# paulvoliva/XNODE-WAN-PDE-solver

Measured on AMD Instinct MI355X. Metric: WAN training-steps/sec (optimiser sub-steps, d=20 cube, N_r=4096 paths per GPU), higher is better.
Workload: dtype f64

## Files before the change

include/xnwan.h:

```cpp
#ifndef XNWAN_H
#define XNWAN_H
#ifdef __cplusplus
extern "C" {
#endif

#define XW_E_DIMS     (-1)
#define XW_E_ARG      (-2)
#define XW_E_WORKSPACE (-3)
#define XW_E_COMM     (-4)

int xw_abi_version(void);
int xw_supported_dims(char* buf, int buflen);

int xw_theta_size(int d, int H, int K);
int xw_phi_size(int d, int W);

int xw_ode_fwd(const double* xT, const double* t, const double* start, const double* theta,
               int method, int N, int L, int d, int H, int K, int m,
               double* u, double* Y, void* stream);

typedef struct { const double* xT; const double* start; double* u; double* Y; double* act; int N;
                 int act_x_only;
                 int narrow;
                 int prio_drop;
               } XwOdeFwdJob;
int xw_ode_act_rows(int method, int H, int K, int m);
int xw_ode_fwd_multi(const XwOdeFwdJob* jobs, int njobs, const double* t, const double* theta,
                     int method, int L, int d, int H, int K, int m, double* zero16, void* stream);

int xw_ode_bwd_slabs(int N);

int xw_ode_bwd(const double* xT, const double* t, const double* start, const double* theta, const double* Y,
               const double* ubar, int method, int N, int L, int d, int H, int K, int m, int mode,
               double* gx, double* gs, double* gslab, void* stream);

typedef struct { const double* xT; const double* start; const double* Y; const double* act; const double* ubar;
                 double* gx; double* gs; double* gslab; int N;
                 int res_first_only; const double* res_u; const double* res_ref; double res_coef; double res_base;
                 int res_w_per_point; const double* res_w; const double* res_c; const double* res_cp; double res_kappa2;
               } XwOdeBwdJob;
int xw_ode_bwd_multi(const XwOdeBwdJob* jobs, int njobs, const double* t, const double* theta,
                     int method, int L, int d, int H, int K, int m, int mode, void* stream);

int xw_disc_fwd(const double* xT, const double* t, const double* tpp, const double* phi,
                int N, int L, int d, int W, int q, double* v, double* vt, double* gxv, double* gtv, int ngrad,
                int max_blocks, double* act, void* stream);
int xw_disc_xproj(const double* xT, const double* phi, int N, int d, int W, double* xproj, void* stream);
int xw_disc_fwd_xproj(const double* xT, const double* t, const double* tpp, const double* phi,
                      int N, int L, int d, int W, int q, double* v, double* vt, double* gxv, double* gtv, int ngrad,
                      int max_blocks, double* act, const double* xproj, void* stream);
int xw_disc_act_rows(int W, int q);

int xw_disc_gradx(const double* xT, const double* t, const double* tpp, const double* phi, const double* vbar,
                  int N, int d, int W, int q, double* gxv, double* gtv, void* stream);

int xw_disc_bwd_slabs(int N, int L);
int xw_disc_bwd(const double* xT, const double* t, const double* tpp, const double* phi, const double* vbar,
                int N, int L, int d, int W, int q, const double* act, double* gslab, void* stream);

int xw_weak_partials(const double* u, const double* v, const double* vt, const double* w, int w_per_point,
                     const double* wt, const double* s3x, const double* gx, const double* gs, const double* ghT,
                     const double* gxv, const double* w0, const double* gwx0T, int d, const double* c, double ckappa,
                     const double* f, const double* h, const double* href, int pairwise, double s3_scale, int N, int L,
                     double Vol, double Nglob, double* work, double* scal, int finalize, int Lb, double Nbglob, double alpha,
                     double init_off, double bdry_off, long long* step, const double* ub, const double* gb, long Pb,
                     void* stream);
int xw_pair_fold(double* scal, double Vol, double Nglob, void* stream);
int xw_reduce_work_size(void);
int xw_cube_weight(const float* x, int N, int d, double top, double bot, double* w, double* w0, double* gwT, double* xT,
                   void* stream);
int xw_weak_contract_general(const double* A0, int amode, const double* B0, const double* gx, const double* gs,
                             const double* ghT, const double* gxv, const double* w0, const double* gwx0T, const double* v0,
                             int d, int N, double* s3x, void* stream);
int xw_bdry_partials(const double* ub, const double* g, int Nb, int L, double alpha, double Nbglob,
                     double* ubar_b, double* work, double* scal, void* stream);
int xw_gen_cotangents(const double* u, const double* v, const double* w, int w_per_point, const double* c,
                      const double* cp, double ckappa, const double* h, int N, int L, double Vol, double Nglob,
                      double alpha, double pollution, const double* scal, double* ubarA, double* ubarB, void* stream);
int xw_disc_cotangent(const double* u, const double* v, const double* w, int w_per_point, const double* c,
                      double ckappa, const double* f, const double* h, int N, int L, double Vol, double Nglob,
                      double pollution, double s3_scale, const double* scal_in, double* vbar, void* stream);
int xw_losses(double* scal, int L, int Lb, double Vol, double Nglob, double Nbglob, double alpha, double init_off,
              double bdry_off, long long* step, void* stream);

int xw_adam(double* param, const double* gslabA, int nA, const double* gextraA, const double* gslabB, int nB,
            const double* gextraB, const double* scal, double* m, double* v, long long* step, int bump_step, int P,
            double lr, double beta1, double beta2, double eps, double* gsum_out, int lag_lo, int lag_hi, int skip,
            long long* lag, void* stream);
int xw_slab_sum(const double* gslab, int nslab, int P, int accumulate, double* out, void* stream);
int xw_slab_sum2(const double* gA, int nA, double* outA, const double* gB, int nB, double* outB, int P, void* stream);

typedef struct {
  int N, Nb, L, Lb, d;
  int same_grid;
  int w_per_point, amode, pair_i, pair_b;
  int ns_u, ns_b;
  int narrow;
  int sharded;
  double Vol, Nglob, Nbglob, s3_scale, init_off, bdry_off, ckappa;
  const double *xT, *xvT, *xbT, *t, *tb, *tpp, *xvT_pts;
  const double *start, *start_b, *h, *href, *f, *g, *w, *wt, *w0, *ghT, *gwx0T, *c, *cp, *A0, *B0;
  double *u, *ub, *Y, *Yb, *act, *act_b, *v, *vt, *gxv, *gtv, *gx, *gs, *vbar, *s3x, *vact, *slabA, *slabB, *slab_v, *work_i, *work_b;
  double *xproj;
} XwGroup;
typedef int (*XwExchangeFn)(double* buf, int count, void* ctx, void* stream);
typedef struct {
  int method, H, K, m, W, q, Pu, Pv, adjoint;
  int v_blocks, v_blocks_disc;
  int lag_lo, lag_hi;
  double alpha, pollution, lr_u, lr_v, beta1, beta2, eps;
  double *theta, *phi, *scal, *grad_u, *grad_v, *m_u, *v_u, *m_v, *v_v;
  long long *step_u, *step_v, *lag_u;
  XwExchangeFn exchange;
  void* exchange_ctx;
  double* pack_u;
} XwSolverState;
int xw_substep_gen(const XwGroup* g, const XwSolverState* s, int skip_v, int store_record, double* accum, int adam_skip_field,
                   void* stream);
int xw_substep_disc(const XwGroup* g, const XwSolverState* s, int skip_v, int use_record, double* accum, void* stream);

int xw_comm_available(void);
int xw_comm_unique_id(unsigned char* id128);
int xw_comm_init(const unsigned char* id128, int nranks, int rank, void** comm);
int xw_allreduce(double* buf, int count, void* comm, void* stream);
int xw_comm_destroy(void* comm);

typedef struct XwGather {
  const double* src;
  double* dst;
  long n0, n1, n2;
  long s0, s1, s2;
  long before;
} XwGather;
int xw_gather_fields(const XwGather* table_dev, int count, long total, void* stream);

int xw_mt19937_uniform_f32(void* state_blob, long blob_bytes, float* out, long n, float from, float to, int fused);

int xw_mt19937_legacy_normal_f64(unsigned int* key, int* pos, int* has_gauss, double* cached_gaussian, double* out, long n);

#ifdef __cplusplus
}
#endif
#endif
```

xnode_wan_pde_solver_amd/_lib.py:

```python
import ctypes
import os

_HERE = os.path.dirname(os.path.abspath(__file__))
LIB_PATH = os.environ.get('XW_LIBRARY') or os.path.join(_HERE, 'libxnwan.so')
ABI_VERSION = 31

c_f32p = ctypes.c_void_p
c_f64p = ctypes.c_void_p
c_i64p = ctypes.c_void_p
c_int, c_dbl, c_vp = ctypes.c_int, ctypes.c_double, ctypes.c_void_p


class XwOdeFwdJob(ctypes.Structure):
    _fields_ = [('xT', c_vp), ('start', c_vp), ('u', c_vp), ('Y', c_vp), ('act', c_vp), ('N', c_int), ('act_x_only', c_int),
                ('narrow', c_int), ('prio_drop', c_int)]


class XwOdeBwdJob(ctypes.Structure):
    _fields_ = [('xT', c_vp), ('start', c_vp), ('Y', c_vp), ('act', c_vp), ('ubar', c_vp), ('gx', c_vp), ('gs', c_vp),
                ('gslab', c_vp), ('N', c_int), ('res_first_only', c_int), ('res_u', c_vp), ('res_ref', c_vp),
                ('res_coef', ctypes.c_double), ('res_base', ctypes.c_double), ('res_w_per_point', c_int), ('res_w', c_vp),
                ('res_c', c_vp), ('res_cp', c_vp), ('res_kappa2', ctypes.c_double)]


class XwGroup(ctypes.Structure):
    _fields_ = ([(n, c_int) for n in ('N', 'Nb', 'L', 'Lb', 'd', 'same_grid', 'w_per_point', 'amode', 'pair_i', 'pair_b', 'ns_u', 'ns_b',
                                      'narrow', 'sharded')]
                + [(n, c_dbl) for n in ('Vol', 'Nglob', 'Nbglob', 's3_scale', 'init_off', 'bdry_off', 'ckappa')]
                + [(n, c_vp) for n in ('xT', 'xvT', 'xbT', 't', 'tb', 'tpp', 'xvT_pts', 'start', 'start_b', 'h', 'href', 'f', 'g', 'w',
                                       'wt', 'w0', 'ghT', 'gwx0T', 'c', 'cp', 'A0', 'B0', 'u', 'ub', 'Y', 'Yb', 'act', 'act_b', 'v',
                                       'vt', 'gxv', 'gtv', 'gx', 'gs', 'vbar', 's3x', 'vact', 'slabA', 'slabB', 'slab_v', 'work_i',
                                       'work_b', 'xproj')])


class XwSolverState(ctypes.Structure):
    _fields_ = ([(n, c_int) for n in ('method', 'H', 'K', 'm', 'W', 'q', 'Pu', 'Pv', 'adjoint', 'v_blocks', 'v_blocks_disc', 'lag_lo',
                                      'lag_hi')]
                + [(n, c_dbl) for n in ('alpha', 'pollution', 'lr_u', 'lr_v', 'beta1', 'beta2', 'eps')]
                + [(n, c_vp) for n in ('theta', 'phi', 'scal', 'grad_u', 'grad_v', 'm_u', 'v_u', 'm_v', 'v_v', 'step_u', 'step_v',
                                       'lag_u', 'exchange', 'exchange_ctx', 'pack_u')])


EXCHANGE_FN = ctypes.CFUNCTYPE(ctypes.c_int, ctypes.c_void_p, ctypes.c_int, ctypes.c_void_p, ctypes.c_void_p)


SIGNATURES = {
    'xw_abi_version': [],
    'xw_supported_dims': [ctypes.c_char_p, c_int],
    'xw_theta_size': [c_int, c_int, c_int],
    'xw_phi_size': [c_int, c_int],
    'xw_ode_fwd': [c_f32p, c_f32p, c_f64p, c_f64p, c_int, c_int, c_int, c_int, c_int, c_int, c_int, c_f64p, c_f64p, c_vp],
    'xw_ode_fwd_multi': [ctypes.POINTER(XwOdeFwdJob), c_int, c_f32p, c_f64p, c_int, c_int, c_int, c_int, c_int, c_int, c_f64p,
                         c_vp],
    'xw_ode_bwd_slabs': [c_int],
    'xw_ode_act_rows': [c_int, c_int, c_int, c_int],
    'xw_ode_bwd_multi': [ctypes.POINTER(XwOdeBwdJob), c_int, c_f32p, c_f64p, c_int, c_int, c_int, c_int, c_int, c_int, c_int, c_vp],
    'xw_ode_bwd': [c_f32p, c_f32p, c_f64p, c_f64p, c_f64p, c_f64p, c_int, c_int, c_int, c_int, c_int, c_int, c_int, c_int,
                   c_f64p, c_f64p, c_f64p, c_vp],
    'xw_disc_fwd': [c_f32p, c_f32p, c_f32p, c_f64p, c_int, c_int, c_int, c_int, c_int, c_f64p, c_f64p, c_f64p, c_f64p, c_int,
                    c_int, c_f64p, c_vp],
    'xw_disc_xproj': [c_f32p, c_f64p, c_int, c_int, c_int, c_f64p, c_vp],
    'xw_disc_fwd_xproj': [c_f32p, c_f32p, c_f32p, c_f64p, c_int, c_int, c_int, c_int, c_int, c_f64p, c_f64p, c_f64p, c_f64p, c_int,
                          c_int, c_f64p, c_f64p, c_vp],
    'xw_disc_act_rows': [c_int, c_int],
    'xw_disc_gradx': [c_f32p, c_f32p, c_f32p, c_f64p, c_f64p, c_int, c_int, c_int, c_int, c_f64p, c_f64p, c_vp],
    'xw_disc_bwd_slabs': [c_int, c_int],
    'xw_disc_bwd': [c_f32p, c_f32p, c_f32p, c_f64p, c_f64p, c_int, c_int, c_int, c_int, c_int, c_f64p, c_f64p, c_vp],
    'xw_mt19937_uniform_f32': [c_vp, ctypes.c_long, c_vp, ctypes.c_long, ctypes.c_float, ctypes.c_float, c_int],
    'xw_gather_fields': [c_vp, c_int, ctypes.c_long, c_vp],
    'xw_mt19937_legacy_normal_f64': [c_vp, ctypes.POINTER(c_int), ctypes.POINTER(c_int), ctypes.POINTER(c_dbl), c_vp, ctypes.c_long],
    'xw_weak_partials': [c_f64p, c_f64p, c_f64p, c_f64p, c_int, c_f64p, c_f64p, c_f64p, c_f64p, c_f64p, c_f64p, c_f64p,
                         c_f64p, c_int, c_f64p, c_dbl, c_f64p, c_f64p, c_f64p, c_int, c_dbl, c_int, c_int, c_dbl, c_dbl, c_f64p, c_f64p,
                         c_int, c_int, c_dbl, c_dbl, c_dbl, c_dbl, c_i64p, c_f64p, c_f64p, ctypes.c_long, c_vp],
    'xw_pair_fold': [c_f64p, c_dbl, c_dbl, c_vp],
    'xw_cube_weight': [c_vp, c_int, c_int, c_dbl, c_dbl, c_f64p, c_f64p, c_f64p, c_f64p, c_vp],
    'xw_bdry_partials': [c_f64p, c_f64p, c_int, c_int, c_dbl, c_dbl, c_f64p, c_f64p, c_f64p, c_vp],
    'xw_reduce_work_size': [],
    'xw_weak_contract_general': [c_f64p, c_int, c_f64p, c_f64p, c_f64p, c_f64p, c_f64p, c_f64p, c_f64p, c_f64p, c_int, c_int, c_f64p, c_vp],
    'xw_gen_cotangents': [c_f64p, c_f64p, c_f64p, c_int, c_f64p, c_f64p, c_dbl, c_f64p, c_int, c_int, c_dbl, c_dbl, c_dbl,
                          c_dbl, c_f64p, c_f64p, c_f64p, c_vp],
    'xw_disc_cotangent': [c_f64p, c_f64p, c_f64p, c_int, c_f64p, c_dbl, c_f64p, c_f64p, c_int, c_int, c_dbl, c_dbl, c_dbl,
                          c_dbl, c_f64p, c_f64p, c_vp],
    'xw_losses': [c_f64p, c_int, c_int, c_dbl, c_dbl, c_dbl, c_dbl, c_dbl, c_dbl, c_i64p, c_vp],
    'xw_adam': [c_f64p, c_f64p, c_int, c_f64p, c_f64p, c_int, c_f64p, c_f64p, c_f64p, c_f64p, c_i64p, c_int, c_int, c_dbl,
                c_dbl, c_dbl, c_dbl, c_f64p, c_int, c_int, c_int, c_i64p, c_vp],
    'xw_substep_gen': [ctypes.POINTER(XwGroup), ctypes.POINTER(XwSolverState), c_int, c_int, c_f64p, c_int, c_vp],
    'xw_substep_disc': [ctypes.POINTER(XwGroup), ctypes.POINTER(XwSolverState), c_int, c_int, c_f64p, c_vp],
    'xw_slab_sum': [c_f64p, c_int, c_int, c_int, c_f64p, c_vp],
    'xw_slab_sum2': [c_f64p, c_int, c_f64p, c_f64p, c_int, c_f64p, c_int, c_vp],
    'xw_comm_available': [],
    'xw_comm_unique_id': [ctypes.c_char_p],
    'xw_comm_init': [ctypes.c_char_p, c_int, c_int, ctypes.POINTER(c_vp)],
    'xw_allreduce': [c_f64p, c_int, c_vp, c_vp],
    'xw_comm_destroy': [c_vp],
}

ERRORS = {-1: 'XW_E_DIMS: network widths/depths not among the compiled kernel instantiations',
          -2: 'XW_E_ARG: null pointer, non-positive size or bad enum',
          -3: 'XW_E_WORKSPACE: workspace too small',
          -4: 'XW_E_COMM: RCCL is not available in this process, or a collective call failed'}


class XnwanError(RuntimeError):
    pass


def _load():
    if not os.path.exists(LIB_PATH):
        raise XnwanError(
            'libxnwan.so not found at %s -- build it with `python -c "import __graft_entry__ as g; g.build()"` '
            'or `make -C xnode_wan_pde_solver_amd/csrc`.  There is no CPU fallback.' % LIB_PATH)
    import torch
    lib = ctypes.CDLL(LIB_PATH)
    for name, argtypes in SIGNATURES.items():
        fn = getattr(lib, name)
        fn.argtypes = argtypes
        fn.restype = ctypes.c_int
    got = lib.xw_abi_version()
    if got != ABI_VERSION:
        raise XnwanError('libxnwan.so ABI version %d, host expects %d -- rebuild' % (got, ABI_VERSION))
    return lib


lib = _load()


def check(status, what):
    if status == 0:
        return
    if status in ERRORS:
        buf = ctypes.create_string_buffer(512)
        lib.xw_supported_dims(buf, 512)
        raise XnwanError('%s: %s (compiled: %s)' % (what, ERRORS[status], buf.value.decode()))
    raise XnwanError('%s: HIP launch error %d' % (what, status))
```

xnode_wan_pde_solver_amd/csrc/xw_common.h:

```cpp
#pragma once
#include <hip/hip_runtime.h>

typedef double d4 __attribute__((ext_vector_type(4)));
#define XW_MFMA(a, b, c) __builtin_amdgcn_mfma_f64_16x16x4f64((a), (b), (c), 0, 0, 0)
#define XW_MFMA4(a, b, c) __builtin_amdgcn_mfma_f64_4x4x4f64((a), (b), (c), 0, 0, 0)

#define XW_E_DIMS (-1)
#define XW_ODE_MAX_LAYERS 10
#define XW_E_ARG (-2)
#define XW_E_WORKSPACE (-3)
#define XW_E_COMM (-4)

struct UOff {
  int IL0w, IL0b, IL2w, IL2b, IL4w, IL4b, Win, Winb, Wh, Whb, Wo, Wob, FLw, FLb, total, ldin;
};
__host__ __device__ inline UOff u_offsets(int d, int H, int K) {
  UOff o;
  int p = 0;
  o.IL0w = p; p += H;
  o.IL0b = p; p += H;
  o.IL2w = p; p += H * H;
  o.IL2b = p; p += H;
  o.IL4w = p; p += H * H;
  o.IL4b = p; p += H;
  o.ldin = d + 1 + H;
  o.Win = p; p += K * o.ldin;
  o.Winb = p; p += K;
  o.Wh = p; p += K * K;
  o.Whb = p; p += K;
  o.Wo = p; p += H * K;
  o.Wob = p; p += H;
  o.FLw = p; p += H;
  o.FLb = p; p += 1;
  o.total = p;
  return o;
}
struct VOff {
  int Vin, Vinb, Vh, Vhb, Vo, Vob, total, ldin;
};
__host__ __device__ inline VOff v_offsets(int d, int W) {
  VOff o;
  int p = 0;
  o.ldin = d + 1;
  o.Vin = p; p += W * o.ldin;
  o.Vinb = p; p += W;
  o.Vh = p; p += W * W;
  o.Vhb = p; p += W;
  o.Vo = p; p += W;
  o.Vob = p; p += 1;
  o.total = p;
  return o;
}

typedef const double __attribute__((address_space(1)))* xw_gcp;
typedef double __attribute__((address_space(1)))* xw_gp;
__device__ __forceinline__ double xw_ld_g(const double* p) { return *(xw_gcp)p; }
__device__ __forceinline__ void xw_st_g(double v, double* p) { *(xw_gp)p = v; }
__device__ __forceinline__ double xw_ld_nt(const double* p) { return __builtin_nontemporal_load((xw_gcp)p); }
__device__ __forceinline__ void xw_st_nt(double v, double* p) { __builtin_nontemporal_store(v, (xw_gp)p); }

__device__ __forceinline__ int xw_lane() { return threadIdx.x & 63; }

__device__ __forceinline__ double xw_fragA(const double* __restrict__ Mx, int ld, int rows, int cols, int r0, int c0) {
  const int l = xw_lane();
  const int r = r0 + (l & 15), c = c0 + (l >> 4);
  return (r < rows && c < cols) ? xw_ld_g(Mx + (r * ld + c)) : 0.0;
}
__device__ __forceinline__ double xw_fragAT(const double* __restrict__ Mx, int ld, int rows, int cols, int r0, int c0) {
  const int l = xw_lane();
  const int r = r0 + (l & 15), c = c0 + (l >> 4);
  return (r < cols && c < rows) ? xw_ld_g(Mx + (c * ld + r)) : 0.0;
}
__device__ __forceinline__ double xw_fragAT_l(const double* __restrict__ Mx, int ld, int rows, int cols, int r0, int c0, int l) {
  const int r = r0 + (l & 15), c = c0 + (l >> 4);
  return (r < cols && c < rows) ? xw_ld_g(Mx + (c * ld + r)) : 0.0;
}
__device__ __forceinline__ double xw_fragA4(const double* __restrict__ Mx, int ld, int rows, int cols, int r0, int c0) {
  const int l = xw_lane();
  const int r = r0 + (l & 3), c = c0 + (l >> 4);
  return (r < rows && c < cols) ? xw_ld_g(Mx + (r * ld + c)) : 0.0;
}
__device__ __forceinline__ double xw_fragAT4(const double* __restrict__ Mx, int ld, int rows, int cols, int r0, int c0) {
  const int l = xw_lane();
  const int r = r0 + (l & 3), c = c0 + (l >> 4);
  return (r < cols && c < rows) ? xw_ld_g(Mx + (c * ld + r)) : 0.0;
}
__device__ __forceinline__ double xw_relu1(double x) { return __builtin_fmax(x, 0.0); }
__device__ __forceinline__ d4 xw_vecD(const double* __restrict__ b, int rows, int r0) {
  const int g = xw_lane() >> 4;
  d4 v;
#pragma unroll
  for (int r = 0; r < 4; ++r) {
    const int i = r0 + g + 4 * r;
    v[r] = (i < rows) ? xw_ld_g(b + i) : 0.0;
  }
  return v;
}
__device__ __forceinline__ d4 xw_vecD_strided(const double* __restrict__ b, int stride, int rows, int r0) {
  const int g = xw_lane() >> 4;
  d4 v;
#pragma unroll
  for (int r = 0; r < 4; ++r) {
    const int i = r0 + g + 4 * r;
    v[r] = (i < rows) ? xw_ld_g(b + (long)i * stride) : 0.0;
  }
  return v;
}
__device__ __forceinline__ d4 xw_relu(d4 z) {
  d4 o;
#pragma unroll
  for (int r = 0; r < 4; ++r) o[r] = z[r] > 0.0 ? z[r] : 0.0;
  return o;
}
__device__ __forceinline__ double xw_gate_pos(double b, double x) {
  const unsigned t = (unsigned)__double2loint(b) | (unsigned)__double2hiint(b);
  const int m = -(int)(t < 1u ? t : 1u);
  return __hiloint2double(__double2hiint(x) & m, __double2loint(x) & m);
}
__device__ __forceinline__ d4 xw_zero4() { d4 z = {0.0, 0.0, 0.0, 0.0}; return z; }

__device__ __forceinline__ double xw_tanh(double x) {
  const double am = fmin(fabs(x), 40.0);
  const double y = -2.0 * am;
  const double nb = fma(y, 1.4426950408889634, 6755399441055744.0);
  const double n = nb - 6755399441055744.0;
  double r = fma(n, -6.93147180369123816490e-01, y);
  r = fma(n, -1.90821492927058770002e-10, r);
  double p = 2.08767569878681e-09;
  p = fma(p, r, 2.505210838544172e-08);
  p = fma(p, r, 2.755731922398589e-07);
  p = fma(p, r, 2.7557319223985893e-06);
  p = fma(p, r, 2.48015873015873e-05);
  p = fma(p, r, 0.0001984126984126984);
  p = fma(p, r, 0.001388888888888889);
  p = fma(p, r, 0.008333333333333333);
  p = fma(p, r, 0.041666666666666664);
  p = fma(p, r, 0.16666666666666666);
  p = fma(p, r, 0.5);
  p = fma(p, r, 1.0);
  p = fma(p, r, 1.0);
  const double e = __hiloint2double(__double2hiint(p) + (__double2loint(nb) << 20), __double2loint(p));
  const double num = 1.0 - e, den = 1.0 + e;
  double rc = __builtin_amdgcn_rcp(den);
  rc = fma(fma(-den, rc, 1.0), rc, rc);
  double q = num * rc;
  q = fma(fma(-den, q, num), rc, q);
  return fma(x, 0.0, copysign(q, x));
}

__device__ __forceinline__ double xw_sum_over_g(double x) {
  typedef unsigned xw_u2 __attribute__((ext_vector_type(2)));
  unsigned lo = __double2loint(x), hi = __double2hiint(x);
  xw_u2 a = __builtin_amdgcn_permlane16_swap(lo, lo, false, false);
  xw_u2 b = __builtin_amdgcn_permlane16_swap(hi, hi, false, false);
  x = __hiloint2double(b[0], a[0]) + __hiloint2double(b[1], a[1]);
  lo = __double2loint(x), hi = __double2hiint(x);
  a = __builtin_amdgcn_permlane32_swap(lo, lo, false, false);
  b = __builtin_amdgcn_permlane32_swap(hi, hi, false, false);
  return __hiloint2double(b[0], a[0]) + __hiloint2double(b[1], a[1]);
}
__device__ __forceinline__ double xw_fold32(double a, double b) {
  typedef unsigned xw_u2 __attribute__((ext_vector_type(2)));
  const xw_u2 lo = __builtin_amdgcn_permlane32_swap(__double2loint(a), __double2loint(b), false, false);
  const xw_u2 hi = __builtin_amdgcn_permlane32_swap(__double2hiint(a), __double2hiint(b), false, false);
  return __hiloint2double(hi[0], lo[0]) + __hiloint2double(hi[1], lo[1]);
}
__device__ __forceinline__ double xw_fold16(double a, double b) {
  typedef unsigned xw_u2 __attribute__((ext_vector_type(2)));
  const xw_u2 lo = __builtin_amdgcn_permlane16_swap(__double2loint(a), __double2loint(b), false, false);
  const xw_u2 hi = __builtin_amdgcn_permlane16_swap(__double2hiint(a), __double2hiint(b), false, false);
  return __hiloint2double(hi[0], lo[0]) + __hiloint2double(hi[1], lo[1]);
}
#define XW_DPP_ADD(x, CTRL)                                                                                                    \
  {                                                                                                                            \
    const int lo_ = __builtin_amdgcn_update_dpp(0, __double2loint(x), (CTRL), 0xf, 0xf, true);                                 \
    const int hi_ = __builtin_amdgcn_update_dpp(0, __double2hiint(x), (CTRL), 0xf, 0xf, true);                                 \
    x += __hiloint2double(hi_, lo_);                                                                                           \
  }
__device__ __forceinline__ double xw_sum_over_n(double x) {
  XW_DPP_ADD(x, 0xB1)
  XW_DPP_ADD(x, 0x4E)
  XW_DPP_ADD(x, 0x141)
  XW_DPP_ADD(x, 0x140)
  return x;
}

#define XW_TSTRIDE 17
#define XW_TTILE (16 * XW_TSTRIDE)
__device__ __forceinline__ void xw_writeT(double* tile, d4 q) {
  const int l = xw_lane();
  const int g = l >> 4, n = l & 15;
#pragma unroll
  for (int r = 0; r < 4; ++r) tile[(g + 4 * r) * XW_TSTRIDE + n] = q[r];
}
template <int NR> __device__ __forceinline__ void xw_writeT_n(double* tile, d4 q) {
  const int l = xw_lane();
  const int g = l >> 4, n = l & 15;
#pragma unroll
  for (int r = 0; r < NR; ++r) tile[(g + 4 * r) * XW_TSTRIDE + n] = q[r];
}
template <int NR> __device__ __forceinline__ void xw_writeT_pn(double* tile, d4 q) {
  const int l = xw_lane();
  const int g = l >> 4, n = l & 15, pn = ((n & 3) << 2) | (n >> 2);
#pragma unroll
  for (int r = 0; r < NR; ++r) tile[(g + 4 * r) * XW_TSTRIDE + pn] = q[r];
}
__device__ __forceinline__ double xw_readT(const double* tile, int ks) {
  const int l = xw_lane();
  return tile[(l & 15) * XW_TSTRIDE + 4 * ks + (l >> 4)];
}

static inline int xw_launch_status() {
  hipError_t e = hipGetLastError();
  return e == hipSuccess ? 0 : (int)e;
}
```

xnode_wan_pde_solver_amd/csrc/xw_disc.hip:

```cpp
#include "xw_common.h"
#include "xw_generic.h"
#include <atomic>
#include <cstdlib>

namespace {

template <int W> struct VDim {
  static constexpr int MT = (W + 15) / 16;
  static constexpr int KS = (W + 3) / 4;
  static constexpr int TR = W - 16 * (MT - 1);
  static constexpr bool VTAIL = TR <= 3;
  static constexpr int MTF = VTAIL ? MT - 1 : MT;
  __device__ static constexpr int LR(int mt) { return (W + 1 - 16 * mt) >= 16 ? 4 : (W + 1 - 16 * mt + 3) / 4; }
  static constexpr bool BIASROW = (W % 16) != 0;
  static_assert(MT == 4 || MT == 6 || MT == 8, "row tiles of the compiled widths");
};

struct Pt {
  int p, n;
  bool valid;
  double t;
};
__device__ __forceinline__ Pt locate(long tile, long P, int N, const double* __restrict__ tf, const double* __restrict__ tpp) {
  Pt q;
// ... 74 lines not shown
  }
  if (threadIdx.x < 16 * D::MT) {
    sB[threadIdx.x] = (int)threadIdx.x < W ? ph[o.Vhb + threadIdx.x] : 0.0;
    sB[16 * D::MT + threadIdx.x] = (int)threadIdx.x < W ? ph[o.Vo + threadIdx.x] : 0.0;
    if (VINLDS || XPROJ) {
      sIn[threadIdx.x] = (int)threadIdx.x < W ? ph[o.Vin + (long)threadIdx.x * o.ldin] : 0.0;
      sIn[16 * D::MT + threadIdx.x] = (int)threadIdx.x < W ? ph[o.Vinb + threadIdx.x] : 0.0;
    }
  }
  const int ksd = (d + 3) / 4;
  const int ksl = ksd < VKS ? ksd : VKS;
  if (VINLDS)
    for (int idx = wave; idx < ksl * D::MT; idx += 4) {
      const int ks = idx / D::MT, mt = idx - ks * D::MT;
      sVin[idx * 64 + lane] = xw_fragA(ph + o.Vin + 1, o.ldin, W, d, 16 * mt, 4 * ks);
    }
  if (D::VTAIL)
    for (int idx = threadIdx.x; idx < D::KS * 4 * D::TR; idx += blockDim.x) {
      const int r = idx % D::TR, k = idx / D::TR;
      sT[idx] = k < W ? ph[o.Vh + (long)(16 * (D::MT - 1) + r) * W + k] : 0.0;
    }
  __syncthreads();
  const double vob = ph[o.Vob];
  const long G = (long)gridDim.x * 4;
  const long rot = ntiles >= G ? ntiles % G : 0;
  const int nq = (int)gridDim.x < XW_DISC_NQ ? (int)gridDim.x : XW_DISC_NQ;
  int cur = blockIdx.x % nq, tries = 0;
  int zr = 0;
  asm volatile("" : "+v"(zr));
#ifdef XW_CLOCK_PROBE
  const unsigned long long ck0 = __builtin_amdgcn_s_memtime(), rt0 = __builtin_amdgcn_s_memrealtime();
#endif
  for (long it = (long)blockIdx.x * 4 + wave; it < ntiles;) {
    const long tile = DYN ? it : (it < G ? it - rot + (it < rot ? G : 0) : it);
    long nxt = it + G;
    unsigned int ticket = 0;
    if (DYN && lane == 0) ticket = atomicAdd(queue + cur * XW_DISC_QSTRIDE, 1u);
    const Pt pt = locate(tile, P, N, tf, tpp);
    const bool want_grad = gxv != nullptr && tile * 16 < ngrad;
    d4 a[D::MT], ad[D::MT];
    const long tu = __builtin_amdgcn_readfirstlane((int)tile);
    double* actl = act + tu * ((long)(q + 1) * W * 16);
    asm volatile("" : "+s"(actl));
    const int aoff = lane;
    const double* pht = ph;
    asm volatile("" : "+s"(pht));
    if (XPROJ) {
      const double* xp = xproj + pt.n;
#pragma unroll
      for (int mt = 0; mt < D::MT; ++mt)
#pragma unroll
        for (int r = 0; r < 4; ++r) {
          ad[mt][r] = sIn[16 * mt + g + 4 * r];
          a[mt][r] = (16 * mt + 4 * r < W) ? fma(ad[mt][r], pt.t, xw_ld_g(xp + (long)(16 * mt + 4 * r + g) * N)) : 0.0;
        }
    } else if (VINLDS) {
#pragma unroll
      for (int mt = 0; mt < D::MT; ++mt)
#pragma unroll
        for (int r = 0; r < 4; ++r) {
          ad[mt][r] = sIn[16 * mt + g + 4 * r];
          a[mt][r] = sIn[16 * D::MT + 16 * mt + g + 4 * r] + ad[mt][r] * pt.t;
        }
      for (int ks = 0; ks < ksl; ++ks) {
        const int i = 4 * ks + g;
        const double b = i < d ? xT[(long)i * N + pt.n] : 0.0;
#pragma unroll
        for (int mt = 0; mt < D::MT; ++mt) a[mt] = XW_MFMA(sVin[(ks * D::MT + mt) * 64 + lane], b, a[mt]);
      }
      for (int ks = ksl; ks < ksd; ++ks) {
        const int i = 4 * ks + g;
        const double b = i < d ? xT[(long)i * N + pt.n] : 0.0;
#pragma unroll
        for (int mt = 0; mt < D::MT; ++mt) a[mt] = XW_MFMA(xw_fragA(pht + o.Vin + 1, o.ldin, W, d, 16 * mt, 4 * ks), b, a[mt]);
      }
    } else {
      input_layer<W>(pht, o, xT, N, d, pt, a, ad);
    }
#pragma unroll
    for (int mt = 0; mt < D::MT; ++mt)
#pragma unroll
      for (int r = 0; r < 4; ++r) {
        const double x = a[mt][r];
        a[mt][r] = __hiloint2double(x == 0.0 ? (int)0x80000000 : __double2hiint(x), __double2loint(x));
      }
    if (DYN) {
      nxt = G + cur + (long)nq * (unsigned int)__builtin_amdgcn_readfirstlane((int)ticket);
      while (nxt >= ntiles && tries < XW_DISC_STEAL && tries + 1 < nq) {
        ++tries;
        cur = cur + 1 < nq ? cur + 1 : 0;
        if (lane == 0) ticket = atomicAdd(queue + cur * XW_DISC_QSTRIDE, 1u);
        nxt = G + cur + (long)nq * (unsigned int)__builtin_amdgcn_readfirstlane((int)ticket);
      }
    }
    auto layer = [&](int j, const d4 (&ai)[D::MT], const d4 (&adi)[D::MT], d4 (&nw)[D::MT], d4 (&nd)[D::MT]) {
#pragma unroll
      for (int mt = 0; mt < D::MT; ++mt) {
#pragma unroll
        for (int r = 0; r < 4; ++r) nw[mt][r] = sB[16 * mt + g + 4 * r];
        nd[mt] = xw_zero4();
      }
      if (want_grad) {
        unsigned int mask = 0;
#pragma unroll
        for (int mt = 0; mt < D::MT; ++mt)
#pragma unroll
          for (int r = 0; r < 4; ++r) mask |= (ai[mt][r] > 0.0 ? 1u : 0u) << (4 * mt + r);
        sMask[j][threadIdx.x] = mask;
      }
      double tv[D::TR], td[D::TR];
#pragma unroll
      for (int r = 0; r < D::TR; ++r) tv[r] = td[r] = 0.0;
      double wn[D::MTF], tn[D::TR];
#pragma unroll
      for (int mt = 0; mt < D::MTF; ++mt) wn[mt] = sVh[(mt * D::KS) * 64 + lane];
      if (D::VTAIL)
#pragma unroll
        for (int r = 0; r < D::TR; ++r) tn[r] = sT[g * D::TR + r];
#pragma unroll
      for (int ks = 0; ks < D::KS; ++ks) {
        const double av = ai[ks >> 2][ks & 3];
        int sgn = __double2hiint(av) >> 31;
        asm volatile("" : "+v"(sgn));
        const double adv = adi[ks >> 2][ks & 3];
        const double b = __hiloint2double((sgn & zr) | (~sgn & __double2hiint(av)), (sgn & zr) | (~sgn & __double2loint(av)));
        const double bd = __hiloint2double((sgn & zr) | (~sgn & __double2hiint(adv)), (sgn & zr) | (~sgn & __double2loint(adv)));
        if (ACT) {
          double* __restrict__ rowp = actl + (j * W + 4 * ks) * 16;
          if (4 * ks + 3 < W || 4 * ks + g < W) xw_st_nt(b, rowp + aoff);
        }
        double wc[D::MTF], tc[D::TR];
#pragma unroll
        for (int mt = 0; mt < D::MTF; ++mt) wc[mt] = wn[mt];
#pragma unroll
        for (int r = 0; r < D::TR; ++r) tc[r] = D::VTAIL ? tn[r] : 0.0;
        if (ks + 1 < D::KS) {
#pragma unroll
          for (int mt = 0; mt < D::MTF; ++mt) wn[mt] = sVh[(mt * D::KS + ks + 1) * 64 + lane];
          if (D::VTAIL)
#pragma unroll
            for (int r = 0; r < D::TR; ++r) tn[r] = sT[(4 * (ks + 1) + g) * D::TR + r];
        }
        asm volatile("" ::: "memory");
#pragma unroll
        for (int mt = 0; mt < D::MTF; ++mt) {
          nw[mt] = XW_MFMA(wc[mt], b, nw[mt]);
          nd[mt] = XW_MFMA(wc[mt], bd, nd[mt]);
        }
        if (D::VTAIL) {
#pragma unroll
          for (int r = 0; r < D::TR; ++r) {
            tv[r] = fma(tc[r], b, tv[r]);
            td[r] = fma(tc[r], bd, td[r]);
          }
        }
      }
      if (D::VTAIL && D::TR == 2) {
        const double R = xw_fold16(xw_fold32(tv[0], td[0]), xw_fold32(tv[1], td[1]));
        d4 tw = xw_zero4(), tdd = xw_zero4();
        tw[0] = R + nw[D::MT - 1][0];
        const unsigned rl = __double2loint(R), rh = __double2hiint(R);
        typedef unsigned xw_u2 __attribute__((ext_vector_type(2)));
        const xw_u2 sl = __builtin_amdgcn_permlane32_swap(rl, rl, false, false), sh = __builtin_amdgcn_permlane32_swap(rh, rh, false, false);
        tdd[0] = __hiloint2double(sh[1], sl[1]);
        nw[D::MT - 1] = tw;
        nd[D::MT - 1] = tdd;
      } else
      if (D::VTAIL) {
        d4 tw = xw_zero4(), tdd = xw_zero4();
#pragma unroll
        for (int r = 0; r < D::TR; ++r) {
          const double sv_ = xw_sum_over_g(tv[r]) + nw[D::MT - 1][0], sd_ = xw_sum_over_g(td[r]);
          if (g == r) {
            tw[0] = sv_;
            tdd[0] = sd_;
          }
        }
        nw[D::MT - 1] = tw;
        nd[D::MT - 1] = tdd;
      }
    };
    {
      d4 b0[D::MT], bd0[D::MT];
      int j = 0;
      for (; j + 1 < q; j += 2) {
        layer(j, a, ad, b0, bd0);
        layer(j + 1, b0, bd0, a, ad);
      }
      if (j < q) {
        layer(j, a, ad, b0, bd0);
#pragma unroll
        for (int mt = 0; mt < D::MT; ++mt) {
          a[mt] = b0[mt];
          ad[mt] = bd0[mt];
        }
      }
    }
    double sv = 0.0, sd = 0.0;
#pragma unroll
    for (int mt = 0; mt < D::MT; ++mt)
#pragma unroll
      for (int r = 0; r < 4; ++r)
        if (16 * mt + 4 * r < W) {
          const double th = xw_tanh(a[mt][r]);
          if (ACT && (16 * mt + 4 * r + 3 < W || 16 * mt + 4 * r + g < W))
            xw_st_nt(th, actl + (q * W + 16 * mt + 4 * r) * 16 + aoff);
          const double vo = sB[16 * D::MT + 16 * mt + g + 4 * r];
          sv += vo * th;
          sd += vo * (1.0 - th * th) * ad[mt][r];
          a[mt][r] = vo * (1.0 - th * th);
        } else {
          a[mt][r] = 0.0;
        }
    sv = xw_sum_over_g(sv) + vob;
    sd = xw_sum_over_g(sd);
    if (g == 0 && pt.valid) {
      v[pt.p] = sv;
      if (vt != nullptr) vt[pt.p] = sd;
    }
    if (want_grad) {
      const double* phg = ph;
      asm volatile("" : "+s"(phg));
      int ll = lane;
      asm volatile("" : "+v"(ll));
      d4 (&dl)[D::MT] = a;
      auto fragT = [&](int mt, int ks) -> double { return xw_fragAT_l(phg + o.Vh, W, W, W, 16 * mt, 4 * ks, ll); };
      for (int j = q - 1; j >= 0; --j) {
        d4 nd[D::MT];
#pragma unroll
        for (int mt = 0; mt < D::MT; ++mt) nd[mt] = xw_zero4();
        double fn[D::MT];
#pragma unroll
        for (int mt = 0; mt < D::MT; ++mt) fn[mt] = fragT(mt, 0);
#pragma unroll
        for (int ks = 0; ks < D::KS; ++ks) {
          const double b = dl[ks >> 2][ks & 3];
          double fc[D::MT];
#pragma unroll
          for (int mt = 0; mt < D::MT; ++mt) fc[mt] = fn[mt];
          if (ks + 1 < D::KS) {
#pragma unroll
            for (int mt = 0; mt < D::MT; ++mt) fn[mt] = fragT(mt, ks + 1);
          }
          asm volatile("" ::: "memory");
#pragma unroll
          for (int mt = 0; mt < D::MT; ++mt) nd[mt] = XW_MFMA(fc[mt], b, nd[mt]);
        }
        const unsigned int mask = sMask[j][threadIdx.x];
#pragma unroll
        for (int mt = 0; mt < D::MT; ++mt)
#pragma unroll
          for (int r = 0; r < 4; ++r) dl[mt][r] = ((mask >> (4 * mt + r)) & 1u) ? nd[mt][r] : 0.0;
      }
      int ngl = ngrad;
      asm volatile("" : "+s"(ngl));
      const bool gl = pt.valid && pt.p < ngl;
      for (int rt = 0; rt < (d + 15) / 16; ++rt) {
        d4 vv = xw_zero4();
#pragma unroll
        for (int ks = 0; ks < D::KS; ++ks) {
          if ((ks & 3) == 0) asm volatile("" ::: "memory");
          vv = XW_MFMA(xw_fragAT_l(phg + o.Vin + 1, o.ldin, W, d, 16 * rt, 4 * ks, ll), dl[ks >> 2][ks & 3], vv);
        }
#pragma unroll
        for (int r = 0; r < 4; ++r) {
          const int i = 16 * rt + g + 4 * r;
          if (i < d && gl) gxv[(long)i * ngl + pt.p] = vv[r];
        }
      }
      double st_ = 0.0;
#pragma unroll
      for (int mt = 0; mt < D::MT; ++mt) {
        const d4 v0 = xw_vecD_strided(phg + o.Vin, o.ldin, W, 16 * mt);
#pragma unroll
        for (int r = 0; r < 4; ++r) st_ += v0[r] * dl[mt][r];
      }
      st_ = xw_sum_over_g(st_);
      if (gtv != nullptr && g == 0 && gl) gtv[pt.p] = st_;
    }
    it = nxt;
  }
#ifdef XW_CLOCK_PROBE
  if (lane == 0 && blockIdx.x * 4 + wave < 4096) {
    xw_clock_buf[2 * (blockIdx.x * 4 + wave)] = __builtin_amdgcn_s_memtime() - ck0;
    xw_clock_buf[2 * (blockIdx.x * 4 + wave) + 1] = __builtin_amdgcn_s_memrealtime() - rt0;
  }
#endif
  if (DYN && lane == 0) {
    if (atomicAdd(&sDone, 1u) == 3u && atomicAdd(queue + XW_DISC_NQ * XW_DISC_QSTRIDE, 1u) == gridDim.x - 1u)
      for (int s_ = 0; s_ <= XW_DISC_NQ; ++s_) atomicExch(queue + s_ * XW_DISC_QSTRIDE, 0u);
  }
}

template <int W> struct BwdLds {
  typedef VDim<W> D;
  static constexpr int nfrag = D::MT * D::KS * 64;
  static constexpr int ntt = 4 * D::MT * XW_TTILE;
  static constexpr int oVh = 0, oVhT = nfrag, oD = 2 * nfrag, oR = 2 * nfrag + ntt, oO = 2 * nfrag + 2 * ntt;
  static constexpr int oB = oO + 4 * 64 * 16;
  static constexpr int total = oB + 2 * 16 * D::MT;
  static_assert(total * 8 <= 160 * 1024, "LDS budget of one CU");
};

template <int W, int Q, int CTG, bool PARAMS, bool INGRAD>
__global__ void __launch_bounds__(256) k_disc_bwd(const double* __restrict__ xT, const double* __restrict__ tf,
                                                  const double* __restrict__ tpp, const double* __restrict__ ph,
                                                  const double* __restrict__ vbar, int N, int L, int d,
                                                  double* __restrict__ gslab, double* __restrict__ gxv,
                                                  double* __restrict__ gtv) {
  typedef VDim<W> D;
  typedef BwdLds<W> S;
  static_assert(D::MT == 4, "the recomputing reverse kernel maps the 4 row tiles of dVh onto the 4 waves of a block");
  static_assert(D::BIASROW, "the recomputing reverse kernel takes dVh.b from the ones row");
  __shared__ double lds[S::total];
  double* sVh = lds + S::oVh;
  double* sVhT = lds + S::oVhT;
  double* sD = lds + S::oD;
  double* sR = lds + S::oR;
  double* sO = lds + S::oO;
  const int lane = xw_lane(), g = lane >> 4, n = lane & 15;
  const int wave = threadIdx.x >> 6;
  const VOff o = v_offsets(d, W);
  const long P = (long)N * L;
  const long nsuper = (P + 63) / 64;

  double* sB = lds + S::oB;
  for (int idx = wave; idx < D::MT * D::KS; idx += 4) {
    const int mt = idx / D::KS, ks = idx - mt * D::KS;
    sVh[idx * 64 + lane] = xw_fragA(ph + o.Vh, W, W, W, 16 * mt, 4 * ks);
    sVhT[idx * 64 + lane] = xw_fragAT(ph + o.Vh, W, W, W, 16 * mt, 4 * ks);
  }
  if (threadIdx.x < 16 * D::MT) {
    sB[threadIdx.x] = (int)threadIdx.x < W ? ph[o.Vhb + threadIdx.x] : 0.0;
    sB[16 * D::MT + threadIdx.x] = (int)threadIdx.x < W ? ph[o.Vo + threadIdx.x] : 0.0;
  }
  if (PARAMS)
    for (int i = 0; i < 16; ++i) sO[i * 256 + wave * 64 + lane] = 0.0;
  __syncthreads();

  d4 accH[D::MT], accIn[CTG * 4];
#pragma unroll
  for (int ct = 0; ct < D::MT; ++ct) accH[ct] = xw_zero4();
#pragma unroll
  for (int ct = 0; ct < CTG * 4; ++ct) accIn[ct] = xw_zero4();

  auto layer = [&](const d4 (&r)[D::MT], d4 (&out)[D::MT]) {
    asm volatile("" ::: "memory");
#pragma unroll
    for (int mt = 0; mt < D::MT; ++mt)
#pragma unroll
      for (int rr = 0; rr < 4; ++rr) out[mt][rr] = sB[16 * mt + g + 4 * rr];
#pragma unroll
    for (int ks = 0; ks < D::KS; ++ks) {
      const double b = r[ks >> 2][ks & 3];
#pragma unroll
      for (int mt = 0; mt < D::MT; ++mt) out[mt] = XW_MFMA(sVh[(mt * D::KS + ks) * 64 + lane], b, out[mt]);
    }
  };

  constexpr int SEG = CTG == 1 ? 1 : 3;
  constexpr int NSEG = (Q + SEG - 1) / SEG;
  for (long st = blockIdx.x; st < nsuper; st += gridDim.x) {
    const Pt pt = locate(st * 4 + wave, P, N, tf, tpp);
    d4 ck[NSEG][D::MT];
    d4 a[D::MT], ad[D::MT];
    input_layer<W>(ph, o, xT, N, d, pt, a, ad);
#pragma unroll
    for (int j = 0; j < Q; ++j) {
      d4 r[D::MT];
#pragma unroll
      for (int mt = 0; mt < D::MT; ++mt) {
#pragma unroll
        for (int q_ = 0; q_ < 4; ++q_)
          if (q_ < D::LR(mt)) {
            r[mt][q_] = a[mt][q_] > 0.0 ? a[mt][q_] : 0.0;
            if (j % SEG == 0) ck[j / SEG][mt][q_] = r[mt][q_];
          }
      }
      layer(r, a);
    }
    const double vb = pt.valid ? (vbar != nullptr ? vbar[pt.p] : 1.0) : 0.0;
    d4 dl[D::MT];
#pragma unroll
    for (int mt = 0; mt < D::MT; ++mt)
#pragma unroll
      for (int r = 0; r < 4; ++r) {
        double th = 0.0;
        if (16 * mt + 4 * r < W) th = xw_tanh(a[mt][r]);
        dl[mt][r] = sB[16 * D::MT + 16 * mt + g + 4 * r] * (1.0 - th * th) * vb;
        if (PARAMS) sO[(mt * 4 + r) * 256 + wave * 64 + lane] += (mt == D::MT - 1 && r == 3) ? (g == 0 ? vb : 0.0) : vb * th;
      }
#pragma unroll
    for (int sg = NSEG - 1; sg >= 0; --sg) {
      d4 seg[SEG][D::MT];
#pragma unroll
      for (int mt = 0; mt < D::MT; ++mt)
#pragma unroll
        for (int q_ = 0; q_ < 4; ++q_)
          if (q_ < D::LR(mt)) seg[0][mt][q_] = ck[sg][mt][q_];
#pragma unroll
      for (int k = 1; k < SEG; ++k)
        if (sg * SEG + k < Q) {
          d4 tmp[D::MT];
          layer(seg[k - 1], tmp);
#pragma unroll
          for (int mt = 0; mt < D::MT; ++mt)
#pragma unroll
            for (int q_ = 0; q_ < 4; ++q_)
              if (q_ < D::LR(mt)) seg[k][mt][q_] = tmp[mt][q_] > 0.0 ? tmp[mt][q_] : 0.0;
        }
#pragma unroll
      for (int k = SEG - 1; k >= 0; --k) {
        if (sg * SEG + k >= Q) continue;
        if (PARAMS) {
#pragma unroll
          for (int mt = 0; mt < D::MT; ++mt) {
            d4 rj = seg[k][mt];
            if (mt == (W >> 4)) {
              if (g == ((W & 15) & 3)) rj[(W & 15) >> 2] = 1.0;
            }
            if (mt < D::MT - 1) {
              xw_writeT(sD + (wave * D::MT + mt) * XW_TTILE, dl[mt]);
              xw_writeT(sR + (wave * D::MT + mt) * XW_TTILE, rj);
            } else {
              xw_writeT_n<D::LR(D::MT - 1)>(sD + (wave * D::MT + mt) * XW_TTILE, dl[mt]);
              xw_writeT_n<D::LR(D::MT - 1)>(sR + (wave * D::MT + mt) * XW_TTILE, rj);
            }
          }
        }
        d4 nd[D::MT];
        asm volatile("" ::: "memory");
#pragma unroll
        for (int mt = 0; mt < D::MT; ++mt) nd[mt] = xw_zero4();
#pragma unroll
        for (int ks = 0; ks < D::KS; ++ks) {
          const double b = dl[ks >> 2][ks & 3];
#pragma unroll
          for (int mt = 0; mt < D::MT; ++mt) nd[mt] = XW_MFMA(sVhT[(mt * D::KS + ks) * 64 + lane], b, nd[mt]);
        }
        if (PARAMS) {
          __syncthreads();
#pragma unroll
          for (int pw = 0; pw < 4; ++pw)
#pragma unroll
            for (int ks = 0; ks < 4; ++ks) {
              const double av = xw_readT(sD + (pw * D::MT + wave) * XW_TTILE, ks);
#pragma unroll
              for (int ct = 0; ct < D::MT; ++ct)
                accH[ct] = XW_MFMA(av, xw_readT(sR + (pw * D::MT + ct) * XW_TTILE, ks), accH[ct]);
            }
          __syncthreads();
        }
#pragma unroll
        for (int mt = 0; mt < D::MT; ++mt)
#pragma unroll
          for (int r = 0; r < 4; ++r)
            if (r < D::LR(mt)) dl[mt][r] = seg[k][mt][r] > 0.0 ? nd[mt][r] : 0.0;
      }
    }
    if (PARAMS) {
#pragma unroll
      for (int mt = 0; mt < D::MT; ++mt) xw_writeT(sD + (wave * D::MT + mt) * XW_TTILE, dl[mt]);
#pragma unroll
      for (int grp = 0; grp < CTG; ++grp) {
#pragma unroll
        for (int rr = 0; rr < 16; ++rr) {
          const int cl = g + 4 * rr;
          const int c = 64 * grp + cl;
          double val = 0.0;
          if (pt.valid) {
            if (c == 0) val = pt.t;
            else if (c <= d) val = xT[(long)(c - 1) * N + pt.n];
            else if (c == d + 1) val = 1.0;
          }
          sR[(wave * D::MT + (cl >> 4)) * XW_TTILE + (cl & 15) * XW_TSTRIDE + n] = val;
        }
        __syncthreads();
#pragma unroll
        for (int pw = 0; pw < 4; ++pw)
#pragma unroll
          for (int ks = 0; ks < 4; ++ks) {
            const double av = xw_readT(sD + (pw * D::MT + wave) * XW_TTILE, ks);
#pragma unroll
            for (int ct = 0; ct < 4; ++ct)
              accIn[grp * 4 + ct] = XW_MFMA(av, xw_readT(sR + (pw * D::MT + ct) * XW_TTILE, ks), accIn[grp * 4 + ct]);
          }
        __syncthreads();
      }
    }
    if (INGRAD) {
      for (int rt = 0; rt < (d + 15) / 16; ++rt) {
        d4 vv = xw_zero4();
#pragma unroll
        for (int ks = 0; ks < D::KS; ++ks)
          vv = XW_MFMA(xw_fragAT(ph + o.Vin + 1, o.ldin, W, d, 16 * rt, 4 * ks), dl[ks >> 2][ks & 3], vv);
#pragma unroll
        for (int r = 0; r < 4; ++r) {
          const int i = 16 * rt + g + 4 * r;
          if (i < d && pt.valid) gxv[(long)i * P + pt.p] = vv[r];
        }
      }
      double st_ = 0.0;
#pragma unroll
      for (int mt = 0; mt < D::MT; ++mt) {
        const d4 v0 = xw_vecD_strided(ph + o.Vin, o.ldin, W, 16 * mt);
#pragma unroll
        for (int r = 0; r < 4; ++r) st_ += v0[r] * dl[mt][r];
      }
      st_ = xw_sum_over_g(st_);
      if (gtv != nullptr && g == 0 && pt.valid) gtv[pt.p] = st_;
    }
  }

  if (PARAMS) {
    double* slab = gslab + (long)blockIdx.x * o.total;
#pragma unroll
    for (int ct = 0; ct < D::MT; ++ct) {
      const int c = 16 * ct + n;
#pragma unroll
      for (int r = 0; r < 4; ++r) {
        const int row = 16 * wave + g + 4 * r;
        if (row < W) {
          if (c < W) slab[o.Vh + row * W + c] = accH[ct][r];
          else if (c == W) slab[o.Vhb + row] = accH[ct][r];
        }
      }
    }
#pragma unroll
    for (int ct = 0; ct < CTG * 4; ++ct) {
      const int c = 16 * ct + n;
#pragma unroll
      for (int r = 0; r < 4; ++r) {
        const int row = 16 * wave + g + 4 * r;
        if (row < W) {
          if (c <= d) slab[o.Vin + row * o.ldin + c] = accIn[ct][r];
          else if (c == d + 1) slab[o.Vinb + row] = accIn[ct][r];
        }
      }
    }
    __syncthreads();
    const int tid = threadIdx.x;
    if (tid <= W) {
      double s = 0.0;
      if (tid < W) {
        const int mt = tid >> 4, gg = tid & 3, r = (tid & 15) >> 2;
        for (int wv = 0; wv < 4; ++wv)
          for (int nn = 0; nn < 16; ++nn) s += sO[(mt * 4 + r) * 256 + wv * 64 + gg * 16 + nn];
        slab[o.Vo + tid] = s;
      } else {
        for (int wv = 0; wv < 4; ++wv)
          for (int nn = 0; nn < 16; ++nn) s += sO[15 * 256 + wv * 64 + nn];
        slab[o.Vob] = s;
      }
    }
  }
}

#ifdef XW_REC_PROBE
__device__ unsigned long long xw_rec_clock[12 * 2048];
#define XW_PH(i) { const unsigned long long t_ = __builtin_amdgcn_s_memtime(); phc[i] += t_ - phl; phl = t_; }
#else
#define XW_PH(i)
#endif
template <int W> struct RecLds {
  typedef VDim<W> D;
  static constexpr bool VT = D::VTAIL;
  static_assert(!VT || D::LR(D::MT - 1) == 1, "short last row tile: vector-ALU tail + one live 4-row group");
  static constexpr int T3 = VT ? 4 * XW_TSTRIDE : XW_TTILE;
  static constexpr int wset = (D::MT - 1) * XW_TTILE + T3;
  static constexpr bool FRAG_LDS = D::MT == 4;
  static constexpr int oVhT = 0;
  static constexpr int oTT = oVhT + (FRAG_LDS ? D::MTF * D::KS * 64 : 0);
  static constexpr int oVo = oTT + (VT ? 4 * D::KS * D::TR : 0);
  static constexpr int oD = oVo + 16 * D::MT;
  static constexpr int oR = oD + 4 * wset;
  static constexpr int oO = oR + 4 * wset;
  static constexpr int NO = 4 * D::MT;
  static constexpr int total = oO + (NO + 1) * 16;
  static_assert(total * 8 <= (VT ? 80 : 160) * 1024, "two blocks per CU (short tail) / one");
  __device__ static constexpr int toff(int mt) { return mt * XW_TTILE; }
};

template <int W> __device__ __forceinline__ double rec_readT(const double* set, int mt, int ks) {
  const int l = xw_lane();
  const int row = (RecLds<W>::VT && mt == VDim<W>::MT - 1) ? (l & 3) : (l & 15);
  return set[RecLds<W>::toff(mt) + row * XW_TSTRIDE + 4 * ks + (l >> 4)];
}

template <int W, int Q, int NG, bool TSUM>
__global__ void __launch_bounds__(256, RecLds<W>::VT ? 2 : 1) k_disc_rec(const double* __restrict__ xT, const double* __restrict__ tf,
                                                     const double* __restrict__ tpp, const double* __restrict__ ph,
                                                     const double* __restrict__ vbar, int N, int L, int d,
                                                     double* __restrict__ gslab, const double* __restrict__ act, int qrt) {
  typedef VDim<W> D;
  typedef RecLds<W> S;
  __shared__ double lds[S::total];
  double* sVhT = lds + S::oVhT;
  double* sTT = lds + S::oTT;
  double* sVo = lds + S::oVo;
  double* sO = lds + S::oO;
  const int lane = xw_lane(), g = lane >> 4, n = lane & 15;
  const int wave = threadIdx.x >> 6;
  double* myD = lds + S::oD + wave * S::wset;
  double* myR = lds + S::oR + wave * S::wset;
#ifdef XW_REC_PROBE
  const unsigned long long ck_in = __builtin_amdgcn_s_memtime(), rt_in = __builtin_amdgcn_s_memrealtime();
#endif
  const VOff o = v_offsets(d, W);
  const long P = (long)N * L;
  const long nsuper = (P + 63) / 64;
  const int nq = Q > 0 ? Q : qrt;
  constexpr int UNROLL = Q > 0 ? Q : 1;
  constexpr int TW = D::MT / 2;
  const int wi = wave >> 1, wj = wave & 1;

  if (S::FRAG_LDS)
    for (int idx = wave; idx < D::MTF * D::KS; idx += 4) {
      const int mt = idx / D::KS, ks = idx - mt * D::KS;
      sVhT[idx * 64 + lane] = xw_fragAT(ph + o.Vh, W, W, W, 16 * mt, 4 * ks);
    }
  if (S::VT)
    for (int idx = threadIdx.x; idx < 4 * D::KS * D::TR; idx += blockDim.x) {
      const int r = idx % D::TR, k = idx / D::TR;
      sTT[idx] = k < W ? ph[o.Vh + (long)k * W + 16 * (D::MT - 1) + r] : 0.0;
    }
  if (threadIdx.x < 16 * D::MT) sVo[threadIdx.x] = (int)threadIdx.x < W ? ph[o.Vo + threadIdx.x] : 0.0;
  for (int idx = threadIdx.x; idx < (S::NO + 1) * 16; idx += blockDim.x) sO[idx] = 0.0;
  __syncthreads();

  d4 accH[TW * TW], accB[D::MT];
#pragma unroll
  for (int ct = 0; ct < TW * TW; ++ct) accH[ct] = xw_zero4();
#pragma unroll
  for (int ct = 0; ct < D::MT; ++ct) accB[ct] = xw_zero4();
  constexpr bool EDGE = S::VT;
  constexpr int NE = 7;
  double accE[NE];
#pragma unroll
  for (int e = 0; e < NE; ++e) accE[e] = 0.0;
  const int vstart = wave == 1 ? 7 : wave == 3 ? 6 : 0;
  const int lane16 = (lane & 15) * XW_TSTRIDE + (lane >> 4);
  const int lane4 = (lane & 3) * XW_TSTRIDE + ((lane >> 2) & 3) * 4 + (lane >> 4);
  const int offC = (wave < 3 ? S::oD + wave * XW_TTILE : S::oR + 2 * XW_TTILE) + lane16;
  const int offW = (wave < 3 ? S::oR : S::oD) + lane16;
  const int offX = (wave < 2 ? S::oD : S::oR) + 48 * XW_TSTRIDE + lane4;
  const int offV = (wave < 2 ? S::oR : S::oD) + vstart * 4 * XW_TSTRIDE + lane4;
  double* slab = gslab + (long)blockIdx.x * o.total;

#ifdef XW_REC_PROBE
  unsigned long long phc[8] = {0, 0, 0, 0, 0, 0, 0, 0}, phl = __builtin_amdgcn_s_memtime();
#endif
  const long ngs = N >> 6;
  const long ub = nsuper / gridDim.x, ur = nsuper % gridDim.x;
  const long u0 = (long)blockIdx.x * ub + ((long)blockIdx.x < ur ? (long)blockIdx.x : ur), u1 = u0 + ub + ((long)blockIdx.x < ur ? 1 : 0);
  d4 sumS[D::MT], sumT[D::MT];
#pragma unroll
  for (int mt = 0; mt < D::MT; ++mt) sumS[mt] = sumT[mt] = xw_zero4();
  bool slab_first = true;
  for (long it = TSUM ? u0 : (long)blockIdx.x; it < (TSUM ? u1 : nsuper); it += TSUM ? 1 : (long)gridDim.x) {
    const long ung = TSUM ? it / L : 0;
    const long st = TSUM ? (it - ung * L) * ngs + ung : it;
    const Pt pt = locate(st * 4 + wave, P, N, tf, tpp);
    const long ntile = (P + 15) >> 4;
    const long tl = st * 4 + wave < ntile ? st * 4 + wave : ntile - 1;
    const double* tbase = act + (long)__builtin_amdgcn_readfirstlane((int)tl) * ((long)(nq + 1) * W * 16);
    const int aoff = lane;
    auto load_layer = [&](int j, d4 (&r)[D::MT]) {
      const double* base = tbase + j * W * 16;
      asm volatile("" : "+s"(base));
#pragma unroll
      for (int mt = 0; mt < D::MT; ++mt)
#pragma unroll
        for (int q_ = 0; q_ < 4; ++q_)
          if (q_ < D::LR(mt)) {
            const int row = 16 * mt + 4 * q_ + g;
            r[mt][q_] = (16 * mt + 4 * q_ + 3 < W || row < W) ? xw_ld_nt(base + (16 * mt + 4 * q_) * 16 + aoff) : 0.0;
          }
    };
    d4 a[D::MT], rnext[D::MT];
    load_layer(nq, a);
    if (nq > 0) load_layer(nq - 1, rnext);
    const double vb = pt.valid ? (vbar != nullptr ? xw_ld_g(vbar + pt.p) : 1.0) : 0.0;
    d4 dl[D::MT];
#pragma unroll
    for (int mt = 0; mt < D::MT; ++mt)
#pragma unroll
      for (int r = 0; r < 4; ++r) {
        if (r < D::LR(mt) && 16 * mt + 4 * r < W) {
          const double th = a[mt][r];
          dl[mt][r] = sVo[16 * mt + g + 4 * r] * (1.0 - th * th) * vb;
          const double s_ = xw_sum_over_n(vb * th);
          if (n == 0) sO[(mt * 4 + r) * 16 + wave * 4 + g] += s_;
        } else {
          dl[mt][r] = 0.0;
        }
      }
    {
      const double s_ = xw_sum_over_n(vb);
      if (lane == 0) sO[S::NO * 16 + wave * 4] += s_;
    }
    XW_PH(6)
#pragma unroll UNROLL
    for (int sg = nq - 1; sg >= 0; --sg) {
      bool open[4 * D::MT];
#pragma unroll
      for (int mt = 0; mt < D::MT; ++mt)
#pragma unroll
        for (int r = 0; r < 4; ++r) open[4 * mt + r] = r < D::LR(mt) && rnext[mt][r] > 0.0;
#pragma unroll
      for (int mt = 0; mt < D::MT; ++mt) {
        d4 rr = rnext[mt];
        if (D::BIASROW && mt == (W >> 4)) {
          if (g == ((W & 15) & 3)) rr[(W & 15) >> 2] = 1.0;
        }
        if (!D::BIASROW) accB[mt] = accB[mt] + dl[mt];
        if (mt < D::MT - 1 || !S::VT) {
          xw_writeT(myD + S::toff(mt), dl[mt]);
          xw_writeT(myR + S::toff(mt), rr);
        } else {
          xw_writeT_n<1>(myD + S::toff(mt), dl[mt]);
          xw_writeT_n<1>(myR + S::toff(mt), rr);
        }
      }
      if (sg > 0) load_layer(sg - 1, rnext);
      XW_PH(0)
      d4 nd[D::MT];
      asm volatile("" ::: "memory");
#pragma unroll
      for (int mt = 0; mt < D::MT; ++mt) nd[mt] = xw_zero4();
      double tv[D::TR];
#pragma unroll
      for (int r = 0; r < D::TR; ++r) tv[r] = 0.0;
      if constexpr (S::FRAG_LDS) {
#pragma unroll
        for (int ks = 0; ks < D::KS; ++ks) {
          const double b = dl[ks >> 2][ks & 3];
          if ((ks & 1) == 0) asm volatile("" ::: "memory");
#pragma unroll
          for (int mt = 0; mt < D::MTF; ++mt) nd[mt] = XW_MFMA(sVhT[(mt * D::KS + ks) * 64 + lane], b, nd[mt]);
          if (S::VT) {
#pragma unroll
            for (int r = 0; r < D::TR; ++r) tv[r] = fma(sTT[(4 * ks + g) * D::TR + r], b, tv[r]);
          }
        }
      } else {
        const double* phg = ph;
        int ll = lane;
        asm volatile("" : "+s"(phg), "+v"(ll));
        double fn[D::MT];
#pragma unroll
        for (int mt = 0; mt < D::MT; ++mt) fn[mt] = xw_fragAT_l(phg + o.Vh, W, W, W, 16 * mt, 0, ll);
#pragma unroll
        for (int ks = 0; ks < D::KS; ++ks) {
          const double b = dl[ks >> 2][ks & 3];
          double fc[D::MT];
#pragma unroll
          for (int mt = 0; mt < D::MT; ++mt) fc[mt] = fn[mt];
          if (ks + 1 < D::KS) {
#pragma unroll
            for (int mt = 0; mt < D::MT; ++mt) fn[mt] = xw_fragAT_l(phg + o.Vh, W, W, W, 16 * mt, 4 * (ks + 1), ll);
          }
          asm volatile("" ::: "memory");
#pragma unroll
          for (int mt = 0; mt < D::MT; ++mt) nd[mt] = XW_MFMA(fc[mt], b, nd[mt]);
        }
      }
      if (S::VT) {
#pragma unroll
        for (int r = 0; r < D::TR; ++r) {
          const double s_ = xw_sum_over_g(tv[r]);
          if (g == r) nd[D::MT - 1][0] = s_;
        }
      }
      XW_PH(1)
      if (EDGE) {
#pragma unroll
        for (int ks = 0; ks < 4; ++ks)
          accH[2] = XW_MFMA(xw_readT(myD + S::toff(2), ks), xw_readT(myR + S::toff(2), ks), accH[2]);
      }
      XW_PH(2)
      __syncthreads();
      XW_PH(3)
      if (EDGE) {
#pragma unroll
        for (int pw = 0; pw < 4; ++pw) {
          const double* set = lds + pw * S::wset;
#pragma unroll
          for (int ks = 0; ks < 4; ++ks) {
            if ((ks & 1) == 0) asm volatile("" ::: "memory");
            const double xc = set[offC + 4 * ks], w0 = set[offW + 4 * ks], w1 = set[offW + XW_TTILE + 4 * ks];
            accH[0] = XW_MFMA(xc, w0, accH[0]);
            accH[1] = XW_MFMA(xc, w1, accH[1]);
          }
          asm volatile("" ::: "memory");
          const double x = set[offX];
#pragma unroll
          for (int e = 0; e < NE; ++e)
            if (e < NE - 1 || wave == 0) accE[e] = XW_MFMA4(x, set[offV + e * 4 * XW_TSTRIDE], accE[e]);
        }
      } else {
#pragma unroll
        for (int pw = 0; pw < 4; ++pw) {
          const double* setD = lds + S::oD + pw * S::wset;
          const double* setR = lds + S::oR + pw * S::wset;
#pragma unroll
          for (int ks = 0; ks < 4; ++ks) {
            if ((ks & 1) == 0) asm volatile("" ::: "memory");
            double aa[TW], bb[TW];
#pragma unroll
            for (int i_ = 0; i_ < TW; ++i_) {
              aa[i_] = rec_readT<W>(setD, TW * wi + i_, ks);
              bb[i_] = rec_readT<W>(setR, TW * wj + i_, ks);
            }
#pragma unroll
            for (int i_ = 0; i_ < TW; ++i_)
#pragma unroll
              for (int j_ = 0; j_ < TW; ++j_) accH[i_ * TW + j_] = XW_MFMA(aa[i_], bb[j_], accH[i_ * TW + j_]);
          }
        }
      }
      XW_PH(4)
      __syncthreads();
      XW_PH(5)
#pragma unroll
      for (int mt = 0; mt < D::MT; ++mt)
#pragma unroll
        for (int r = 0; r < 4; ++r) dl[mt][r] = open[4 * mt + r] ? nd[mt][r] : 0.0;
    }
    constexpr int RH = (D::MT + 3) / 4;
    struct InAcc { d4 v[RH]; };
    auto contract_input = [&](const d4 (&Dm)[D::MT], const int rows, const InAcc& acc0, InAcc* keep0) {
#pragma unroll
      for (int mt = 0; mt < D::MT; ++mt) {
        if (mt < D::MT - 1 || !S::VT) xw_writeT(myD + S::toff(mt), Dm[mt]);
        else xw_writeT_n<1>(myD + S::toff(mt), Dm[mt]);
      }
      const double* xl = xT;
      double* sl = slab;
      int gl = g, nl = n;
      asm volatile("" : "+s"(xl), "+s"(sl), "+v"(gl), "+v"(nl));
#pragma unroll
      for (int grp = 0; grp < NG; ++grp) {
        if (rows == 2 && grp > 0) break;
        const int nct = rows == 2 ? 1 : (d + 2 - 48 * grp >= 33 ? 3 : d + 2 - 48 * grp >= 17 ? 2 : 1);
#pragma unroll
        for (int rr = 0; rr < 12; ++rr) {
          if (rr >= 4 * nct) continue;
          const int cl = gl + 4 * rr;
          const int c = 48 * grp + cl;
          double val = 0.0;
          if (pt.valid) {
            if (rows == 2) val = c == 0 ? 1.0 : 0.0;
            else if (c == 0) val = rows == 0 ? pt.t : 0.0;
            else if (c <= d) val = xw_ld_g(xl + (long)(c - 1) * N + pt.n);
            else if (c == d + 1) val = 1.0;
          }
          myR[S::toff(cl >> 4) + (cl & 15) * XW_TSTRIDE + nl] = val;
        }
        __syncthreads();
        d4 accIn[RH][3];
#pragma unroll
        for (int rh = 0; rh < RH; ++rh) {
#pragma unroll
          for (int ct = 0; ct < 3; ++ct) accIn[rh][ct] = xw_zero4();
          if (grp == 0) accIn[rh][0] = acc0.v[rh];
        }
#pragma unroll
        for (int pw = 0; pw < 4; ++pw) {
          const double* setD = lds + S::oD + pw * S::wset;
          const double* setR = lds + S::oR + pw * S::wset;
#pragma unroll
          for (int ks = 0; ks < 4; ++ks) {
            double av[RH], bv[3];
#pragma unroll
            for (int rh = 0; rh < RH; ++rh) av[rh] = rec_readT<W>(setD, wave + 4 * rh < D::MT ? wave + 4 * rh : wave, ks);
#pragma unroll
            for (int ct = 0; ct < 3; ++ct) bv[ct] = ct < nct ? rec_readT<W>(setR, ct, ks) : 0.0;
#pragma unroll
            for (int rh = 0; rh < RH; ++rh)
#pragma unroll
              for (int ct = 0; ct < 3; ++ct)
                if (ct < nct) accIn[rh][ct] = XW_MFMA(av[rh], bv[ct], accIn[rh][ct]);
          }
        }
        __syncthreads();
        if (keep0 != nullptr) {
#pragma unroll
          for (int rh = 0; rh < RH; ++rh) keep0->v[rh] = accIn[rh][0];
          break;
        }
#pragma unroll
        for (int rh = 0; rh < RH; ++rh)
#pragma unroll
          for (int ct = 0; ct < 3; ++ct) {
            if (ct >= nct) continue;
            const int c = 48 * grp + 16 * ct + nl;
#pragma unroll
            for (int r = 0; r < 4; ++r) {
              const int row = 16 * (wave + 4 * rh) + gl + 4 * r;
              if (wave + 4 * rh < D::MT && row < W && c <= d + 1) {
                double* dst = c <= d ? sl + o.Vin + row * o.ldin + c : sl + o.Vinb + row;
                xw_st_g(slab_first ? accIn[rh][ct][r] : xw_ld_g(dst) + accIn[rh][ct][r], dst);
              }
            }
          }
      }
    };
    InAcc zacc;
#pragma unroll
    for (int rh = 0; rh < RH; ++rh) zacc.v[rh] = xw_zero4();
    if (!TSUM) {
      contract_input(dl, 0, zacc, nullptr);
      slab_first = false;
    } else {
      const double tl = pt.t;
#pragma unroll
      for (int mt = 0; mt < D::MT; ++mt)
#pragma unroll
        for (int r = 0; r < 4; ++r)
          if (r < D::LR(mt)) {
            sumS[mt][r] += dl[mt][r];
            sumT[mt][r] = fma(tl, dl[mt][r], sumT[mt][r]);
          }
      if (it + 1 == u1 || (it + 1) / L != ung) {
        InAcc tcol;
        contract_input(sumT, 2, zacc, &tcol);
        contract_input(sumS, 1, tcol, nullptr);
        slab_first = false;
#pragma unroll
        for (int mt = 0; mt < D::MT; ++mt) sumS[mt] = sumT[mt] = xw_zero4();
      }
    }
    XW_PH(7)
  }
#ifdef XW_REC_PROBE
  const unsigned long long ck_loop = __builtin_amdgcn_s_memtime();
#endif

  if (EDGE) {
#pragma unroll
    for (int t2 = 0; t2 < 2; ++t2)
#pragma unroll
      for (int r = 0; r < 4; ++r) {
        const int row = wave < 3 ? 16 * wave + g + 4 * r : 16 * t2 + n, c = wave < 3 ? 16 * t2 + n : 32 + g + 4 * r;
        slab[o.Vh + row * W + c] = accH[t2][r];
      }
    __syncthreads();
    double* s22 = lds + S::oD;
#pragma unroll
    for (int r = 0; r < 4; ++r) s22[wave * 256 + (g + 4 * r) * 16 + n] = accH[2][r];
    __syncthreads();
    {
      const int i = threadIdx.x >> 4, j = threadIdx.x & 15;
      slab[o.Vh + (32 + i) * W + 32 + j] = (s22[threadIdx.x] + s22[256 + threadIdx.x]) + (s22[512 + threadIdx.x] + s22[768 + threadIdx.x]);
    }
#pragma unroll
    for (int e = 0; e < NE; ++e) {
      double s_ = accE[e];
      s_ += __shfl_xor(s_, 4);
      s_ += __shfl_xor(s_, 8);
      if ((e < NE - 1 || wave == 0) && (lane & 12) == 0) {
        const int i = lane >> 4, j = lane & 3, blk = vstart + e;
        const int row = wave < 2 ? 48 + i : 4 * blk + j, c = wave < 2 ? 4 * blk + j : 48 + i;
        if (row < W) {
          if (c < W) slab[o.Vh + row * W + c] = s_;
          else if (c == W) slab[o.Vhb + row] = s_;
        }
      }
    }
  } else {
#pragma unroll
    for (int t4 = 0; t4 < TW * TW; ++t4) {
      const int c = 16 * (TW * wj + (t4 % TW)) + n;
#pragma unroll
      for (int r = 0; r < 4; ++r) {
        const int row = 16 * (TW * wi + (t4 / TW)) + g + 4 * r;
        if (row < W) {
          if (c < W) slab[o.Vh + row * W + c] = accH[t4][r];
          else if (c == W) slab[o.Vhb + row] = accH[t4][r];
        }
      }
    }
  }
  __syncthreads();
  const int tid = threadIdx.x;
  if (!D::BIASROW) {
    double* sBsum = lds + S::oD;
#pragma unroll
    for (int mt = 0; mt < D::MT; ++mt)
#pragma unroll
      for (int r = 0; r < 4; ++r) {
        const double s_ = xw_sum_over_n(accB[mt][r]);
        if (n == 0) sBsum[wave * 16 * D::MT + 16 * mt + 4 * r + g] = s_;
      }
    __syncthreads();
    if (tid < W) slab[o.Vhb + tid] = sBsum[tid] + sBsum[16 * D::MT + tid] + sBsum[32 * D::MT + tid] + sBsum[48 * D::MT + tid];
  }
  if (tid <= W) {
    double s_ = 0.0;
    if (tid < W) {
      const int mt = tid >> 4, gg = tid & 3, r = (tid & 15) >> 2;
      for (int wv = 0; wv < 4; ++wv) s_ += sO[(mt * 4 + r) * 16 + wv * 4 + gg];
      slab[o.Vo + tid] = s_;
    } else {
      for (int wv = 0; wv < 4; ++wv) s_ += sO[S::NO * 16 + wv * 4];
      slab[o.Vob] = s_;
    }
  }
#ifdef XW_REC_PROBE
  if (lane == 0 && blockIdx.x * 4 + wave < 2048) {
    unsigned long long* o_ = xw_rec_clock + 12 * (blockIdx.x * 4 + wave);
    for (int i = 0; i < 8; ++i) o_[i] = phc[i];
    const unsigned long long ck_out = __builtin_amdgcn_s_memtime();
    o_[8] = ck_loop - ck_in - (phc[0] + phc[1] + phc[2] + phc[3] + phc[4] + phc[5] + phc[6] + phc[7]);
    o_[9] = ck_out - ck_loop;
    o_[10] = ck_out - ck_in;
    o_[11] = __builtin_amdgcn_s_memrealtime() - rt_in;
  }
#endif
}

int bwd_blocks(long P) {
  long nsuper = (P + 63) / 64;
  return (int)(nsuper < 512 ? nsuper : 512);
}

}

static bool disc_width_ok(int W) { return W == 50 || W == 64 || W == 96 || W == 128; }
extern "C" int xw_disc_act_rows(int W, int q) { return ((disc_width_ok(W) && q >= 0) || xwg_disc_ok(1, W, q)) ? (q + 1) * W : XW_E_DIMS; }

namespace {
__global__ void __launch_bounds__(256) k_disc_xproj(const double* __restrict__ xT, const double* __restrict__ ph, int N, int d, int W,
                                                     double* __restrict__ xproj) {
  const int n = blockIdx.x * 256 + threadIdx.x;
  const int r0 = blockIdx.y * 4;
  if (n >= N) return;
  const VOff o = v_offsets(d, W);
  const int r1 = r0 + 1 < W ? r0 + 1 : W - 1, r2 = r0 + 2 < W ? r0 + 2 : W - 1, r3 = r0 + 3 < W ? r0 + 3 : W - 1, rr = r0 < W ? r0 : W - 1;
  const double* w0 = ph + o.Vin + (long)rr * o.ldin + 1;
  const double* w1 = ph + o.Vin + (long)r1 * o.ldin + 1;
  const double* w2 = ph + o.Vin + (long)r2 * o.ldin + 1;
  const double* w3 = ph + o.Vin + (long)r3 * o.ldin + 1;
  double a0 = ph[o.Vinb + rr], a1 = ph[o.Vinb + r1], a2 = ph[o.Vinb + r2], a3 = ph[o.Vinb + r3];
#pragma unroll 4
  for (int i = 0; i < d; ++i) {
    const double x = xT[(long)i * N + n];
    a0 = fma(w0[i], x, a0);
    a1 = fma(w1[i], x, a1);
    a2 = fma(w2[i], x, a2);
    a3 = fma(w3[i], x, a3);
  }
  xproj[(long)r0 * N + n] = r0 < W ? a0 : 0.0;
  xproj[(long)(r0 + 1) * N + n] = r0 + 1 < W ? a1 : 0.0;
  xproj[(long)(r0 + 2) * N + n] = r0 + 2 < W ? a2 : 0.0;
  xproj[(long)(r0 + 3) * N + n] = r0 + 3 < W ? a3 : 0.0;
}
}

extern "C" int xw_disc_xproj(const double* xT, const double* phi, int N, int d, int W, double* xproj, void* stream) {
  if (!xT || !phi || !xproj || N <= 0 || d <= 0) return XW_E_ARG;
  if (!disc_width_ok(W)) return XW_E_DIMS;
  hipLaunchKernelGGL(k_disc_xproj, dim3((N + 255) / 256, W > 96 ? 32 : W > 64 ? 24 : 16), dim3(256), 0, (hipStream_t)stream, xT, phi, N, d, W, xproj);
  return xw_launch_status();
}

extern "C" int xw_disc_fwd(const double* xT, const double* t, const double* tpp, const double* phi, int N, int L, int d,
                           int W, int q, double* v, double* vt, double* gxv, double* gtv, int ngrad, int max_blocks,
                           double* act, void* stream) {
  return xw_disc_fwd_xproj(xT, t, tpp, phi, N, L, d, W, q, v, vt, gxv, gtv, ngrad, max_blocks, act, nullptr, stream);
}

extern "C" int xw_disc_fwd_xproj(const double* xT, const double* t, const double* tpp, const double* phi, int N, int L, int d,
                                 int W, int q, double* v, double* vt, double* gxv, double* gtv, int ngrad, int max_blocks,
                                 double* act, const double* xproj, void* stream) {
  if (!xT || !phi || !v || N <= 0 || L <= 0 || d <= 0 || q < 0) return XW_E_ARG;
  if (!tpp && !t) return XW_E_ARG;
  if (tpp && L != 1) return XW_E_ARG;
  if (gxv && (ngrad <= 0 || (long)ngrad > (long)N * L || q > XW_QMAX)) return XW_E_ARG;
  if (!disc_width_ok(W)) return xwg_disc_fwd(xT, t, tpp, phi, N, L, d, W, q, v, vt, gxv, gtv, ngrad, act, stream);
  if (xproj != nullptr && tpp != nullptr) return XW_E_ARG;
  const long ntiles = ((long)N * L + 15) / 16;
  long blocks = (ntiles + 3) / 4;
  long cap = max_blocks > 0 ? max_blocks : 512;
  if (blocks > cap) blocks = cap;
  if ((long)N * L * 4 >= (1L << 31)) return XW_E_ARG;
  static const bool dyn_on = [] { const char* e = getenv("XW_DISC_DYNAMIC"); return !(e && e[0] == '0'); }();
  static unsigned int* qbase = [] { void* p = nullptr; (void)hipGetSymbolAddress(&p, HIP_SYMBOL(xw_disc_queue)); return (unsigned int*)p; }();
  static std::atomic<unsigned int> next_slot[2];
  const bool dyn = dyn_on && qbase != nullptr && ntiles > 4 * blocks;
  unsigned int* queue = nullptr;
  if (dyn) {
    hipStreamCaptureStatus cs = hipStreamCaptureStatusNone;
    if (hipStreamIsCapturing((hipStream_t)stream, &cs) != hipSuccess) cs = hipStreamCaptureStatusNone;
    const int half = cs == hipStreamCaptureStatusActive ? 1 : 0;
    const unsigned int slot = half * (XW_DISC_SLOTS / 2) + next_slot[half].fetch_add(1) % (XW_DISC_SLOTS / 2);
    queue = qbase + (size_t)slot * ((XW_DISC_NQ + 1) * XW_DISC_QSTRIDE);
  }
  static const bool vin_on = [] { const char* e = getenv("XW_DISC_VIN_LDS"); return !(e && e[0] == '0'); }();
  const int vks = xproj != nullptr ? -1 : (!vin_on || W > 64) ? 0 : ((d + 3) / 4 <= XW_VIN_KS ? XW_VIN_KS : XW_VIN_KS_WIDE);
#define XW_DISC_FWD2(W_, ACT_, DYN_, VIN_)                                                                                \
  hipLaunchKernelGGL((k_disc_fwd<W_, ACT_, DYN_, VIN_>), dim3((unsigned)blocks), dim3(256), 0, (hipStream_t)stream, xT, t,  \
                     tpp, phi, N, L, d, q, v, vt, gxv, gtv, ngrad, act, queue, xproj)
#define XW_DISC_FWD(W_, ACT_, DYN_) do { if (vks < 0) XW_DISC_FWD2(W_, ACT_, DYN_, -1); else if (vks == XW_VIN_KS) XW_DISC_FWD2(W_, ACT_, DYN_, XW_VIN_KS); else if (vks) XW_DISC_FWD2(W_, ACT_, DYN_, XW_VIN_KS_WIDE); else XW_DISC_FWD2(W_, ACT_, DYN_, 0); } while (0)
#define XW_DISC_FWD_W(W_)                                                                                                 \
  if (act != nullptr) {                                                                                                   \
    if (dyn) XW_DISC_FWD(W_, true, true); else XW_DISC_FWD(W_, true, false);                                              \
  } else {                                                                                                                \
    if (dyn) XW_DISC_FWD(W_, false, true); else XW_DISC_FWD(W_, false, false);                                            \
  }
  if (W == 50) { XW_DISC_FWD_W(50) } else if (W == 64) { XW_DISC_FWD_W(64) }
  else {
    if (blocks > 256) blocks = 256;
#define XW_DISC_FWDW(W_, ACT_, DYN_) do { if (vks < 0) XW_DISC_FWD2(W_, ACT_, DYN_, -1); else XW_DISC_FWD2(W_, ACT_, DYN_, 0); } while (0)
#define XW_DISC_FWD128(ACT_, DYN_) do { if (W == 96) XW_DISC_FWDW(96, ACT_, DYN_); else XW_DISC_FWDW(128, ACT_, DYN_); } while (0)
    const bool dyn128 = dyn && ntiles > 4 * blocks;
    if (!dyn128) queue = nullptr;
    if (act != nullptr) { if (dyn128) XW_DISC_FWD128(true, true); else XW_DISC_FWD128(true, false); }
    else { if (dyn128) XW_DISC_FWD128(false, true); else XW_DISC_FWD128(false, false); }
#undef XW_DISC_FWD128
#undef XW_DISC_FWDW
  }
#undef XW_DISC_FWD_W
#undef XW_DISC_FWD
#undef XW_DISC_FWD2
  return xw_launch_status();
}

#ifdef XW_CLOCK_PROBE
extern "C" int xw_debug_clock(unsigned long long* host, int nwaves) {
  return (int)hipMemcpyFromSymbol(host, HIP_SYMBOL(xw_clock_buf), sizeof(unsigned long long) * 2 * nwaves);
}
#endif

#ifdef XW_REC_PROBE
extern "C" int xw_debug_rec_clock(unsigned long long* host, int nwaves) {
  return (int)hipMemcpyFromSymbol(host, HIP_SYMBOL(xw_rec_clock), sizeof(unsigned long long) * 12 * nwaves);
}
#endif

extern "C" int xw_disc_bwd_slabs(int N, int L) { return bwd_blocks((long)N * L); }

#define XW_DISC_BWD(PARAMS, INGRAD)                                                                                      \
  if (d + 2 <= 64)                                                                                                       \
    hipLaunchKernelGGL((k_disc_bwd<50, 9, 1, PARAMS, INGRAD>), dim3(blocks), dim3(256), 0, s, xT, t, tpp, phi, vbar,     \
                       N, L, d, gslab, gxv, gtv);                                                                        \
  else                                                                                                                   \
    hipLaunchKernelGGL((k_disc_bwd<50, 9, 2, PARAMS, INGRAD>), dim3(blocks), dim3(256), 0, s, xT, t, tpp, phi, vbar,     \
                       N, L, d, gslab, gxv, gtv);

extern "C" int xw_disc_bwd(const double* xT, const double* t, const double* tpp, const double* phi, const double* vbar,
                           int N, int L, int d, int W, int q, const double* act, double* gslab, void* stream) {
  if (!xT || !phi || !gslab || N <= 0 || L <= 0 || d <= 0) return XW_E_ARG;
  if (!tpp && !t) return XW_E_ARG;
  if (tpp && L != 1) return XW_E_ARG;
  if (!disc_width_ok(W)) return xwg_disc_bwd(xT, t, tpp, phi, vbar, N, L, d, W, q, act, gslab, bwd_blocks((long)N * L), stream);
  if (q < 0 || d + 2 > 128 || ((q != 9 || W != 50) && act == nullptr)) return XW_E_DIMS;
  if ((long)N * L * 4 >= (1L << 31)) return XW_E_ARG;
  hipStream_t s = (hipStream_t)stream;
  const int blocks = bwd_blocks((long)N * L);
  double* gxv = nullptr;
  double* gtv = nullptr;
  if (act != nullptr) {
    const int ng = d + 2 <= 48 ? 1 : d + 2 <= 96 ? 2 : 3;
    static const bool tsum_on = [] { const char* e = getenv("XW_DISC_REC_TSUM"); return !(e && e[0] == '0'); }();
    const bool tsum = tsum_on && tpp == nullptr && (N % 64) == 0;
#define XW_DISC_REC(W_, Q, NG)                                                                                          \
    if (tsum) hipLaunchKernelGGL((k_disc_rec<W_, Q, NG, true>), dim3(blocks), dim3(256), 0, s, xT, t, tpp, phi, vbar, N, L, d, gslab, act, q); \
    else hipLaunchKernelGGL((k_disc_rec<W_, Q, NG, false>), dim3(blocks), dim3(256), 0, s, xT, t, tpp, phi, vbar, N, L, d, gslab, act, q);
    if (W == 128) {
      if (ng == 1) { XW_DISC_REC(128, 0, 1) } else if (ng == 2) { XW_DISC_REC(128, 0, 2) } else { XW_DISC_REC(128, 0, 3) }
    } else if (W == 96) {
      if (ng == 1) { XW_DISC_REC(96, 0, 1) } else if (ng == 2) { XW_DISC_REC(96, 0, 2) } else { XW_DISC_REC(96, 0, 3) }
    } else if (W == 64) {
      if (ng == 1) { XW_DISC_REC(64, 0, 1) } else if (ng == 2) { XW_DISC_REC(64, 0, 2) } else { XW_DISC_REC(64, 0, 3) }
    } else {
      if (ng == 1) { XW_DISC_REC(50, 0, 1) } else if (ng == 2) { XW_DISC_REC(50, 0, 2) } else { XW_DISC_REC(50, 0, 3) }
    }
#undef XW_DISC_REC
  } else {
    XW_DISC_BWD(true, false)
  }
  return xw_launch_status();
}

extern "C" int xw_disc_gradx(const double* xT, const double* t, const double* tpp, const double* phi, const double* vbar,
                             int N, int d, int W, int q, double* gxv, double* gtv, void* stream) {
  if (!xT || !phi || !gxv || N <= 0 || d <= 0) return XW_E_ARG;
  if (!tpp && !t) return XW_E_ARG;
  if (W != 50 || q != 9 || d + 2 > 128) return XW_E_DIMS;
  hipStream_t s = (hipStream_t)stream;
  const int L = 1;
  const int blocks = bwd_blocks((long)N);
  double* gslab = nullptr;
  XW_DISC_BWD(false, true)
  return xw_launch_status();
}
```

xnode_wan_pde_solver_amd/csrc/xw_substep.hip:

```cpp
#include <hip/hip_runtime.h>
#include <string.h>
#include "xnwan.h"

namespace {
struct Side {
  hipStream_t s = nullptr;
  hipEvent_t fork = nullptr, fwd = nullptr, done = nullptr;
};
Side* side_of_current_device() {
  static Side sides[64];
  int dev = 0;
  if (hipGetDevice(&dev) != hipSuccess || dev < 0 || dev >= 64) return nullptr;
  Side& x = sides[dev];
  if (x.s == nullptr) {
    if (hipStreamCreateWithFlags(&x.s, hipStreamNonBlocking) != hipSuccess) return nullptr;
    if (hipEventCreateWithFlags(&x.fork, hipEventDisableTiming) != hipSuccess || hipEventCreateWithFlags(&x.fwd, hipEventDisableTiming) != hipSuccess ||
        hipEventCreateWithFlags(&x.done, hipEventDisableTiming) != hipSuccess)
      return nullptr;
  }
  return &x;
}
#define XW_HIP(call) { const hipError_t e_ = (call); if (e_ != hipSuccess) return (int)e_; }

inline XwOdeFwdJob fwd_job(const double* xT, const double* start, double* u, double* Y, double* act, int N, int x_only, int narrow) {
  XwOdeFwdJob j;
  j.xT = xT; j.start = start; j.u = u; j.Y = Y; j.act = act; j.N = N; j.act_x_only = x_only; j.narrow = narrow; j.prio_drop = 0;
  return j;
}
inline XwOdeBwdJob bwd_job(const double* xT, const double* start, const double* Y, const double* act, int N) {
  XwOdeBwdJob j;
  memset(&j, 0, sizeof(j));
  j.xT = xT; j.start = start; j.Y = Y; j.act = act; j.N = N;
  return j;
}
#define XW_TRY(call) { const int rc_ = (call); if (rc_ != 0) return rc_; }

int test_net(const XwGroup* g, const XwSolverState* s, int blocks, double* record, void* stream) {
  if (g->tpp != nullptr)
    return xw_disc_fwd(g->xvT_pts, nullptr, g->tpp, s->phi, g->N * g->L, 1, g->d, s->W, s->q, g->v, g->vt, g->gxv, g->gtv, g->N, blocks,
                       record, stream);
  if (g->xproj != nullptr) XW_TRY(xw_disc_xproj(g->xvT, s->phi, g->N, g->d, s->W, g->xproj, stream));
  return xw_disc_fwd_xproj(g->xvT, g->t, nullptr, s->phi, g->N, g->L, g->d, s->W, s->q, g->v, g->vt, g->gxv, g->gtv, g->N, blocks, record,
                           g->xproj, stream);
}
int contract(const XwGroup* g, const XwSolverState* s, long long* step, bool with_bdry, bool finalize, void* stream) {
  const double* s3x = nullptr;
  if (g->A0 != nullptr || g->B0 != nullptr) {
    XW_TRY(xw_weak_contract_general(g->A0, g->amode, g->B0, g->gx, g->gs, g->ghT, g->gxv, g->w0, g->gwx0T, g->v, g->d, g->N, g->s3x,
                                    stream));
    s3x = g->s3x;
  }
  const bool fused = s3x == nullptr;
  return xw_weak_partials(g->u, g->v, g->vt, g->w, g->w_per_point, g->wt, s3x, fused ? g->gx : nullptr, fused ? g->gs : nullptr,
                          fused ? g->ghT : nullptr, fused ? g->gxv : nullptr, fused ? g->w0 : nullptr, fused ? g->gwx0T : nullptr,
                          fused ? g->d : 0, g->c, g->ckappa, g->f, g->h, g->pair_i ? g->href : nullptr, g->pair_i ? 1 : 0,
                          g->pair_i ? g->s3_scale : 1.0, g->N, g->L, g->Vol, g->Nglob, g->work_i, s->scal, finalize ? 1 : 0,
                          g->Lb > 0 ? g->Lb : 1, g->Nbglob, s->alpha, g->init_off, g->bdry_off, finalize ? step : nullptr, with_bdry && g->Nb > 0 ? g->ub : nullptr,
                          with_bdry && g->Nb > 0 ? g->g : nullptr, with_bdry && g->Nb > 0 ? (long)g->Nb * g->Lb : 0, stream);
}
inline bool sharded(const XwGroup* g, const XwSolverState* s) { return g->sharded != 0 && s->exchange != nullptr; }
#define XW_ZERO(ptr, count) XW_HIP(hipMemsetAsync((ptr), 0, sizeof(double) * (size_t)(count), (hipStream_t)stream))
}

extern "C" int xw_substep_gen(const XwGroup* g, const XwSolverState* s, int skip_v, int store_record, double* accum,
                              int adam_skip_field, void* stream) {
  if (!g || !s || g->N < 0 || g->Nb < 0 || g->L <= 0) return XW_E_ARG;
  const bool shard = sharded(g, s);
  if (g->N == 0 && !shard) return XW_E_ARG;
  if (shard && (!s->pack_u || s->scal != s->pack_u + 2 * (long)s->Pu)) return XW_E_ARG;
  const bool fused_x = s->pollution == 1.0 && !s->adjoint;
  const bool have_i = g->N > 0, have_b = g->Nb > 0;
  const bool joint = have_i && have_b && g->same_grid;
  const int adj = s->adjoint ? 8 : 0;
  void* const main_stream = stream;
  if (have_i) {
    Side* sd = side_of_current_device();
    if (sd == nullptr) return XW_E_ARG;
    XW_HIP(hipEventRecord(sd->fork, (hipStream_t)main_stream));
    XW_HIP(hipStreamWaitEvent(sd->s, sd->fork, 0));
    if (!skip_v) XW_TRY(test_net(g, s, s->v_blocks, store_record ? g->vact : nullptr, main_stream));
    stream = (void*)sd->s;
    {
      XwOdeFwdJob jobs[2] = {fwd_job(g->xT, g->start, g->u, g->Y, g->act, g->N, 0, (g->narrow >> 0) & 1),
                             fwd_job(g->xbT, g->start_b, g->ub, g->Yb, g->act_b, g->Nb, 0, (g->narrow >> 0) & 1)};
      XW_TRY(xw_ode_fwd_multi(jobs, joint ? 2 : 1, g->t, s->theta, s->method, g->L, g->d, s->H, s->K, s->m, s->scal, stream));
      if (have_b && !joint) {
        XwOdeFwdJob jb = fwd_job(g->xbT, g->start_b, g->ub, g->Yb, g->act_b, g->Nb, 0, (g->narrow >> 1) & 1);
        XW_TRY(xw_ode_fwd_multi(&jb, 1, g->tb, s->theta, s->method, g->Lb, g->d, s->H, s->K, s->m, nullptr, stream));
      }
    }
    XW_HIP(hipEventRecord(sd->fwd, sd->s));
    stream = main_stream;
    XW_HIP(hipStreamWaitEvent((hipStream_t)main_stream, sd->fwd, 0));
  } else {
    XW_ZERO(s->scal, 16);
    if (have_b) {
      XwOdeFwdJob jb = fwd_job(g->xbT, g->start_b, g->ub, g->Yb, g->act_b, g->Nb, 0, (g->narrow >> 1) & 1);
      XW_TRY(xw_ode_fwd_multi(&jb, 1, g->tb, s->theta, s->method, g->Lb, g->d, s->H, s->K, s->m, nullptr, stream));
    }
  }
  if (have_i && !fused_x) {
    XwOdeBwdJob jx = bwd_job(g->xT, g->start, g->Y, g->act, g->N);
    jx.gx = g->gx; jx.gs = g->gs;
    XW_TRY(xw_ode_bwd_multi(&jx, 1, g->t, s->theta, s->method, g->L, g->d, s->H, s->K, s->m, 1 | adj | (((g->narrow >> 5) & 1) ? 16 : 0),
                            stream));
  }
  {
    XwOdeBwdJob jobs[3];
    int nj = 0;
    if (have_i) {
      jobs[nj] = bwd_job(g->xT, g->start, g->Y, g->act, g->N);
      jobs[nj].gslab = g->slabA;
      if (fused_x) { jobs[nj].gx = g->gx; jobs[nj].gs = g->gs; }
      jobs[nj].res_u = g->u; jobs[nj].res_ref = g->pair_i ? g->href : g->h; jobs[nj].res_first_only = 1;
      jobs[nj].res_coef = 2.0 * s->alpha / g->Nglob; jobs[nj].res_base = s->pollution;
      ++nj;
    }
    XwOdeBwdJob jb = bwd_job(g->xbT, g->start_b, g->Yb, g->act_b, g->Nb);
    if (have_b) {
      jb.gslab = g->slabA + (long)g->ns_u * s->Pu;
      jb.res_u = g->ub; jb.res_ref = g->g; jb.res_first_only = 0;
      jb.res_coef = 2.0 * s->alpha / (g->Nbglob * g->Lb); jb.res_base = 0.0;
    }
    if (joint) jobs[nj++] = jb;
    if (have_i) {
      XwOdeBwdJob jB = bwd_job(g->xT, g->start, g->Y, g->act, g->N);
      jB.gslab = g->slabB;
      jB.res_first_only = 2; jB.res_u = g->u; jB.res_ref = g->v;
      jB.res_coef = g->Vol / g->Nglob / g->L * g->s3_scale; jB.res_base = g->Vol / g->Nglob;
      jB.res_w_per_point = g->w_per_point; jB.res_w = g->w; jB.res_c = g->c; jB.res_cp = g->cp; jB.res_kappa2 = 2.0 * g->ckappa;
      jobs[nj++] = jB;
      const int modeA = (fused_x ? (1 | 2 | 4) : 2) | adj | (((g->narrow >> 2) & 1) ? 16 : 0);
      XW_TRY(xw_ode_bwd_multi(jobs, nj, g->t, s->theta, s->method, g->L, g->d, s->H, s->K, s->m, modeA, stream));
    }
    if (have_b && !joint)
      XW_TRY(xw_ode_bwd_multi(&jb, 1, g->tb, s->theta, s->method, g->Lb, g->d, s->H, s->K, s->m, 2 | adj | (((g->narrow >> 3) & 1) ? 16 : 0),
                              stream));
  }
  if (have_i) {
    XW_TRY(contract(g, s, s->step_u, true, !shard, stream));
  } else if (have_b) {
    XW_TRY(xw_bdry_partials(g->ub, g->g, g->Nb, g->Lb, s->alpha, g->Nbglob, nullptr, g->work_b, s->scal, stream));
  }
  if (!shard) {
    XW_TRY(xw_adam(s->theta, g->slabA, g->ns_u + g->ns_b, accum, g->slabB, g->ns_u, nullptr, s->scal, s->m_u, s->v_u, s->step_u, -1, s->Pu,
                   s->lr_u, s->beta1, s->beta2, s->eps, s->grad_u, s->lag_lo, s->lag_hi, adam_skip_field, s->lag_u, stream));
  } else {
    const int nA = (have_i ? g->ns_u : 0) + (have_b ? g->ns_b : 0), nB = have_i ? g->ns_u : 0;
    double* const pA = s->pack_u;
    double* const pB = s->pack_u + s->Pu;
    if (nA > 0 && nB > 0) {
      XW_TRY(xw_slab_sum2(g->slabA, nA, pA, g->slabB, nB, pB, s->Pu, stream));
    } else {
      if (nA > 0) { XW_TRY(xw_slab_sum(g->slabA + (have_i ? 0 : (long)g->ns_u * s->Pu), nA, s->Pu, 0, pA, stream)); } else { XW_ZERO(pA, s->Pu); }
      XW_ZERO(pB, s->Pu);
    }
    XW_TRY(s->exchange(s->pack_u, 2 * s->Pu + 16, s->exchange_ctx, stream));
    if (g->pair_i) XW_TRY(xw_pair_fold(s->scal, g->Vol, g->Nglob, stream));
    XW_TRY(xw_losses(s->scal, g->L, g->Lb > 0 ? g->Lb : 1, g->Vol, g->Nglob, g->Nbglob, s->alpha, g->init_off, g->bdry_off, s->step_u, stream));
    XW_TRY(xw_adam(s->theta, accum, accum != nullptr ? 1 : 0, pA, nullptr, 0, pB, s->scal, s->m_u, s->v_u, s->step_u, -1, s->Pu, s->lr_u,
                   s->beta1, s->beta2, s->eps, s->grad_u, s->lag_lo, s->lag_hi, adam_skip_field, s->lag_u, stream));
  }
  if (accum != nullptr) {
    const hipError_t e = hipMemcpyAsync(accum, s->grad_u, sizeof(double) * s->Pu, hipMemcpyDeviceToDevice, (hipStream_t)stream);
    if (e != hipSuccess) return (int)e;
  }
  return 0;
}

extern "C" int xw_substep_disc(const XwGroup* g, const XwSolverState* s, int skip_v, int use_record, double* accum, void* stream) {
  if (!g || !s || g->N < 0 || g->L <= 0) return XW_E_ARG;
  const bool shard = sharded(g, s);
  if (g->N == 0 && !shard) return XW_E_ARG;
  const bool have_i = g->N > 0;
  const int adj = s->adjoint ? 8 : 0;
  double* record = use_record ? g->vact : nullptr;
  void* const main_stream = stream;
  if (have_i) {
    Side* sd = side_of_current_device();
    if (sd == nullptr) return XW_E_ARG;
    XW_HIP(hipEventRecord(sd->fork, (hipStream_t)main_stream));
    XW_HIP(hipStreamWaitEvent(sd->s, sd->fork, 0));
    if (!skip_v) XW_TRY(test_net(g, s, s->v_blocks_disc, record, main_stream));
    stream = (void*)sd->s;
    {
      XwOdeFwdJob jf = fwd_job(g->xT, g->start, g->u, g->Y, g->act, g->N, 1, (g->narrow >> 6) & 1);
      XW_TRY(xw_ode_fwd_multi(&jf, 1, g->t, s->theta, s->method, g->L, g->d, s->H, s->K, s->m, s->scal, stream));
      XwOdeBwdJob jx = bwd_job(g->xT, g->start, g->Y, g->act, g->N);
      jx.gx = g->gx; jx.gs = g->gs;
      XW_TRY(xw_ode_bwd_multi(&jx, 1, g->t, s->theta, s->method, g->L, g->d, s->H, s->K, s->m, 1 | adj | (((g->narrow >> 7) & 1) ? 16 : 0),
                              stream));
    }
    XW_HIP(hipEventRecord(sd->done, sd->s));
    stream = main_stream;
    XW_HIP(hipStreamWaitEvent((hipStream_t)main_stream, sd->done, 0));
    XW_TRY(contract(g, s, s->step_v, false, !shard, stream));
  } else {
    XW_ZERO(s->scal, 16);
  }
  if (shard) {
    XW_TRY(s->exchange(s->scal, 9, s->exchange_ctx, stream));
    if (g->pair_i) XW_TRY(xw_pair_fold(s->scal, g->Vol, g->Nglob, stream));
  }
  const int nsv = have_i ? xw_disc_bwd_slabs(g->N, g->L) : 0;
  if (have_i) {
    XW_TRY(xw_disc_cotangent(g->u, g->v, g->w, g->w_per_point, g->c, g->ckappa, g->f, g->h, g->N, g->L, g->Vol, g->Nglob, s->pollution,
                             g->s3_scale, s->scal, g->vbar, stream));
    if (g->tpp != nullptr) {
      XW_TRY(xw_disc_bwd(g->xvT_pts, nullptr, g->tpp, s->phi, g->vbar, g->N * g->L, 1, g->d, s->W, s->q, record, g->slab_v, stream));
    } else {
      XW_TRY(xw_disc_bwd(g->xvT, g->t, nullptr, s->phi, g->vbar, g->N, g->L, g->d, s->W, s->q, record, g->slab_v, stream));
    }
  }
  if (!shard) {
    XW_TRY(xw_adam(s->phi, g->slab_v, nsv, accum, nullptr, 0, nullptr, nullptr, s->m_v, s->v_v, s->step_v, -1, s->Pv, s->lr_v, s->beta1,
                   s->beta2, s->eps, s->grad_v, 0, 0, 0, nullptr, stream));
  } else {
    if (have_i) { XW_TRY(xw_slab_sum(g->slab_v, nsv, s->Pv, 0, s->grad_v, stream)); } else { XW_ZERO(s->grad_v, s->Pv); }
    XW_TRY(s->exchange(s->grad_v, s->Pv, s->exchange_ctx, stream));
    XW_TRY(xw_losses(s->scal, g->L, g->Lb > 0 ? g->Lb : 1, g->Vol, g->Nglob, g->Nbglob, s->alpha, 0.0, 0.0, s->step_v, stream));
    XW_TRY(xw_adam(s->phi, accum, accum != nullptr ? 1 : 0, s->grad_v, nullptr, 0, nullptr, nullptr, s->m_v, s->v_v, s->step_v, -1, s->Pv,
                   s->lr_v, s->beta1, s->beta2, s->eps, s->grad_v, 0, 0, 0, nullptr, stream));
  }
  if (accum != nullptr) {
    const hipError_t e = hipMemcpyAsync(accum, s->grad_v, sizeof(double) * s->Pv, hipMemcpyDeviceToDevice, (hipStream_t)stream);
    if (e != hipSuccess) return (int)e;
  }
  return 0;
}
```

xnode_wan_pde_solver_amd/csrc/xw_weak.hip:

```cpp
#include "xw_common.h"
#include "xnwan.h"

namespace {

__device__ __forceinline__ double wave_sum(double x) { return xw_sum_over_g(xw_sum_over_n(x)); }
template <int NV>
__device__ __forceinline__ bool grid_sum(double (&val)[NV], double* __restrict__ work, double* __restrict__ dst) {
  __shared__ double red[NV][16];
  __shared__ int is_last;
  const int wave = threadIdx.x >> 6, lane = threadIdx.x & 63;
#pragma unroll
  for (int i = 0; i < NV; ++i) {
    const double s = wave_sum(val[i]);
    if (lane == 0) red[i][wave] = s;
  }
  __syncthreads();
  if (threadIdx.x < NV) {
    double s = 0.0;
    for (int w = 0; w < (int)(blockDim.x >> 6); ++w) s += red[threadIdx.x][w];
    work[(long)blockIdx.x * NV + threadIdx.x] = s;
  }
  asm volatile("s_waitcnt vmcnt(0)" ::: "memory");
  __syncthreads();
  unsigned int* ticket = reinterpret_cast<unsigned int*>(work + (long)gridDim.x * NV);
  if (threadIdx.x == 0) {
    __builtin_amdgcn_fence(__ATOMIC_RELEASE, "agent");
    asm volatile("s_waitcnt vmcnt(0)" ::: "memory");
    const unsigned int t = __hip_atomic_fetch_add(ticket, 1u, __ATOMIC_RELAXED, __HIP_MEMORY_SCOPE_AGENT);
    is_last = (t == gridDim.x - 1);
    if (is_last) {
      __builtin_amdgcn_fence(__ATOMIC_ACQUIRE, "agent");
      asm volatile("s_waitcnt vmcnt(0)" ::: "memory");
    }
  }
  __syncthreads();
  if (!is_last) return false;
#pragma unroll
  for (int i = 0; i < NV; ++i) {
    double part = 0.0;
    for (unsigned int b = threadIdx.x; b < gridDim.x; b += blockDim.x) part += work[(long)b * NV + i];
    const double s = wave_sum(part);
    if (lane == 0) red[i][wave] = s;
  }
  __syncthreads();
  if (threadIdx.x < NV) {
    double tot = 0.0;
    for (int w = 0; w < (int)(blockDim.x >> 6); ++w) tot += red[threadIdx.x][w];
    dst[threadIdx.x < 3 ? threadIdx.x : (threadIdx.x < 5 ? threadIdx.x + 4 : threadIdx.x - 2)] += tot;
  }
  if (threadIdx.x == 0) *ticket = 0u;
  return true;
}

__device__ __forceinline__ double interior_loss(const double* scal, double Vol, double Nglob, int L) {
  const double I = scal[0], S = scal[1];
  return log(I * I) - log(Vol * S / (Nglob * (double)L));
}

__device__ __forceinline__ void fold_pairs(double* scal, double cN) {
  scal[0] -= cN * scal[7] * scal[8];
  scal[7] = 0.0;
  scal[8] = 0.0;
}
__device__ __forceinline__ void loss_values(double* scal, int L, int Lb, double Vol, double Nglob, double Nbglob,
                                            double alpha, double init_off, double bdry_off) {
  const double in_ = interior_loss(scal, Vol, Nglob, L);
  scal[6] = in_;
  scal[4] = in_ + alpha * ((scal[2] / Nglob + init_off) + (scal[3] / (Nbglob * (double)Lb) + bdry_off));
  scal[5] = -in_;
}

__global__ void __launch_bounds__(1024) k_weak_partials(const double* __restrict__ u, const double* __restrict__ v,
                                                       const double* __restrict__ vt, const double* __restrict__ w,
                                                       int w_per_point, const double* __restrict__ wt,
                                                       const double* __restrict__ s3x, const double* __restrict__ gx,
                                                       const double* __restrict__ gs, const double* __restrict__ ghT,
                                                       const double* __restrict__ gxv, const double* __restrict__ w0,
                                                       const double* __restrict__ gwx0T, int d,
                                                       const double* __restrict__ c, double ckappa,
                                                       const double* __restrict__ f, const double* __restrict__ h,
                                                       const double* __restrict__ href, int pairwise, double s3_scale,
                                                       int N, int L, double Vol, double Nglob, double* __restrict__ work,
                                                       double* __restrict__ scal, int finalize, int Lb, double Nbglob,
                                                       double alpha, double init_off, double bdry_off,
                                                       long long* __restrict__ step, const double* __restrict__ ub,
                                                       const double* __restrict__ gb, long Pb) {
  double acc[6] = {0.0, 0.0, 0.0, 0.0, 0.0, 0.0};
  const double cN = Vol / Nglob, cNL = Vol / Nglob / (double)L;
  const long P = (long)N * L;
  for (long p = (long)blockIdx.x * blockDim.x + threadIdx.x; p < P; p += (long)gridDim.x * blockDim.x) {
    const int l = (int)(p / N), n = (int)(p - (long)l * N);
    const double ul = u[p], vl = v[p];
    const double wl = w_per_point ? w[p] : w[n];
    const double phi = vl * wl;
    double phit = wl * vt[p];
    if (wt != nullptr) phit += vl * wt[p];
    const double cl = c != nullptr ? c[p] : ckappa * ul;
    double s3 = cl * ul * phi + f[p] * phi;
    double I = 0.0;
    if (l == 0) {
      const double hn = h[n];
      double s31;
      s31 = s3x != nullptr ? s3x[n] : 0.0;
      s3 += s31;
      I -= cN * hn * vl;
      const double hr = href != nullptr ? href[n] : hn;
      acc[2] += (ul - hr) * (ul - hr);
    }
    if (s3x == nullptr) {
      double part = 0.0;
      if (l < d) {
        const double w0n = w0[n], gsn = gs[n], v0n = v[n];
        for (int i = l; i < d; i += L) {
          const long q = (long)i * N + n;
          part += (w0n * gxv[q] + v0n * gwx0T[q]) * (gx[q] + gsn * ghT[q]);
        }
      }
      I += cNL * s3_scale * part;
    }
    if (l == L - 1) I += cN * ul * vl;
    if (pairwise) {
      I += cNL * s3_scale * s3;
      acc[3] += ul;
      acc[4] += phit;
    } else {
      I -= cNL * (ul * phit - s3_scale * s3);
    }
    acc[0] += I;
    acc[1] += vl * vl;
  }
  if (ub != nullptr)
    for (long p = (long)blockIdx.x * blockDim.x + threadIdx.x; p < Pb; p += (long)gridDim.x * blockDim.x) {
      const double r = ub[p] - gb[p];
      acc[5] += r * r;
    }
  const bool last = grid_sum<6>(acc, work, scal);
  if (finalize && last) {
    __syncthreads();
    if (threadIdx.x == 0) {
      if (step != nullptr) *step += 1;
      if (pairwise) fold_pairs(scal, cN);
      loss_values(scal, L, Lb, Vol, Nglob, Nbglob, alpha, init_off, bdry_off);
    }
  }
}

__global__ void __launch_bounds__(1024) k_bdry(const double* __restrict__ ub, const double* __restrict__ gb, long P,
                                              double coef, double* __restrict__ ubar_b, double* __restrict__ work,
                                              double* __restrict__ scal) {
  double acc[1] = {0.0};
  for (long p = (long)blockIdx.x * blockDim.x + threadIdx.x; p < P; p += (long)gridDim.x * blockDim.x) {
    const double r = ub[p] - gb[p];
    acc[0] += r * r;
    if (ubar_b != nullptr) ubar_b[p] = coef * r;
  }
  grid_sum<1>(acc, work, scal + 3);
}


__global__ void __launch_bounds__(256) k_gen_cots(const double* __restrict__ u, const double* __restrict__ v,
                                                  const double* __restrict__ w, int w_per_point,
                                                  const double* __restrict__ c, const double* __restrict__ cp,
                                                  double ckappa, const double* __restrict__ h, int N, int L, double Vol,
                                                  double Nglob, double alpha, double pollution,
                                                  const double* __restrict__ scal, double* __restrict__ ubarA,
                                                  double* __restrict__ ubarB) {
  const double cI = scal != nullptr ? 2.0 / scal[0] : 0.0;
  const double cN = Vol / Nglob, cNL = Vol / Nglob / (double)L;
  const long P = (long)N * L;
  for (long p = (long)blockIdx.x * blockDim.x + threadIdx.x; p < P; p += (long)gridDim.x * blockDim.x) {
    const int l = (int)(p / N), n = (int)(p - (long)l * N);
    const double ul = u[p];
    const bool needB = ubarB != nullptr || scal != nullptr;
    const double vl = needB ? v[p] : 0.0;
    const double wl = w_per_point ? w[p] : w[n];
    const double dcu = c != nullptr ? c[p] + ul * cp[p] : 2.0 * ckappa * ul;
    double gB = 0.0;
    if (needB) {
      gB = cNL * dcu * vl * wl;
      if (l == L - 1) gB += cN * vl;
      if (ubarB != nullptr) ubarB[p] = gB;
    }
    if (ubarA != nullptr) {
      double gA = pollution;
      if (l == 0) gA += alpha * 2.0 * (ul - h[n]) / Nglob;
      ubarA[p] = gA + cI * gB;
    }
  }
}

__global__ void k_losses(double* __restrict__ scal, int L, int Lb, double Vol, double Nglob, double Nbglob, double alpha,
                         double init_off, double bdry_off, long long* __restrict__ step) {
  if (blockIdx.x == 0 && threadIdx.x == 0) {
    if (step != nullptr) *step += 1;
    loss_values(scal, L, Lb, Vol, Nglob, Nbglob, alpha, init_off, bdry_off);
  }
}
__global__ void k_pair_fold(double* __restrict__ scal, double cN) {
  if (blockIdx.x == 0 && threadIdx.x == 0) fold_pairs(scal, cN);
}

__global__ void __launch_bounds__(256) k_cube_weight(const float* __restrict__ x, int N, int d, float top, float bot,
                                                     double* __restrict__ w, double* __restrict__ w0,
                                                     double* __restrict__ gwT, double* __restrict__ xT) {
  for (int n = blockIdx.x * blockDim.x + threadIdx.x; n < N; n += gridDim.x * blockDim.x) {
    const float* xn = x + (long)n * d;
    float at = fabsf(top - xn[0]), ab = fabsf(bot - xn[0]);
    int it = 0, ib = 0;
    for (int i = 1; i < d; ++i) {
      const float a = fabsf(top - xn[i]), b = fabsf(bot - xn[i]);
      if (a < at) { at = a; it = i; }
      if (b < ab) { ab = b; ib = i; }
    }
    const float wv = ab < at ? ab : at;
    const float ct = (at < ab ? 1.0f : 0.0f) + (at == ab ? 0.5f : 0.0f), cb = (ab < at ? 1.0f : 0.0f) + (at == ab ? 0.5f : 0.0f);
    const float dt = top - xn[it], db = bot - xn[ib];
    const float gt = -(dt > 0.0f ? 1.0f : (dt < 0.0f ? -1.0f : 0.0f)) * ct, gb = -(db > 0.0f ? 1.0f : (db < 0.0f ? -1.0f : 0.0f)) * cb;
    w[n] = (double)wv;
    if (w0) w0[n] = (double)wv;
    for (int i = 0; i < d; ++i) {
      float g = 0.0f;
      if (i == it) g += gt;
      if (i == ib) g += gb;
      gwT[(long)i * N + n] = (double)g;
      if (xT) xT[(long)i * N + n] = (double)xn[i];
    }
  }
}

__global__ void __launch_bounds__(256) k_disc_cot(const double* __restrict__ u, const double* __restrict__ v,
                                                  const double* __restrict__ w, int w_per_point,
                                                  const double* __restrict__ c, double ckappa,
                                                  const double* __restrict__ f, const double* __restrict__ h, int N,
                                                  int L, double Vol, double Nglob, double pollution, double s3_scale,
                                                  const double* __restrict__ scal_in, double* __restrict__ vbar) {
  const double I = scal_in[0], S = scal_in[1];
  const double cI = 2.0 / I;
  const double cN = Vol / Nglob, cNL = Vol / Nglob / (double)L;
  const long P = (long)N * L;
  for (long p = (long)blockIdx.x * blockDim.x + threadIdx.x; p < P; p += (long)gridDim.x * blockDim.x) {
    const int l = (int)(p / N), n = (int)(p - (long)l * N);
    const double ul = u[p], vl = v[p];
    const double wl = w_per_point ? w[p] : w[n];
    const double cl = c != nullptr ? c[p] : ckappa * ul;
    double dI = cNL * s3_scale * (cl * ul + f[p]) * wl;
    if (l == L - 1) dI += cN * ul;
    if (l == 0) dI -= cN * h[n];
    vbar[p] = pollution * wl - cI * dI + 2.0 * vl / S;
  }
}

#define XW_ADAM_PARAMS 16
#define XW_ADAM_GROUPS 64
__global__ void __launch_bounds__(1024) k_adam(double* __restrict__ param, const double* __restrict__ gA, int nA,
                                               const double* eA, const double* __restrict__ gB, int nB,
                                               const double* eB, const double* __restrict__ scal,
                                               double* __restrict__ m, double* __restrict__ v,
                                               const long long* __restrict__ step, int step_is_current, int P, double lr,
                                               double beta1, double beta2, double eps, double* gsum_out,
                                               int lag_lo, int lag_hi, int skip, const long long* __restrict__ lag) {
  __shared__ double red[2][XW_ADAM_GROUPS][XW_ADAM_PARAMS];
  const int tx = threadIdx.x % XW_ADAM_PARAMS, ty = threadIdx.x / XW_ADAM_PARAMS;
  const int i = blockIdx.x * XW_ADAM_PARAMS + tx;
  double a = 0.0, b = 0.0;
  if (i < P) {
    for (int s = ty; s < nA; s += XW_ADAM_GROUPS) a += gA[(long)s * P + i];
    for (int s = ty; s < nB; s += XW_ADAM_GROUPS) b += gB[(long)s * P + i];
  }
  red[0][ty][tx] = a;
  red[1][ty][tx] = b;
  __syncthreads();
  if (ty != 0 || i >= P) return;
  a = eA != nullptr ? eA[i] : 0.0;
  b = eB != nullptr ? eB[i] : 0.0;
#pragma unroll 8
  for (int k = 0; k < XW_ADAM_GROUPS; ++k) {
    a += red[0][k][tx];
    b += red[1][k][tx];
  }
  const double coefB = scal != nullptr ? 2.0 / scal[0] : 1.0;
  const double g = a + coefB * b;
  if (gsum_out != nullptr) gsum_out[i] = g;
  const bool lagged = i >= lag_lo && i < lag_hi;
  if (lagged && skip) return;
  const long long t = *step + (step_is_current ? 0 : 1) - (lagged && lag != nullptr ? *lag : 0);
  const double bc1 = 1.0 - pow(beta1, (double)t), bc2 = 1.0 - pow(beta2, (double)t);
  const double mi = beta1 * m[i] + (1.0 - beta1) * g;
  const double vi = beta2 * v[i] + (1.0 - beta2) * g * g;
  m[i] = mi;
  v[i] = vi;
  param[i] -= (lr / bc1) * (mi / (sqrt(vi) / sqrt(bc2) + eps));
}
__global__ void k_step_inc(long long* step) { *step += 1; }

__global__ void __launch_bounds__(1024) k_slab_sum(const double* __restrict__ gslab, int nslab, int P, int accumulate,
                                                   double* __restrict__ out) {
  __shared__ double red[XW_ADAM_GROUPS][XW_ADAM_PARAMS];
  const int tx = threadIdx.x % XW_ADAM_PARAMS, ty = threadIdx.x / XW_ADAM_PARAMS;
  const int i = blockIdx.x * XW_ADAM_PARAMS + tx;
  double a = 0.0;
  if (i < P)
    for (int s = ty; s < nslab; s += XW_ADAM_GROUPS) a += gslab[(long)s * P + i];
  red[ty][tx] = a;
  __syncthreads();
  if (ty != 0 || i >= P) return;
  double g = accumulate ? out[i] : 0.0;
#pragma unroll 8
  for (int k = 0; k < XW_ADAM_GROUPS; ++k) g += red[k][tx];
  out[i] = g;
}

inline int reduce_cap(long points) {
  static const int v = [] { const char* e = getenv("XW_REDUCE_BLOCKS"); const int x = e ? atoi(e) : 0; return x > 0 && x <= 1024 ? x : 0; }();
  return v ? v : (points > (1L << 18) ? 256 : 128);
}
inline int reduce_threads() {
  static const int v = [] { const char* e = getenv("XW_REDUCE_THREADS"); const int x = e ? atoi(e) : 0; return (x == 256 || x == 512) ? x : 1024; }();
  return v;
}
inline int blocks_for(long n, int per, int cap) {
  long b = (n + per - 1) / per;
  if (b < 1) b = 1;
  return (int)(b > cap ? cap : b);
}


__global__ void __launch_bounds__(256) k_weak_contract(const double* __restrict__ A0, int amode,
                                                       const double* __restrict__ B0, const double* __restrict__ gx,
                                                       const double* __restrict__ gs, const double* __restrict__ ghT,
                                                       const double* __restrict__ gxv, const double* __restrict__ w0,
                                                       const double* __restrict__ gwx0T, const double* __restrict__ v0,
                                                       int d, int N, double* __restrict__ s3x) {
  const int n = blockIdx.x * blockDim.x + threadIdx.x;
  if (n >= N) return;
  const double w = w0[n], v = v0[n], gsn = gs[n];
  double acc = 0.0, bsum = 0.0;
  for (int i = 0; i < d; ++i) {
    const double dphi = w * gxv[(long)i * N + n] + v * gwx0T[(long)i * N + n];
    const double dui = gx[(long)i * N + n] + gsn * ghT[(long)i * N + n];
    if (B0 != nullptr) bsum += B0[(long)i * N + n] * dui;
    if (amode == 0) {
      acc += dphi * dui;
    } else if (amode == 2) {
      acc += A0[(long)i * N + n] * dphi * dui;
    } else {
      double row = 0.0;
      for (int j = 0; j < d; ++j) {
        const double duj = gx[(long)j * N + n] + gsn * ghT[(long)j * N + n];
        const double a = amode == 1 ? A0[i * d + j] : A0[((long)i * d + j) * N + n];
        row += a * duj;
      }
      acc += dphi * row;
    }
  }
  s3x[n] = acc + v * w * bsum;
}
}

extern "C" int xw_weak_partials(const double* u, const double* v, const double* vt, const double* w, int w_per_point,
                                const double* wt, const double* s3x, const double* gx, const double* gs, const double* ghT,
                                const double* gxv, const double* w0, const double* gwx0T, int d, const double* c,
                                double ckappa, const double* f, const double* h, const double* href, int pairwise,
                                double s3_scale, int N, int L, double Vol, double Nglob, double* work, double* scal,
                                int finalize, int Lb, double Nbglob, double alpha, double init_off, double bdry_off,
                                long long* step, const double* ub, const double* gb, long Pb, void* stream) {
  if (!u || !v || !vt || !w || !f || !h || !work || !scal || N <= 0 || L <= 0 || (finalize && Lb <= 0)) return XW_E_ARG;
  if ((ub == nullptr) != (gb == nullptr) || (ub != nullptr && Pb <= 0)) return XW_E_ARG;
  if (!s3x && (!gx || !gs || !ghT || !gxv || !w0 || !gwx0T || d <= 0)) return XW_E_ARG;
  if (pairwise && L != 1) return XW_E_ARG;
  hipLaunchKernelGGL(k_weak_partials, dim3(blocks_for((long)N * L, reduce_threads(), reduce_cap((long)N * L))), dim3(reduce_threads()), 0, (hipStream_t)stream, u, v, vt, w,
                     w_per_point, wt, s3x, gx, gs, ghT, gxv, w0, gwx0T, d, c, ckappa, f, h, href, pairwise, s3_scale, N, L, Vol,
                     Nglob, work, scal, finalize, Lb, Nbglob, alpha, init_off, bdry_off, step, ub, gb, Pb);
  return xw_launch_status();
}

extern "C" int xw_bdry_partials(const double* ub, const double* g, int Nb, int L, double alpha, double Nbglob,
                                double* ubar_b, double* work, double* scal, void* stream) {
  if (!ub || !g || !work || !scal || Nb <= 0 || L <= 0) return XW_E_ARG;
  const long P = (long)Nb * L;
  const double coef = alpha * 2.0 / (Nbglob * (double)L);
  hipLaunchKernelGGL(k_bdry, dim3(blocks_for(P, reduce_threads(), reduce_cap(P))), dim3(reduce_threads()), 0, (hipStream_t)stream, ub, g, P, coef, ubar_b, work, scal);
  return xw_launch_status();
}

extern "C" int xw_gen_cotangents(const double* u, const double* v, const double* w, int w_per_point, const double* c,
                                 const double* cp, double ckappa, const double* h, int N, int L, double Vol, double Nglob,
                                 double alpha, double pollution, const double* scal, double* ubarA, double* ubarB,
                                 void* stream) {
  if (!u || !w || !h || (!ubarA && !ubarB) || ((ubarB || scal) && !v) || (scal && (!ubarA || ubarB)) || N <= 0 || L <= 0)
    return XW_E_ARG;
  if ((c == nullptr) != (cp == nullptr)) return XW_E_ARG;
  hipLaunchKernelGGL(k_gen_cots, dim3(blocks_for((long)N * L, 256, 2048)), dim3(256), 0, (hipStream_t)stream, u, v, w,
                     w_per_point, c, cp, ckappa, h, N, L, Vol, Nglob, alpha, pollution, scal, ubarA, ubarB);
  return xw_launch_status();
}

extern "C" int xw_losses(double* scal, int L, int Lb, double Vol, double Nglob, double Nbglob, double alpha,
                         double init_off, double bdry_off, long long* step, void* stream) {
  if (!scal || L <= 0 || Lb <= 0) return XW_E_ARG;
  hipLaunchKernelGGL(k_losses, dim3(1), dim3(64), 0, (hipStream_t)stream, scal, L, Lb, Vol, Nglob, Nbglob, alpha, init_off,
                     bdry_off, step);
  return xw_launch_status();
}

extern "C" int xw_pair_fold(double* scal, double Vol, double Nglob, void* stream) {
  if (!scal || Nglob <= 0) return XW_E_ARG;
  hipLaunchKernelGGL(k_pair_fold, dim3(1), dim3(64), 0, (hipStream_t)stream, scal, Vol / Nglob);
  return xw_launch_status();
}

extern "C" int xw_cube_weight(const float* x, int N, int d, double top, double bot, double* w, double* w0, double* gwT,
                              double* xT, void* stream) {
  if (!x || !w || !gwT || N <= 0 || d <= 0 || !(top > bot)) return XW_E_ARG;
  hipLaunchKernelGGL(k_cube_weight, dim3(blocks_for(N, 256, 1024)), dim3(256), 0, (hipStream_t)stream, x, N, d, (float)top,
                     (float)bot, w, w0, gwT, xT);
  return xw_launch_status();
}

namespace {
__global__ __launch_bounds__(256) void k_gather_fields(const XwGather* __restrict__ tab, int count, long total) {
  __shared__ long first[1025];
  for (int r = threadIdx.x; r <= count; r += blockDim.x) first[r] = r < count ? tab[r].before : total;
  __syncthreads();
  const long stride = (long)gridDim.x * blockDim.x;
  for (long e = (long)blockIdx.x * blockDim.x + threadIdx.x; e < total; e += stride) {
    int lo = 0, hi = count;
    while (hi - lo > 1) {
      const int mid = (lo + hi) >> 1;
      if (first[mid] <= e) lo = mid; else hi = mid;
    }
    const XwGather g = tab[lo];
    const long local = e - g.before;
    const long k = local % g.n2, ij = local / g.n2, j = ij % g.n1, i = ij / g.n1;
    g.dst[local] = g.src[i * g.s0 + j * g.s1 + k * g.s2];
  }
}
}

extern "C" int xw_gather_fields(const XwGather* table_dev, int count, long total, void* stream) {
  if (!table_dev || count <= 0 || count > 1024 || total <= 0) return XW_E_ARG;
  hipLaunchKernelGGL(k_gather_fields, dim3(blocks_for(total, 256, 2048)), dim3(256), 0, (hipStream_t)stream, table_dev, count, total);
  return xw_launch_status();
}

extern "C" int xw_disc_cotangent(const double* u, const double* v, const double* w, int w_per_point, const double* c,
                                 double ckappa, const double* f, const double* h, int N, int L, double Vol, double Nglob,
                                 double pollution, double s3_scale, const double* scal_in, double* vbar, void* stream) {
  if (!u || !v || !w || !f || !h || !scal_in || !vbar || N <= 0 || L <= 0) return XW_E_ARG;
  hipLaunchKernelGGL(k_disc_cot, dim3(blocks_for((long)N * L, 256, 2048)), dim3(256), 0, (hipStream_t)stream, u, v, w,
                     w_per_point, c, ckappa, f, h, N, L, Vol, Nglob, pollution, s3_scale, scal_in, vbar);
  return xw_launch_status();
}

extern "C" int xw_adam(double* param, const double* gslabA, int nA, const double* gextraA, const double* gslabB, int nB,
                       const double* gextraB, const double* scal, double* m, double* v, long long* step, int bump_step,
                       int P, double lr, double beta1, double beta2, double eps, double* gsum_out, int lag_lo, int lag_hi,
                       int skip, long long* lag, void* stream) {
  if (!param || !m || !v || !step || P <= 0 || nA < 0 || nB < 0 || (nA > 0 && !gslabA) || (nB > 0 && !gslabB)) return XW_E_ARG;
  if (lag_lo < 0 || lag_hi > P || (skip && (!lag || lag_hi <= lag_lo))) return XW_E_ARG;
  hipLaunchKernelGGL(k_adam, dim3((P + XW_ADAM_PARAMS - 1) / XW_ADAM_PARAMS), dim3(1024), 0, (hipStream_t)stream, param, gslabA, nA, gextraA, gslabB,
                     nB, gextraB, scal, m, v, step, bump_step < 0 ? 1 : 0, P, lr, beta1, beta2, eps, gsum_out, lag_lo, lag_hi, skip,
                     lag);
  if (skip) hipLaunchKernelGGL(k_step_inc, dim3(1), dim3(1), 0, (hipStream_t)stream, lag);
  if (bump_step > 0) hipLaunchKernelGGL(k_step_inc, dim3(1), dim3(1), 0, (hipStream_t)stream, step);
  return xw_launch_status();
}

namespace {
__global__ void __launch_bounds__(1024) k_slab_sum2(const double* __restrict__ gA, int nA, double* __restrict__ outA,
                                                    const double* __restrict__ gB, int nB, double* __restrict__ outB, int P) {
  __shared__ double red[XW_ADAM_GROUPS][XW_ADAM_PARAMS];
  const double* __restrict__ gslab = blockIdx.y == 0 ? gA : gB;
  const int nslab = blockIdx.y == 0 ? nA : nB;
  double* __restrict__ out = blockIdx.y == 0 ? outA : outB;
  const int tx = threadIdx.x % XW_ADAM_PARAMS, ty = threadIdx.x / XW_ADAM_PARAMS;
  const int i = blockIdx.x * XW_ADAM_PARAMS + tx;
  double a = 0.0;
  if (i < P)
    for (int s = ty; s < nslab; s += XW_ADAM_GROUPS) a += gslab[(long)s * P + i];
  red[ty][tx] = a;
  __syncthreads();
  if (ty != 0 || i >= P) return;
  double g = 0.0;
#pragma unroll 8
  for (int k = 0; k < XW_ADAM_GROUPS; ++k) g += red[k][tx];
  out[i] = g;
}
}
extern "C" int xw_slab_sum2(const double* gA, int nA, double* outA, const double* gB, int nB, double* outB, int P, void* stream) {
  if (!gA || !gB || !outA || !outB || P <= 0 || nA <= 0 || nB <= 0) return XW_E_ARG;
  hipLaunchKernelGGL(k_slab_sum2, dim3((P + XW_ADAM_PARAMS - 1) / XW_ADAM_PARAMS, 2), dim3(XW_ADAM_PARAMS * XW_ADAM_GROUPS), 0,
                     (hipStream_t)stream, gA, nA, outA, gB, nB, outB, P);
  return xw_launch_status();
}

extern "C" int xw_slab_sum(const double* gslab, int nslab, int P, int accumulate, double* out, void* stream) {
  if (!gslab || !out || P <= 0 || nslab <= 0) return XW_E_ARG;
  hipLaunchKernelGGL(k_slab_sum, dim3((P + XW_ADAM_PARAMS - 1) / XW_ADAM_PARAMS), dim3(XW_ADAM_PARAMS * XW_ADAM_GROUPS), 0,
                     (hipStream_t)stream, gslab, nslab, P, accumulate, out);
  return xw_launch_status();
}

extern "C" int xw_abi_version(void) { return 31; }
extern "C" int xw_reduce_work_size(void) { return 6 * 1024 + 8; }

extern "C" int xw_supported_dims(char* buf, int buflen) {
  static const char s[] = "ode (H,K)=(20,10),(32,12),(64,16), m=1..10 [MFMA]; any other H<=64, K<=16, m<=32 [generic path: vector ALU, slow]; disc_fwd W=50,64,96,128 any q; disc_bwd W=50 (q=9 unrolled, any q from the record), W=64,96,128 (from the record) [MFMA]; any other W<=128, q<=16 [generic path, from the record]; d<=126";
  int i = 0;
  for (; s[i] && i < buflen - 1; ++i) buf[i] = s[i];
  if (buflen > 0) buf[i] = 0;
  return i;
}

extern "C" int xw_theta_size(int d, int H, int K) { return u_offsets(d, H, K).total; }
extern "C" int xw_phi_size(int d, int W) { return v_offsets(d, W).total; }

extern "C" int xw_weak_contract_general(const double* A0, int amode, const double* B0, const double* gx, const double* gs,
                                        const double* ghT, const double* gxv, const double* w0, const double* gwx0T,
                                        const double* v0, int d, int N, double* s3x, void* stream) {
  if (!gx || !gs || !ghT || !gxv || !w0 || !gwx0T || !v0 || !s3x || d <= 0 || N <= 0 || amode < 0 || amode > 3 ||
      (amode != 0 && !A0))
    return XW_E_ARG;
  hipLaunchKernelGGL(k_weak_contract, dim3((N + 255) / 256), dim3(256), 0, (hipStream_t)stream, A0, amode, B0, gx, gs, ghT, gxv,
                     w0, gwx0T, v0, d, N, s3x);
  return xw_launch_status();
}
```

xnode_wan_pde_solver_amd/engine.py:

```python
import contextlib
import math
import os

import torch

from . import kernels as KN
from ._lib import XnwanError
from .options import EngineOptions
from .sampling import HIP_HOST_LOCK, _PIN_POOL, Hypercube, _paths


def ctypes_addr(fn):
    import ctypes
    return ctypes.cast(fn, ctypes.c_void_p).value

_KEPT_GRAPHS = []

_NOSTREAM = contextlib.nullcontext()

_SCRATCH_POOL = []


_DEVICE_STREAMS = {}

# ... 781 lines not shown
                return 0
            except BaseException as e:
                self._exchange_error = e
                return -4
        return EXCHANGE_FN(exchange)

    def _runner_group(self, G):
        from ._lib import XwGroup
        xg = getattr(G, '_xw_group', None)
        if xg is None:
            xg = G._xw_group = XwGroup()
            p = lambda t: 0 if t is None else t.data_ptr()
            xg.N, xg.Nb, xg.L, xg.Lb, xg.d = G.N, G.Nb, G.L, G.Lb, self.d
            xg.same_grid, xg.w_per_point, xg.amode = int(bool(G.same_grid)), int(G.w.dim() == 2), int(G.amode)
            xg.ns_u, xg.ns_b = G.ns_u, G.ns_b
            for k in ('xT', 'xvT', 'xbT', 't', 'tb', 'tpp', 'xvT_pts', 'start', 'start_b', 'h', 'href', 'f', 'g', 'w', 'wt', 'w0', 'ghT',
                      'gwx0T', 'A0', 'B0', 'u', 'Y', 'act', 'act_b', 'v', 'vt', 'gxv', 'gtv', 'gx', 'gs', 'vbar', 's3x', 'vact',
                      'xproj', 'slabA', 'slabB', 'slab_v', 'work_i', 'work_b', 'ub', 'Yb'):
                setattr(xg, k, G.ptr(k))
            nar = lambda jobs, **kw: self._narrow_ok(jobs, **kw)
            ji, jb = self._job(G, 'i'), (self._job(G, 'b') if G.Nb else None)
            joint = G.Nb and G.same_grid
            bits = [nar([ji] + ([jb] if joint else []), alone=False, forward=True),
                    bool(jb) and nar([jb], alone=False, forward=True),
                    nar([ji] + ([jb] if joint else []) + [ji], alone=False),
                    bool(jb) and nar([jb], alone=False),
                    False,
                    nar([ji], alone=False, params=False),
                    nar([ji], alone=False, forward=True),
                    nar([ji], alone=False, params=False)]
            xg.narrow = sum(1 << i for i, b in enumerate(bits) if b)
        xg.sharded = int(bool(getattr(G, 'sharded', False)))
        xg.pair_i, xg.pair_b = int(bool(G.pair_i)), int(bool(G.pair_b))
        xg.Vol, xg.Nglob, xg.Nbglob, xg.s3_scale = float(G.Vol), float(G.Nglob), float(G.Nbglob), float(G.s3_scale)
        xg.init_off, xg.bdry_off, xg.ckappa = float(G.init_off), float(G.bdry_off), float(self.structure.c_kappa)
        xg.href = 0 if G.href is None else G.href.data_ptr()
        xg.c = xg.cp = 0
        return xg

    def _runner_ok(self, G):
        return (self.use_runner and self.structure.c_kappa is not None and G.c is None and not getattr(G, 'persistent', True))

    def _world_of(self, G):
        return self.world if getattr(G, 'sharded', self.world is not None) else None

    def _field_seen(self, G):
        touched = G.L > 1 or (getattr(G, 'has_bdry', G.Nb > 0) and G.Lb > 1)
        self._field_touched = touched or (self.accum_u is not None and self._field_touched)
        return self._field_touched

    def _narrow_ok(self, jobs, alone, forward=False, params=True):
        kind = 'f' if forward else ('p' if params else 'x')
        if self.narrow == '0' or kind not in self.narrow_set:
            return False
        if not forward and (self.adjoint or self.method > 1 or any(j.get('act') is None for j in jobs)):
            return False
        if self.narrow == '2':
            return True
        tiles = sum((j['xT'].shape[1] + 15) // 16 for j in jobs)
        return tiles <= (self.narrow_tiles_alone if alone else self.narrow_tiles)[kind]

    def _job(self, G, which, ubar=None, gslab=None, want_x=False):
        if which == 'i':
            j = dict(xT=G.xT, start=G.start, u=G.u, Y=G.Y, act=G.act, ubar=ubar, gslab=gslab)
            if want_x:
                j.update(gx=G.gx, gs=G.gs)
        else:
            j = dict(xT=G.xbT, start=G.start_b, u=G.ub, Y=G.Yb, act=G.act_b, ubar=ubar, gslab=gslab)
        return j

    def _contract(self, G, adam_state=None, with_bdry=False):
        fin = None
        if self._world_of(G) is None and adam_state is not None:
            fin = dict(Lb=G.Lb, Nbglob=G.Nbglob, alpha=self.alpha, step=adam_state['step'], init_off=G.init_off, bdry_off=G.bdry_off)
        pair = dict(href=G.href, s3_scale=G.s3_scale) if G.pair_i else None
        bdry = dict(ub=G.ub, g=G.g) if (with_bdry and G.Nb) else None
        if G.A0 is None and G.B0 is None:
            KN.weak_partials(G.u, G.v, G.vt, G.w, G.f, G.h, G.Vol, G.Nglob, self.scal, G.work_i, c=G.c, ckappa=G.ck, wt=G.wt,
                             contract=dict(gx=G.gx, gs=G.gs, ghT=G.ghT, gxv=G.gxv, w0=G.w0, gwx0T=G.gwx0T), finalize=fin, pair=pair,
                             bdry=bdry)
            return
        KN.weak_contract_general(G.A0, G.amode, G.B0, G.gx, G.gs, G.ghT, G.gxv, G.w0, G.gwx0T, G.v[0], G.s3x)
        KN.weak_partials(G.u, G.v, G.vt, G.w, G.f, G.h, G.Vol, G.Nglob, self.scal, G.work_i, s3x=G.s3x, c=G.c, ckappa=G.ck,
                         wt=G.wt, finalize=fin, pair=pair, bdry=bdry)

    def _gen_all(self, G):
        self._gen_front(G)
        self._gen_back(G)

    def _gen_front(self, G):
        th = self.theta.data
        M = (self.method, self.H, self.K, self.m)
        e0 = self._mark()
        fused_x = self.pollution == 1.0 and not self.adjoint
        joint = G.Nb and G.same_grid
        e_x = None
        if self._compact(G, fused_x, joint):
            return self._gen_front_compact(G)
        if not getattr(G, 'skip_v', False):
            self._launch_test_net_here(G)
        with self._side(1, e0):
            fwd = [self._job(G, 'i')] + ([self._job(G, 'b')] if joint else [])
            KN.ode_fwd_multi(fwd, G.t, th, *M, zero16=self.scal, narrow=self._narrow_ok(fwd, alone=False, forward=True),
                             prio_drop=self.prio_drop['G'])
            if G.Nb and not joint:
                fwd_b = [self._job(G, 'b')]
                KN.ode_fwd_multi(fwd_b, G.tb, th, *M, narrow=self._narrow_ok(fwd_b, alone=False, forward=True))
            self._reaction(G)
            e_f = self._mark()
            res_A = dict(u=G.u, ref=G.href if G.pair_i else G.h, coef=2.0 * self.alpha / G.Nglob, base=self.pollution, first_only=True)
            res_b = dict(u=G.ub, ref=G.g, coef=2.0 * self.alpha / (G.Nbglob * G.Lb), base=0.0, first_only=False) if G.Nb else None
            e_b = None
            if not fused_x:
                with self._side(2, e_f):
                    sweep_x = [self._job(G, 'i', want_x=True)]
                    KN.ode_bwd_multi(sweep_x, G.t, th, *M, want_x=True, want_params=False, adjoint=self.adjoint,
                                     narrow=self._narrow_ok(sweep_x, alone=False, params=False))
                    e_x = self._mark()
            sweeps = [dict(self._job(G, 'i', None, G.slabA[:G.ns_u], want_x=fused_x), res=res_A)]
            if joint:
                sweeps.append(dict(self._job(G, 'b', None, G.slabA[G.ns_u:]), res=res_b))
            KN.ode_bwd_multi(sweeps, G.t, th, *M, want_x=fused_x, want_params=True, x_cot_ones=fused_x, adjoint=self.adjoint,
                             narrow=self._narrow_ok(sweeps, alone=False), prio_drop=self.prio_drop['A'])
            if G.Nb and not joint:
                sweep_b = [dict(self._job(G, 'b', None, G.slabA[G.ns_u:]), res=res_b)]
                KN.ode_bwd_multi(sweep_b, G.tb, th, *M, want_x=False, want_params=True, adjoint=self.adjoint,
                                 narrow=self._narrow_ok(sweep_b, alone=False))
            e_A = self._mark()
            G.sumA_ready = self.early_slab_sum and self._world_of(G) is None and self.accum_u is None and self.use_streams
            e_S = None
            if G.sumA_ready:
                if getattr(G, 'sumA', None) is None:
                    G.sumA = torch.empty(self.Pu, dtype=F64, device=self.dev)
                KN.slab_sum(G.slabA, out=G.sumA)
                e_S = self._mark()
        e_v = self._mark()
        self._join(e_f)
        res_B = dict(u=G.u, ref=G.v, coef=G.Vol / G.Nglob / G.L * G.s3_scale, base=G.Vol / G.Nglob,
                     weak=dict(w=G.w, c=G.c, cp=G.cp, ckappa=G.ck))
        sweep_B = [dict(self._job(G, 'i', None, G.slabB), res=res_B)]
        KN.ode_bwd_multi(sweep_B, G.t, th, *M, want_x=False, want_params=True, adjoint=self.adjoint,
                         narrow=self._narrow_ok(sweep_B, alone=True))
        with self._side(3, e_A, e_v, *[e for e in (e_x, e_b) if e is not None]):
            self._contract(G, self.adam_u, with_bdry=True)
            e_C = self._mark()
        self._join(e_C, e_S)

    def _compact(self, G, fused_x, joint):
        tiles = (G.N + 15) // 16 + ((G.Nb + 15) // 16 if G.Nb else 0)
        if not (self.compact_tiles > 0 and self.use_streams and fused_x and joint):
            return False
        return tiles <= self.compact_tiles or bool(getattr(G, 'skip_v', False))

    def _gen_front_compact(self, G):
        th = self.theta.data
        M = (self.method, self.H, self.K, self.m)
        e0 = self._mark()
        if not getattr(G, 'skip_v', False):
            self._launch_test_net_here(G)
        with self._side(1, e0):
            fwd = [self._job(G, 'i'), self._job(G, 'b')]
            lone = bool(getattr(G, 'skip_v', False))
            KN.ode_fwd_multi(fwd, G.t, th, *M, zero16=self.scal, narrow=self._narrow_ok(fwd, alone=lone, forward=True),
                             prio_drop=self.prio_drop['G'])
            self._reaction(G)
            e_f = self._mark()
        self._join(e_f)
        res_A = dict(u=G.u, ref=G.href if G.pair_i else G.h, coef=2.0 * self.alpha / G.Nglob, base=self.pollution, first_only=True)
        res_b = dict(u=G.ub, ref=G.g, coef=2.0 * self.alpha / (G.Nbglob * G.Lb), base=0.0, first_only=False)
        res_B = dict(u=G.u, ref=G.v, coef=G.Vol / G.Nglob / G.L * G.s3_scale, base=G.Vol / G.Nglob,
                     weak=dict(w=G.w, c=G.c, cp=G.cp, ckappa=G.ck))
        sweeps = [dict(self._job(G, 'i', None, G.slabA[:G.ns_u], want_x=True), res=res_A),
                  dict(self._job(G, 'b', None, G.slabA[G.ns_u:]), res=res_b),
                  dict(self._job(G, 'i', None, G.slabB), res=res_B)]
        KN.ode_bwd_multi(sweeps, G.t, th, *M, want_x=True, want_params=True, x_cot_ones=True, adjoint=self.adjoint,
                         narrow=self._narrow_ok(sweeps, alone=bool(getattr(G, 'skip_v', False))))
        G.sumA_ready = False
        self._contract(G, self.adam_u, with_bdry=True)

    def begin_substep(self, which, accumulate):
        name, P = ('accum_u', self.Pu) if which == 'u' else ('accum_v', self.Pv)
        if which == 'u':
            self._field_touched = False
        if not accumulate:
            setattr(self, name, None)
        elif getattr(self, name) is None:
            setattr(self, name, torch.zeros(P, dtype=F64, device=self.dev))
        else:
            getattr(self, name).zero_()

    def _gen_back(self, G):
        lr, st = self.config['u_rate'], self.adam_u
        acc = self.accum_u
        world = self._world_of(G)
        lag = dict(lag=st['lag'], lag_range=self.field_range, skip=self.adam_skips_untouched and not self._field_seen(G))
        if world is not None:
            if G.pair_i:
                KN.pair_fold(self.scal, G.Vol, G.Nglob)
            KN.losses(self.scal, G.L, G.Lb, G.Vol, G.Nglob, G.Nbglob, self.alpha, step=st['step'], init_off=G.init_off,
                      bdry_off=G.bdry_off)
        if world is None and getattr(G, 'sumA_ready', False) and acc is None:
            KN.adam(self.theta.data, None, st['m'], st['v'], st['step'], lr, gslabB=G.slabB, scal=self.scal,
                    gextraA=G.sumA, gsum_out=self.grad_u, bump_step=-1, **lag)
        elif world is None:
            KN.adam(self.theta.data, G.slabA, st['m'], st['v'], st['step'], lr, gslabB=G.slabB, scal=self.scal,
                    gextraA=acc, gsum_out=self.grad_u, bump_step=-1, **lag)
        else:
            P = self.Pu
            if acc is not None:
                self.pack_u[:P].add_(acc)
            KN.adam(self.theta.data, None, st['m'], st['v'], st['step'], lr, gextraA=self.pack_u[:P],
                    gextraB=self.pack_u[P:2 * P], scal=self.scal, gsum_out=self.grad_u, bump_step=-1, **lag)
        if acc is not None:
            acc.copy_(self.grad_u)

    def _v_fresh(self, G, store=False):
        now = self._v_key(G)
        G.skip_v = self.reuse_test_net and getattr(G, 'v_version', None) == now
        G.v_version = now
        if not G.skip_v:
            G.vact_valid = G.vact is not None and (store or self.reuse_test_net)
        return ('_vcached' if G.skip_v else '') + ('_act' if getattr(G, 'vact_valid', False) else '')

    def _v_key(self, G):
        return (self._phi_version, sum(p._version for p in self.phi.params), G.sample_version)

    def invalidate_test_net(self):
        self._phi_version += 1

    def _run_runner(self, fn, *args):
        from ._lib import check
        self._exchange_error = None
        rc = fn(*args)
        if getattr(self, '_exchange_error', None) is not None:
            err, self._exchange_error = self._exchange_error, None
            raise err
        check(rc, fn.__name__)

    def generator_step(self, G):
        sfx = self._v_fresh(G)
        world = self._world_of(G)
        if self._runner_ok(G):
            from ._lib import lib
            skip = self.adam_skips_untouched and not self._field_seen(G)
            G.ck = self.structure.c_kappa
            self._run_runner(lib.xw_substep_gen, self._runner_group(G), self._runner_state(), int(bool(G.skip_v)),
                             int(bool(getattr(G, 'vact_valid', False))), KN._p(self.accum_u), int(skip), KN._stream())
            return
        if world is None:
            self._run(G, 'gen' + sfx, self._gen_all)
            return
        if self.capture_exchange:
            self._run(G, 'gen_dist' + sfx, self._gen_all_dist)
            return
        self._run(G, 'gen_front' + sfx, self._gen_front_packed)
        world.all_reduce(self.pack_u)
        self._run(G, 'gen_back', self._gen_back)

    def _gen_all_dist(self, G):
        self._gen_front_packed(G)
        self.world.all_reduce(self.pack_u)
        self._gen_back(G)

    def _gen_front_packed(self, G):
        P = self.Pu
        if G.N == 0:
            return self._gen_front_empty(G)
        self._gen_front(G)
        KN.slab_sum2(G.slabA, self.pack_u[:P], G.slabB, self.pack_u[P:2 * P])

    def _gen_front_empty(self, G):
        P, th = self.Pu, self.theta.data
        M = (self.method, self.H, self.K, self.m)
        self.pack_u.zero_()
        if not G.Nb:
            return
        fwd_b = [self._job(G, 'b')]
        KN.ode_fwd_multi(fwd_b, G.tb, th, *M, narrow=self._narrow_ok(fwd_b, alone=False, forward=True))
        res_b = dict(u=G.ub, ref=G.g, coef=2.0 * self.alpha / (G.Nbglob * G.Lb), base=0.0, first_only=False)
        sweep_b = [dict(self._job(G, 'b', None, G.slabA[G.ns_u:]), res=res_b)]
        KN.ode_bwd_multi(sweep_b, G.tb, th, *M, want_x=False, want_params=True, adjoint=self.adjoint,
                         narrow=self._narrow_ok(sweep_b, alone=False))
        KN.bdry_partials(G.ub, G.g, self.alpha, G.Nbglob, self.scal, G.work_b)
        KN.slab_sum(G.slabA[G.ns_u:], out=self.pack_u[:P])

    def _disc_front(self, G):
        th = self.theta.data
        M = (self.method, self.H, self.K, self.m)
        if G.N == 0:
            self.scal.zero_()
            return
        e0 = self._mark()
        if not getattr(G, 'skip_v', False):
            self._launch_test_net_here(G, blocks=self.v_blocks_disc)
        with self._side(1, e0):
            fwd = [self._job(G, 'i')]
            lone = bool(getattr(G, 'skip_v', False))
            KN.ode_fwd_multi(fwd, G.t, th, *M, zero16=self.scal, act_x_only=True, narrow=self._narrow_ok(fwd, alone=lone, forward=True),
                             prio_drop=self.prio_drop['F'])
            self._reaction(G)
            sweep_x = [self._job(G, 'i', want_x=True)]
            KN.ode_bwd_multi(sweep_x, G.t, th, *M, want_x=True, want_params=False, adjoint=self.adjoint,
                             narrow=self._narrow_ok(sweep_x, alone=lone, params=False), prio_drop=self.prio_drop['X'])
            e_x = self._mark()
        self._join(e_x)
        self._contract(G, self.adam_v)

    def _disc_mid(self, G):
        KN.disc_cotangent(G.u, G.v, G.w, G.f, G.h, G.Vol, G.Nglob, self.scal, G.vbar, c=G.c, ckappa=G.ck,
                          pollution=self.pollution, s3_scale=G.s3_scale)
        act = G.vact if getattr(G, 'vact_valid', False) else None
        if G.tpp is None:
            KN.disc_bwd(G.xvT, G.t, self.phi.data, G.vbar, self.W, self.q, gslab=G.slab_v, act=act)
        else:
            KN.disc_bwd(G.xvT_pts, None, self.phi.data, G.vbar.view(1, -1), self.W, self.q, tpp=G.tpp, gslab=G.slab_v, act=act)

    def _disc_mid_packed(self, G):
        if G.N == 0:
            self.grad_v.zero_()
            return
        self._disc_mid(G)
        KN.slab_sum(G.slab_v, out=self.grad_v)

    def _disc_back(self, G):
        lr, st = self.config['v_rate'], self.adam_v
        acc = self.accum_v
        world = self._world_of(G)
        if world is not None:
            KN.losses(self.scal, G.L, G.Lb, G.Vol, G.Nglob, G.Nbglob, self.alpha, step=st['step'])
        if world is None:
            KN.adam(self.phi.data, G.slab_v, st['m'], st['v'], st['step'], lr, gextraA=acc, gsum_out=self.grad_v,
                    bump_step=-1)
        else:
            if acc is not None:
                self.grad_v.add_(acc)
            KN.adam(self.phi.data, None, st['m'], st['v'], st['step'], lr, gextraA=self.grad_v, bump_step=-1)
        if acc is not None:
            acc.copy_(self.grad_v)

    def _reduce_sums(self, G):
        self.world.all_reduce(self.scal[0:9])
        if G.pair_i:
            KN.pair_fold(self.scal, G.Vol, G.Nglob)

    def _disc_all(self, G):
        self._disc_front(G)
        self._disc_mid(G)
        self._disc_back(G)

    def _disc_all_dist(self, G):
        self._disc_front(G)
        self._reduce_sums(G)
        self._disc_mid_packed(G)
        self.world.all_reduce(self.grad_v)
        self._disc_back(G)

    def discriminator_step(self, G):
        sfx = self._v_fresh(G, store=True)
        self._phi_version += 1
        world = self._world_of(G)
        if self._runner_ok(G):
            from ._lib import lib
            G.ck = self.structure.c_kappa
            self._run_runner(lib.xw_substep_disc, self._runner_group(G), self._runner_state(), int(bool(G.skip_v)),
                             int(bool(getattr(G, 'vact_valid', False))), KN._p(self.accum_v), KN._stream())
            return
        if world is None:
            self._run(G, 'disc' + sfx, self._disc_all)
            return
        if self.capture_exchange:
            self._run(G, 'disc_dist' + sfx, self._disc_all_dist)
            return
        self._run(G, 'disc_front' + sfx, self._disc_front)
        self._reduce_sums(G)
        self._run(G, 'disc_mid' + ('_act' if getattr(G, 'vact_valid', False) else ''), self._disc_mid_packed)
        world.all_reduce(self.grad_v)
        self._run(G, 'disc_back', self._disc_back)

    def _run(self, G, key, fn, scratch=False):
        capturable = (self.use_graphs and self.accum_u is None and self.accum_v is None and getattr(G, 'persistent', True)
                      and not (G.pair_i or G.pair_b))
        g = G.graphs.get(key) if capturable else False
        if g is False:
            if not getattr(G, 'persistent', True) and self.use_streams:
                self.use_streams = False
                self._eager_seen = getattr(self, '_eager_seen', 0) + 1
                KN.TRUSTED = self._eager_seen > self.eager_checked
                try:
                    fn(G)
                finally:
                    self.use_streams = True
                    KN.TRUSTED = False
                return
            fn(G)
            return
        if g is None:
            ran_eager = self.structure.c_kappa is None
            if ran_eager:
                fn(G)
            g = torch.cuda.CUDAGraph()
            torch.cuda.synchronize()
            try:
                with HIP_HOST_LOCK, torch.cuda.graph(g, pool=_scratch_pool(int(scratch) - 1) if scratch else None, stream=self._capture_stream(),
                                                     capture_error_mode='thread_local'):
                    fn(G)
            except Exception as exc:
                if self.options.strict_graphs:
                    raise
                import warnings
                warnings.warn('HIP graph capture of sub-step segment %r failed (%s: %s); this segment now runs as eager kernel launches '
                              '(expect a several times lower step rate)' % (key, type(exc).__name__, exc), RuntimeWarning, stacklevel=2)
                G.graphs[key] = False
                self.eager_segments = getattr(self, 'eager_segments', 0) + 1
                torch.cuda.synchronize()
                if not ran_eager:
                    fn(G)
                return
            G.graphs[key] = g
            _KEPT_GRAPHS.append(g)
            if len(_KEPT_GRAPHS) in (256, 1024, 4096):
                import warnings
                warnings.warn('%d captured HIP graphs are being kept alive (destroying one faults a later launch on this runtime, '
                              'engine._KEPT_GRAPHS): a long-lived process that keeps building solvers should run them with '
                              'XW_GRAPHS=0 or in child processes' % len(_KEPT_GRAPHS), RuntimeWarning, stacklevel=3)
            if ran_eager:
                return
        with HIP_HOST_LOCK:
            g.replay()

    def _capture_stream(self):
        return self._cap

    def loss_u(self):
        return self.scal[4]

    def loss_v(self):
        return self.scal[5]

    def predict_group(self, G):
        u, _ = KN.ode_fwd(G.xT, G.t, G.start, self.theta.data, self.method, self.H, self.K, self.m, want_Y=False)
        return u.t().unsqueeze(2)

    def predict(self, X):
        Xd = X.detach()
        starts_T0 = float(Xd[0, 0, 0]) == self.setup['T0']
        s = self.funcs['h'](Xd[:, 0, :]) if starts_T0 else self.funcs['g'](Xd[:, 0, :].unsqueeze(1)).reshape(-1)
        u, _ = KN.ode_fwd(Xd[:, 0, 1:].to(self.dev).to(F64).t().contiguous(), Xd[0, :, 0].to(self.dev).to(F64).contiguous(),
                          s.detach().to(self.dev).to(F64).reshape(-1).contiguous(), self.theta.data, self.method,
                          self.H, self.K, self.m, want_Y=False)
        return u
```

xnode_wan_pde_solver_amd/kernels.py:

```python
import torch

from ._lib import lib, check, XnwanError, XwOdeFwdJob, XwOdeBwdJob

METHODS = {'euler': 0, 'midpoint': 1, 'rk4': 2}
F32, F64 = torch.float32, torch.float64


def _need_gpu():
    if not torch.cuda.is_available():
        raise XnwanError('no GPU visible: the XNODE-WAN kernels only run on an MI355X (gfx950); there is no CPU path')


TRUSTED = False
LONE_NARROW = __import__('os').environ.get('XW_LONE_NARROW', '1') == '1'


def _chk(t, dtype, shape, name):
    if t is None or TRUSTED:
        return
    if not (torch.is_tensor(t) and t.is_cuda):
        raise XnwanError('%s must be a CUDA/HIP tensor' % name)
    if t.dtype != dtype:
        raise XnwanError('%s must be %s, got %s' % (name, dtype, t.dtype))
    if not t.is_contiguous():
        raise XnwanError('%s must be contiguous' % name)
    if shape is not None and tuple(t.shape) != tuple(shape):
        raise XnwanError('%s must have shape %s, got %s' % (name, tuple(shape), tuple(t.shape)))


def _p(t):
    return 0 if t is None else t.data_ptr()


_raw_stream = getattr(torch._C, '_cuda_getCurrentRawStream', None)


def _stream():
    if _raw_stream is not None:
        return _raw_stream(torch.cuda.current_device())
    return torch.cuda.current_stream().cuda_stream


def method_id(name):
    if name not in METHODS:
        raise XnwanError("solver %r is not a fixed-grid scheme of this engine (have: %s)" % (name, sorted(METHODS)))
    return METHODS[name]


ODE_WIDTHS = [(20, 10), (32, 12), (64, 16)]
DISC_WIDTHS = [50, 64, 96, 128]
GENERIC_ODE_MAX = (64, 16)
GENERIC_DISC_MAX = 128


ODE_WIDE_MAX_DEPTH = 10
ODE_MAX_DEPTH = 10
GENERIC_ODE_MAX_DEPTH = 32


def ode_container(H, K, m=1):
    for Hc, Kc in ODE_WIDTHS:
        if m > (ODE_WIDE_MAX_DEPTH if (Hc, Kc) == ODE_WIDTHS[-1] else ODE_MAX_DEPTH):
            continue
        if H <= Hc and K <= Kc and lib.xw_theta_size(1, Hc, Kc) > 0 and lib.xw_ode_act_rows(0, Hc, Kc, 1) >= 0:
            return Hc, Kc
    if H <= GENERIC_ODE_MAX[0] and K <= GENERIC_ODE_MAX[1] and m <= GENERIC_ODE_MAX_DEPTH and lib.xw_ode_act_rows(0, H, K, m) >= 0:
        return H, K
    raise XnwanError('u_hidden_dim = %d, u_hidden_hidden_dim = %d, u_layers = %d: the stepper kernels serve widths up to %s (MFMA) / %s (generic '
                     'path), depths up to %d / %d' % (H, K, m, ODE_WIDTHS[-1], GENERIC_ODE_MAX, ODE_MAX_DEPTH, GENERIC_ODE_MAX_DEPTH))


def ode_generic(H, K, m=1):
    return (H, K) not in ODE_WIDTHS or m > (ODE_WIDE_MAX_DEPTH if (H, K) == ODE_WIDTHS[-1] else ODE_MAX_DEPTH)


def disc_container(W):
    for Wc in DISC_WIDTHS:
        if W <= Wc and lib.xw_disc_act_rows(Wc, 1) >= 0:
            return Wc
    if W <= GENERIC_DISC_MAX and lib.xw_disc_act_rows(W, 1) >= 0:
        return W
    raise XnwanError('v_hidden_dim = %d: the test-network kernels serve widths up to %d (MFMA) / %d (generic path)'
                     % (W, DISC_WIDTHS[-1], GENERIC_DISC_MAX))


def disc_generic(W):
    return W not in DISC_WIDTHS


def theta_size(d, H, K):
    return lib.xw_theta_size(d, H, K)


def phi_size(d, W):
    return lib.xw_phi_size(d, W)


def ode_fwd(xT, t, start, theta, method, H, K, m, want_Y=True, u=None, Y=None):
    _need_gpu()
    d, N = xT.shape
    L = t.shape[0]
    _chk(xT, F64, (d, N), 'xT'); _chk(t, F64, (L,), 't'); _chk(start, F64, (N,), 'start')
    _chk(theta, F64, (theta_size(d, H, K),), 'theta')
    if u is None:
        u = torch.empty(L, N, dtype=F64, device=xT.device)
    if Y is None and want_Y:
        Y = torch.empty(L, H, N, dtype=F64, device=xT.device)
    _chk(u, F64, (L, N), 'u'); _chk(Y, F64, (L, H, N), 'Y')
    if Y is None and LONE_NARROW and (N + 15) // 16 <= 256 and (H, K) in ODE_WIDTHS:
        arr = (XwOdeFwdJob * 1)()
        a = arr[0]
        a.xT, a.start, a.u, a.Y, a.act, a.N, a.act_x_only, a.narrow, a.prio_drop = _p(xT), _p(start), _p(u), 0, 0, N, 0, 1, 0
        check(lib.xw_ode_fwd_multi(arr, 1, _p(t), _p(theta), method, L, d, H, K, m, 0, _stream()), 'xw_ode_fwd_multi')
        return u, None
    check(lib.xw_ode_fwd(_p(xT), _p(t), _p(start), _p(theta), method, N, L, d, H, K, m, _p(u), _p(Y), _stream()), 'xw_ode_fwd')
    return u, Y


def ode_fwd_multi(jobs, t, theta, method, H, K, m, zero16=None, act_x_only=False, narrow=False, prio_drop=0):
    _need_gpu()
    L = t.shape[0]
    d = jobs[0]['xT'].shape[0]
    _chk(t, F64, (L,), 't'); _chk(theta, F64, (theta_size(d, H, K),), 'theta')
    arr = (XwOdeFwdJob * len(jobs))()
    for a, j in zip(arr, jobs):
        N = j['xT'].shape[1]
        _chk(j['xT'], F64, (d, N), 'xT'); _chk(j['start'], F64, (N,), 'start'); _chk(j['u'], F64, (L, N), 'u')
        _chk(j.get('Y'), F64, (L, H, N), 'Y')
        if j.get('act') is not None:
            _chk(j['act'], F64, (max(L - 1, 1), ode_act_rows(method, H, K, m), ode_act_cols(N)), 'act')
        a.xT, a.start, a.u, a.Y, a.act, a.N = _p(j['xT']), _p(j['start']), _p(j['u']), _p(j.get('Y')), _p(j.get('act')), N
        a.act_x_only = 1 if act_x_only else 0
        a.narrow = 1 if narrow else 0
        a.prio_drop = int(prio_drop)
    _chk(zero16, F64, (16,), 'zero16')
    check(lib.xw_ode_fwd_multi(arr, len(jobs), _p(t), _p(theta), method, L, d, H, K, m, _p(zero16), _stream()), 'xw_ode_fwd_multi')


def ode_bwd_multi(jobs, t, theta, method, H, K, m, want_x, want_params, x_cot_ones=False, adjoint=False, narrow=False, prio_drop=0):
    _need_gpu()
    L = t.shape[0]
    d = jobs[0]['xT'].shape[0]
    P = theta_size(d, H, K)
    _chk(t, F64, (L,), 't'); _chk(theta, F64, (P,), 'theta')
    arr = (XwOdeBwdJob * len(jobs))()
    for a, j in zip(arr, jobs):
        N = j['xT'].shape[1]
        _chk(j['xT'], F64, (d, N), 'xT'); _chk(j['start'], F64, (N,), 'start'); _chk(j['Y'], F64, (L, H, N), 'Y')
        _chk(j.get('ubar'), F64, (L, N), 'ubar')
        if want_x and not (x_cot_ones and j.get('gx') is None):
            _chk(j['gx'], F64, (d, N), 'gx'); _chk(j['gs'], F64, (N,), 'gs')
        if want_params:
            _chk(j['gslab'], F64, (ode_bwd_slabs(N), P), 'gslab')
        if j.get('act') is not None:
            _chk(j['act'], F64, (max(L - 1, 1), ode_act_rows(method, H, K, m), ode_act_cols(N)), 'act')
        a.xT, a.start, a.Y, a.ubar, a.N = _p(j['xT']), _p(j['start']), _p(j['Y']), _p(j.get('ubar')), N
        a.act = _p(j.get('act'))
        a.gx, a.gs, a.gslab = _p(j.get('gx')), _p(j.get('gs')), _p(j.get('gslab'))
        res = j.get('res')
        if res is not None:
            if j.get('ubar') is not None:
                raise XnwanError('a sweep job takes a stored cotangent (ubar) or a residual (res), not both')
            if res.get('weak') is not None:
                wk = res['weak']
                wpp = wk['w'].dim() == 2
                _chk(res['u'], F64, (L, N), 'res.u'); _chk(res['ref'], F64, (L, N), 'res.ref (v)')
                _chk(wk['w'], F64, (L, N) if wpp else (N,), 'res.weak.w'); _chk(wk.get('c'), F64, (L, N), 'res.weak.c')
                _chk(wk.get('cp'), F64, (L, N), 'res.weak.cp')
                a.res_first_only, a.res_u, a.res_ref = 2, _p(res['u']), _p(res['ref'])
                a.res_w_per_point, a.res_w, a.res_c, a.res_cp = int(wpp), _p(wk['w']), _p(wk.get('c')), _p(wk.get('cp'))
                a.res_kappa2 = 2.0 * float(wk.get('ckappa', 0.0))
            else:
                first = bool(res['first_only'])
                _chk(res['u'], F64, (L, N), 'res.u'); _chk(res['ref'], F64, (N,) if first else (L, N), 'res.ref')
                a.res_first_only, a.res_u, a.res_ref = int(first), _p(res['u']), _p(res['ref'])
            a.res_coef, a.res_base = float(res['coef']), float(res['base'])
    if x_cot_ones and not (want_x and want_params):
        raise XnwanError('x_cot_ones needs want_x and want_params')
    if x_cot_ones and adjoint:
        raise XnwanError('x_cot_ones is not available with the continuous adjoint')
    if narrow and (adjoint or method > 1 or any(j.get('act') is None for j in jobs)):
        raise XnwanError('narrow-tile sweeps run from the activation store of euler / midpoint (no adjoint=True, no rk4)')
    mode = (1 if want_x else 0) | (2 if want_params else 0) | (4 if x_cot_ones else 0) | (8 if adjoint else 0) | (16 if narrow else 0) | ((int(prio_drop) & 3) << 5)
    check(lib.xw_ode_bwd_multi(arr, len(jobs), _p(t), _p(theta), method, L, d, H, K, m, mode, _stream()), 'xw_ode_bwd_multi')


def ode_bwd_slabs(N):
    return lib.xw_ode_bwd_slabs(N)


def ode_act_cols(N):
    return (N + 15) // 16 * 16


def ode_act_rows(method, H, K, m):
    r = lib.xw_ode_act_rows(int(method), H, K, m)
    check(min(r, 0), 'xw_ode_act_rows')
    return r


def ode_bwd(xT, t, start, theta, Y, ubar, method, H, K, m, want_x=True, want_params=False, gx=None, gs=None, gslab=None,
            adjoint=False):
    _need_gpu()
    d, N = xT.shape
    L = t.shape[0]
    P = theta_size(d, H, K)
    _chk(xT, F64, (d, N), 'xT'); _chk(t, F64, (L,), 't'); _chk(start, F64, (N,), 'start'); _chk(theta, F64, (P,), 'theta')
    _chk(Y, F64, (L, H, N), 'Y'); _chk(ubar, F64, (L, N), 'ubar')
    mode = (1 if want_x else 0) | (2 if want_params else 0) | (8 if adjoint else 0)
    if want_x:
        gx = torch.empty(d, N, dtype=F64, device=xT.device) if gx is None else gx
        gs = torch.empty(N, dtype=F64, device=xT.device) if gs is None else gs
        _chk(gx, F64, (d, N), 'gx'); _chk(gs, F64, (N,), 'gs')
    if want_params:
        ns = ode_bwd_slabs(N)
        gslab = torch.empty(ns, P, dtype=F64, device=xT.device) if gslab is None else gslab
        _chk(gslab, F64, (ns, P), 'gslab')
    check(lib.xw_ode_bwd(_p(xT), _p(t), _p(start), _p(theta), _p(Y), _p(ubar), method, N, L, d, H, K, m, mode,
                         _p(gx if want_x else None), _p(gs if want_x else None), _p(gslab if want_params else None),
                         _stream()), 'xw_ode_bwd')
    return (gx if want_x else None), (gs if want_x else None), (gslab if want_params else None)


DISC_UNROLLED_DEPTH = 9


def disc_recompute(W, q):
    return W == 50 and q == DISC_UNROLLED_DEPTH


def disc_act_rows(W, q):
    r = lib.xw_disc_act_rows(W, q)
    check(min(r, 0), 'xw_disc_act_rows')
    return r


def disc_act_view(act, W, q):
    rows = disc_act_rows(W, q)
    return act.reshape(-1)[:act.numel()].view(act.shape[1] // 16, rows, 16)


def disc_act_cols(P):
    return (P + 15) // 16 * 16


def disc_xproj_rows(W):
    return 128 if W > 96 else 96 if W > 64 else 64


def disc_xproj(xT, phi, W, out=None):
    _need_gpu()
    d, N = xT.shape
    _chk(xT, F64, (d, N), 'xT'); _chk(phi, F64, (phi_size(d, W),), 'phi')
    rows = disc_xproj_rows(W)
    out = torch.empty(rows, N, dtype=F64, device=xT.device) if out is None else out
    _chk(out, F64, (rows, N), 'xproj')
    check(lib.xw_disc_xproj(_p(xT), _p(phi), N, d, W, _p(out), _stream()), 'xw_disc_xproj')
    return out


def disc_fwd(xT, t, phi, W, q, tpp=None, want_vt=True, v=None, vt=None, gxv=None, gtv=None, ngrad=0, max_blocks=0, act=None,
             xproj=None):
    _need_gpu()
    d, N = xT.shape
    L = 1 if tpp is not None else t.shape[0]
    _chk(xT, F64, (d, N), 'xT'); _chk(phi, F64, (phi_size(d, W),), 'phi')
    _chk(t, F64, None, 't'); _chk(tpp, F64, (N,), 'tpp')
    v = torch.empty(L, N, dtype=F64, device=xT.device) if v is None else v
    if want_vt and vt is None:
        vt = torch.empty(L, N, dtype=F64, device=xT.device)
    _chk(v, F64, (L, N), 'v'); _chk(vt, F64, (L, N), 'vt')
    if gxv is not None:
        _chk(gxv, F64, (d, ngrad), 'gxv'); _chk(gtv, F64, (ngrad,), 'gtv')
    if act is not None:
        _chk(act, F64, (disc_act_rows(W, q), disc_act_cols(L * N)), 'act')
    if xproj is not None:
        _chk(xproj, F64, (disc_xproj_rows(W), N), 'xproj')
    check(lib.xw_disc_fwd_xproj(_p(xT), _p(t), _p(tpp), _p(phi), N, L, d, W, q, _p(v), _p(vt if want_vt else None), _p(gxv),
                                _p(gtv), int(ngrad), int(max_blocks), _p(act), _p(xproj), _stream()), 'xw_disc_fwd')
    return v, (vt if want_vt else None)


def disc_gradx(xT, t, phi, W, q, tpp=None, vbar=None, gxv=None, gtv=None):
    _need_gpu()
    d, N = xT.shape
    _chk(xT, F64, (d, N), 'xT'); _chk(phi, F64, (phi_size(d, W),), 'phi'); _chk(t, F64, None, 't'); _chk(tpp, F64, (N,), 'tpp')
    gxv = torch.empty(d, N, dtype=F64, device=xT.device) if gxv is None else gxv
    gtv = torch.empty(N, dtype=F64, device=xT.device) if gtv is None else gtv
    _chk(gxv, F64, (d, N), 'gxv'); _chk(gtv, F64, (N,), 'gtv')
    if vbar is not None:
        vbar = vbar.reshape(-1)
        _chk(vbar, F64, (N,), 'vbar')
    if not disc_recompute(W, q):
        t0 = t[:1] if tpp is None else None
        disc_fwd(xT, t0, phi, W, q, tpp=tpp, want_vt=False, gxv=gxv, gtv=gtv, ngrad=N)
        if vbar is not None:
            gxv.mul_(vbar)
            gtv.mul_(vbar)
        return gxv, gtv
    check(lib.xw_disc_gradx(_p(xT), _p(t), _p(tpp), _p(phi), _p(vbar), N, d, W, q, _p(gxv), _p(gtv), _stream()), 'xw_disc_gradx')
    return gxv, gtv


def disc_bwd_slabs(N, L):
    return lib.xw_disc_bwd_slabs(N, L)


def disc_bwd(xT, t, phi, vbar, W, q, tpp=None, gslab=None, act=None):
    _need_gpu()
    d, N = xT.shape
    L = 1 if tpp is not None else t.shape[0]
    P = phi_size(d, W)
    _chk(xT, F64, (d, N), 'xT'); _chk(phi, F64, (P,), 'phi'); _chk(vbar, F64, (L, N), 'vbar')
    _chk(t, F64, None, 't'); _chk(tpp, F64, (N,), 'tpp')
    ns = disc_bwd_slabs(N, L)
    gslab = torch.empty(ns, P, dtype=F64, device=xT.device) if gslab is None else gslab
    _chk(gslab, F64, (ns, P), 'gslab')
    if act is None and not disc_recompute(W, q):
        act = torch.empty(disc_act_rows(W, q), disc_act_cols(L * N), dtype=F64, device=xT.device)
        disc_fwd(xT, t, phi, W, q, tpp=tpp, want_vt=False, act=act)
    if act is not None:
        _chk(act, F64, (disc_act_rows(W, q), disc_act_cols(L * N)), 'act')
    check(lib.xw_disc_bwd(_p(xT), _p(t), _p(tpp), _p(phi), _p(vbar), N, L, d, W, q, _p(act), _p(gslab), _stream()),
          'xw_disc_bwd')
    return gslab


def reduce_work_size():
    return lib.xw_reduce_work_size()


def weak_partials(u, v, vt, w, f, h, Vol, Nglob, scal, work, s3x=None, contract=None, c=None, ckappa=0.0, wt=None,
                  finalize=None, pair=None, bdry=None):
    _need_gpu()
    L, N = u.shape
    for name, a in (('u', u), ('v', v), ('vt', vt), ('f', f)):
        _chk(a, F64, (L, N), name)
    per_point = 1 if w.dim() == 2 else 0
    _chk(w, F64, (L, N) if per_point else (N,), 'w'); _chk(wt, F64, (L, N), 'wt'); _chk(c, F64, (L, N), 'c')
    _chk(s3x, F64, (N,), 's3x'); _chk(h, F64, (N,), 'h'); _chk(scal, F64, (16,), 'scal')
    _chk(work, F64, (reduce_work_size(),), 'work')
    fz = finalize or {}
    _chk(fz.get('step'), torch.int64, (1,), 'step')
    bd, Pb = bdry or {}, 0
    if bdry is not None:
        Pb = bdry['ub'].numel()
        _chk(bdry['ub'], F64, tuple(bdry['ub'].shape), 'ub'); _chk(bdry['g'], F64, tuple(bdry['ub'].shape), 'g')
    pr = pair or {}
    _chk(pr.get('href'), F64, (N,), 'href')
    if pair is not None and L != 1:
        raise XnwanError('the pairwise form only exists for single-slice groups (L == 1)')
    k, d = {}, 0
    if s3x is None:
        k = contract
        d = k['gx'].shape[0]
        for name in ('gx', 'ghT', 'gxv', 'gwx0T'):
            _chk(k[name], F64, (d, N), name)
        _chk(k['gs'], F64, (N,), 'gs'); _chk(k['w0'], F64, (N,), 'w0')
    check(lib.xw_weak_partials(_p(u), _p(v), _p(vt), _p(w), per_point, _p(wt), _p(s3x), _p(k.get('gx')), _p(k.get('gs')),
                               _p(k.get('ghT')), _p(k.get('gxv')), _p(k.get('w0')), _p(k.get('gwx0T')), d, _p(c),
                               float(ckappa), _p(f), _p(h), _p(pr.get('href')), 0 if pair is None else 1,
                               float(pr.get('s3_scale', 1.0)), N, L, float(Vol), float(Nglob), _p(work), _p(scal),
                               0 if finalize is None else 1, max(int(fz.get('Lb', 1)), 1), float(fz.get('Nbglob', 1.0)),
                               float(fz.get('alpha', 0.0)), float(fz.get('init_off', 0.0)), float(fz.get('bdry_off', 0.0)),
                               _p(fz.get('step')), _p(bd.get('ub')), _p(bd.get('g')), Pb, _stream()),
          'xw_weak_partials')


def pair_fold(scal, Vol, Nglob):
    _need_gpu()
    _chk(scal, F64, (16,), 'scal')
    check(lib.xw_pair_fold(_p(scal), float(Vol), float(Nglob), _stream()), 'xw_pair_fold')


def cube_weight(x, top, bot, w, gwT, w0=None, xT=None):
    _need_gpu()
    N, d = x.shape
    _chk(x, torch.float32, (N, d), 'x')
    _chk(w, F64, (N,), 'w')
    _chk(gwT, F64, (d, N), 'gwT')
    if w0 is not None:
        _chk(w0, F64, (N,), 'w0')
    if xT is not None:
        _chk(xT, F64, (d, N), 'xT')
    check(lib.xw_cube_weight(_p(x), N, d, float(top), float(bot), _p(w), _p(w0), _p(gwT), _p(xT), _stream()), 'xw_cube_weight')


GATHER_ROWS = 1024


def gather_fields(table, count, total):
    _need_gpu()
    if table.dtype != torch.int64 or table.dim() != 2 or table.shape[1] != 9 or not table.is_contiguous() or table.shape[0] < count:
        raise XnwanError('gather table: need a contiguous int64 [>= count, 9] device tensor')
    check(lib.xw_gather_fields(_p(table), int(count), int(total), _stream()), 'xw_gather_fields')


def weak_contract_general(A0, amode, B0, gx, gs, ghT, gxv, w0, gwx0T, v0, s3x):
    _need_gpu()
    d, N = gx.shape
    for name, a in (('gx', gx), ('ghT', ghT), ('gxv', gxv), ('gwx0T', gwx0T)):
        _chk(a, F64, (d, N), name)
    for name, a in (('gs', gs), ('w0', w0), ('v0', v0), ('s3x', s3x)):
        _chk(a, F64, (N,), name)
    _chk(B0, F64, (d, N), 'B0')
    amode = int(amode)
    if amode not in (0, 1, 2, 3) or (amode == 0) != (A0 is None):
        raise XnwanError('weak_contract_general: amode %r does not match A0' % (amode,))
    if amode:
        _chk(A0, F64, {1: (d, d), 2: (d, N), 3: (d, d, N)}[amode], 'A0')
    check(lib.xw_weak_contract_general(_p(A0), amode, _p(B0), _p(gx), _p(gs), _p(ghT), _p(gxv), _p(w0), _p(gwx0T), _p(v0), d, N,
                                       _p(s3x), _stream()), 'xw_weak_contract_general')
    return s3x


def bdry_partials(ub, g, alpha, Nbglob, scal, work, ubar_b=None):
    _need_gpu()
    L, Nb = ub.shape
    _chk(ub, F64, (L, Nb), 'ub'); _chk(g, F64, (L, Nb), 'g'); _chk(ubar_b, F64, (L, Nb), 'ubar_b'); _chk(scal, F64, (16,), 'scal')
    _chk(work, F64, (reduce_work_size(),), 'work')
    check(lib.xw_bdry_partials(_p(ub), _p(g), Nb, L, float(alpha), float(Nbglob), _p(ubar_b), _p(work), _p(scal), _stream()),
          'xw_bdry_partials')


def gen_cotangents(u, v, w, h, Vol, Nglob, alpha, ubarA, ubarB, c=None, cp=None, ckappa=0.0, pollution=1.0, scal=None):
    _need_gpu()
    if ubarA is None and ubarB is None:
        raise XnwanError('gen_cotangents: nothing to compute')
    L, N = u.shape
    per_point = 1 if w.dim() == 2 else 0
    _chk(u, F64, (L, N), 'u'); _chk(v, F64, (L, N), 'v'); _chk(w, F64, (L, N) if per_point else (N,), 'w')
    _chk(c, F64, (L, N), 'c'); _chk(cp, F64, (L, N), 'cp'); _chk(h, F64, (N,), 'h')
    _chk(ubarA, F64, (L, N), 'ubarA'); _chk(ubarB, F64, (L, N), 'ubarB'); _chk(scal, F64, (16,), 'scal')
    check(lib.xw_gen_cotangents(_p(u), _p(v), _p(w), per_point, _p(c), _p(cp), float(ckappa), _p(h), N, L, float(Vol),
                                float(Nglob), float(alpha), float(pollution), _p(scal), _p(ubarA), _p(ubarB), _stream()),
          'xw_gen_cotangents')


def disc_cotangent(u, v, w, f, h, Vol, Nglob, scal, vbar, c=None, ckappa=0.0, pollution=1.0, s3_scale=1.0):
    _need_gpu()
    L, N = u.shape
    per_point = 1 if w.dim() == 2 else 0
    _chk(u, F64, (L, N), 'u'); _chk(v, F64, (L, N), 'v'); _chk(w, F64, (L, N) if per_point else (N,), 'w')
    _chk(c, F64, (L, N), 'c'); _chk(f, F64, (L, N), 'f'); _chk(h, F64, (N,), 'h'); _chk(vbar, F64, (L, N), 'vbar')
    _chk(scal, F64, (16,), 'scal')
    check(lib.xw_disc_cotangent(_p(u), _p(v), _p(w), per_point, _p(c), float(ckappa), _p(f), _p(h), N, L, float(Vol),
                                float(Nglob), float(pollution), float(s3_scale), _p(scal), _p(vbar), _stream()), 'xw_disc_cotangent')


def losses(scal, L, Lb, Vol, Nglob, Nbglob, alpha, step=None, init_off=0.0, bdry_off=0.0):
    _need_gpu()
    _chk(scal, F64, (16,), 'scal'); _chk(step, torch.int64, (1,), 'step')
    check(lib.xw_losses(_p(scal), L, max(int(Lb), 1), float(Vol), float(Nglob), float(Nbglob), float(alpha), float(init_off),
                        float(bdry_off), _p(step), _stream()), 'xw_losses')


def adam(param, gslabA, m, v, step, lr, beta1=0.9, beta2=0.999, eps=1e-8, gextraA=None, gslabB=None, gextraB=None,
         scal=None, gsum_out=None, bump_step=True, lag=None, lag_range=(0, 0), skip=False):
    _need_gpu()
    P = param.shape[0]
    _chk(param, F64, (P,), 'param'); _chk(m, F64, (P,), 'm'); _chk(v, F64, (P,), 'v'); _chk(step, torch.int64, (1,), 'step')
    nA = nB = 0
    if gslabA is not None:
        nA = gslabA.shape[0]
        _chk(gslabA, F64, (nA, P), 'gslabA')
    if gslabB is not None:
        nB = gslabB.shape[0]
        _chk(gslabB, F64, (nB, P), 'gslabB')
    _chk(gextraA, F64, (P,), 'gextraA'); _chk(gextraB, F64, (P,), 'gextraB'); _chk(gsum_out, F64, (P,), 'gsum_out')
    _chk(scal, F64, (16,), 'scal'); _chk(lag, torch.int64, (1,), 'lag')
    lo, hi = (int(lag_range[0]), int(lag_range[1])) if lag is not None else (0, 0)
    check(lib.xw_adam(_p(param), _p(gslabA), nA, _p(gextraA), _p(gslabB), nB, _p(gextraB), _p(scal), _p(m), _p(v), _p(step),
                      (1 if bump_step is True else 0 if bump_step is False else int(bump_step)), P,
                      float(lr), float(beta1), float(beta2), float(eps), _p(gsum_out), lo, hi, 1 if skip else 0, _p(lag),
                      _stream()), 'xw_adam')


def slab_sum2(gA, outA, gB, outB):
    _need_gpu()
    (nA, P), (nB, P2) = gA.shape, gB.shape
    _chk(gA, F64, (nA, P), 'gA'); _chk(gB, F64, (nB, P), 'gB'); _chk(outA, F64, (P,), 'outA'); _chk(outB, F64, (P,), 'outB')
    check(lib.xw_slab_sum2(_p(gA), nA, _p(outA), _p(gB), nB, _p(outB), P, _stream()), 'xw_slab_sum2')


def slab_sum(gslab, out=None, accumulate=False):
    _need_gpu()
    ns, P = gslab.shape
    _chk(gslab, F64, (ns, P), 'gslab')
    out = torch.empty(P, dtype=F64, device=gslab.device) if out is None else out
    _chk(out, F64, (P,), 'out')
    check(lib.xw_slab_sum(_p(gslab), ns, P, 1 if accumulate else 0, _p(out), _stream()), 'xw_slab_sum')
    return out
```

Before: 2126.

## Fold disc cotangent into disc backward, precomputing dI rows on side stream

The scal-independent part of the discriminator cotangent (dI) is now computed on the side stream right after the ODE x-sweep, overlapping with the main stream. The disc backward kernels form vbar on the fly from dI, v, w and scal. This removes the separate disc_cotangent launch and its vbar write and read from the critical path. In exchange the backward kernels do a few more global loads per point, plus extra branching and a new ABI entry point.

New measurement: 2132 (median of 6 runs). About the same (+0.2%).

```diff
diff --git a/include/xnwan.h b/include/xnwan.h
--- a/include/xnwan.h
+++ b/include/xnwan.h
@@ -57,6 +57,10 @@
 int xw_disc_bwd_slabs(int N, int L);
 int xw_disc_bwd(const double* xT, const double* t, const double* tpp, const double* phi, const double* vbar,
                 int N, int L, int d, int W, int q, const double* act, double* gslab, void* stream);
+int xw_disc_bwd_rows_ok(int W, int q, int have_record);
+int xw_disc_bwd_rows(const double* xT, const double* t, const double* tpp, const double* phi, const double* dI_row,
+                     const double* v, const double* w, int w_per_point, int Nrow, double pollution, const double* scal,
+                     int N, int L, int d, int W, int q, const double* act, double* gslab, void* stream);
 
 int xw_weak_partials(const double* u, const double* v, const double* vt, const double* w, int w_per_point,
                      const double* wt, const double* s3x, const double* gx, const double* gs, const double* ghT,
@@ -80,6 +84,8 @@
 int xw_disc_cotangent(const double* u, const double* v, const double* w, int w_per_point, const double* c,
                       double ckappa, const double* f, const double* h, int N, int L, double Vol, double Nglob,
                       double pollution, double s3_scale, const double* scal_in, double* vbar, void* stream);
+int xw_disc_dI_row(const double* u, const double* w, int w_per_point, const double* c, double ckappa, const double* f,
+                   const double* h, int N, int L, double Vol, double Nglob, double s3_scale, double* dI_row, void* stream);
 int xw_losses(double* scal, int L, int Lb, double Vol, double Nglob, double Nbglob, double alpha, double init_off,
               double bdry_off, long long* step, void* stream);
 
diff --git a/xnode_wan_pde_solver_amd/_lib.py b/xnode_wan_pde_solver_amd/_lib.py
--- a/xnode_wan_pde_solver_amd/_lib.py
+++ b/xnode_wan_pde_solver_amd/_lib.py
@@ -3,7 +3,7 @@
 
 _HERE = os.path.dirname(os.path.abspath(__file__))
 LIB_PATH = os.environ.get('XW_LIBRARY') or os.path.join(_HERE, 'libxnwan.so')
-ABI_VERSION = 31
+ABI_VERSION = 32
 
 c_f32p = ctypes.c_void_p
 c_f64p = ctypes.c_void_p
@@ -66,6 +66,9 @@
     'xw_disc_gradx': [c_f32p, c_f32p, c_f32p, c_f64p, c_f64p, c_int, c_int, c_int, c_int, c_f64p, c_f64p, c_vp],
     'xw_disc_bwd_slabs': [c_int, c_int],
     'xw_disc_bwd': [c_f32p, c_f32p, c_f32p, c_f64p, c_f64p, c_int, c_int, c_int, c_int, c_int, c_f64p, c_f64p, c_vp],
+    'xw_disc_bwd_rows_ok': [c_int, c_int, c_int],
+    'xw_disc_bwd_rows': [c_f32p, c_f32p, c_f32p, c_f64p, c_f64p, c_f64p, c_f64p, c_int, c_int, c_dbl, c_f64p, c_int, c_int, c_int,
+                         c_int, c_int, c_f64p, c_f64p, c_vp],
     'xw_mt19937_uniform_f32': [c_vp, ctypes.c_long, c_vp, ctypes.c_long, ctypes.c_float, ctypes.c_float, c_int],
     'xw_gather_fields': [c_vp, c_int, ctypes.c_long, c_vp],
     'xw_mt19937_legacy_normal_f64': [c_vp, ctypes.POINTER(c_int), ctypes.POINTER(c_int), ctypes.POINTER(c_dbl), c_vp, ctypes.c_long],
@@ -81,6 +84,7 @@
                           c_dbl, c_f64p, c_f64p, c_f64p, c_vp],
     'xw_disc_cotangent': [c_f64p, c_f64p, c_f64p, c_int, c_f64p, c_dbl, c_f64p, c_f64p, c_int, c_int, c_dbl, c_dbl, c_dbl,
                           c_dbl, c_f64p, c_f64p, c_vp],
+    'xw_disc_dI_row': [c_f64p, c_f64p, c_int, c_f64p, c_dbl, c_f64p, c_f64p, c_int, c_int, c_dbl, c_dbl, c_dbl, c_f64p, c_vp],
     'xw_losses': [c_f64p, c_int, c_int, c_dbl, c_dbl, c_dbl, c_dbl, c_dbl, c_dbl, c_i64p, c_vp],
     'xw_adam': [c_f64p, c_f64p, c_int, c_f64p, c_f64p, c_int, c_f64p, c_f64p, c_f64p, c_f64p, c_i64p, c_int, c_int, c_dbl,
                 c_dbl, c_dbl, c_dbl, c_f64p, c_int, c_int, c_int, c_i64p, c_vp],
diff --git a/xnode_wan_pde_solver_amd/csrc/xw_common.h b/xnode_wan_pde_solver_amd/csrc/xw_common.h
--- a/xnode_wan_pde_solver_amd/csrc/xw_common.h
+++ b/xnode_wan_pde_solver_amd/csrc/xw_common.h
@@ -210,6 +210,25 @@
   return tile[(l & 15) * XW_TSTRIDE + 4 * ks + (l >> 4)];
 }
 
+__device__ __forceinline__ double xw_disc_dI_row(double ul, double wl, double cl, double fl, double hn, int l, int L, double cN,
+                                                 double cNL, double s3_scale) {
+  double dI = cNL * s3_scale * (cl * ul + fl) * wl;
+  if (l == L - 1) dI += cN * ul;
+  if (l == 0) dI -= cN * hn;
+  return dI;
+}
+__device__ __forceinline__ double xw_disc_vbar(double pollution, double wl, double cI, double dI, double vl, double S) {
+  return pollution * wl - cI * dI + 2.0 * vl / S;
+}
+struct XwVbarRows {
+  const double* dI;
+  const double* v;
+  const double* w;
+  const double* scal;
+  int w_per_point, Nrow;
+  double pollution;
+};
+
 static inline int xw_launch_status() {
   hipError_t e = hipGetLastError();
   return e == hipSuccess ? 0 : (int)e;
diff --git a/xnode_wan_pde_solver_amd/csrc/xw_disc.hip b/xnode_wan_pde_solver_amd/csrc/xw_disc.hip
--- a/xnode_wan_pde_solver_amd/csrc/xw_disc.hip
+++ b/xnode_wan_pde_solver_amd/csrc/xw_disc.hip
@@ -400,10 +400,18 @@
   static_assert(total * 8 <= 160 * 1024, "LDS budget of one CU");
 };
 
+__device__ __forceinline__ double vbar_at(const double* vbar, const XwVbarRows& vr, double cI, double S, long p) {
+  if (vr.dI != nullptr) {
+    const double wl = xw_ld_g(vr.w + (vr.w_per_point ? p : (long)((int)p % vr.Nrow)));
+    return xw_disc_vbar(vr.pollution, wl, cI, xw_ld_g(vr.dI + p), xw_ld_g(vr.v + p), S);
+  }
+  return vbar != nullptr ? xw_ld_g(vbar + p) : 1.0;
+}
+
 template <int W, int Q, int CTG, bool PARAMS, bool INGRAD>
 __global__ void __launch_bounds__(256) k_disc_bwd(const double* __restrict__ xT, const double* __restrict__ tf,
                                                   const double* __restrict__ tpp, const double* __restrict__ ph,
-                                                  const double* __restrict__ vbar, int N, int L, int d,
+                                                  const double* __restrict__ vbar, XwVbarRows vr, int N, int L, int d,
                                                   double* __restrict__ gslab, double* __restrict__ gxv,
                                                   double* __restrict__ gtv) {
   typedef VDim<W> D;
@@ -421,6 +429,7 @@
   const VOff o = v_offsets(d, W);
   const long P = (long)N * L;
   const long nsuper = (P + 63) / 64;
+  const double vr_cI = vr.dI != nullptr ? 2.0 / vr.scal[0] : 0.0, vr_S = vr.dI != nullptr ? vr.scal[1] : 1.0;
 
   double* sB = lds + S::oB;
   for (int idx = wave; idx < D::MT * D::KS; idx += 4) {
@@ -477,7 +486,7 @@
       }
       layer(r, a);
     }
-    const double vb = pt.valid ? (vbar != nullptr ? vbar[pt.p] : 1.0) : 0.0;
+    const double vb = pt.valid ? vbar_at(vbar, vr, vr_cI, vr_S, pt.p) : 0.0;
     d4 dl[D::MT];
 #pragma unroll
     for (int mt = 0; mt < D::MT; ++mt)
@@ -688,7 +697,7 @@
 template <int W, int Q, int NG, bool TSUM>
 __global__ void __launch_bounds__(256, RecLds<W>::VT ? 2 : 1) k_disc_rec(const double* __restrict__ xT, const double* __restrict__ tf,
                                                      const double* __restrict__ tpp, const double* __restrict__ ph,
-                                                     const double* __restrict__ vbar, int N, int L, int d,
+                                                     const double* __restrict__ vbar, XwVbarRows vr, int N, int L, int d,
                                                      double* __restrict__ gslab, const double* __restrict__ act, int qrt) {
   typedef VDim<W> D;
   typedef RecLds<W> S;
@@ -707,6 +716,7 @@
   const VOff o = v_offsets(d, W);
   const long P = (long)N * L;
   const long nsuper = (P + 63) / 64;
+  const double vr_cI = vr.dI != nullptr ? 2.0 / vr.scal[0] : 0.0, vr_S = vr.dI != nullptr ? vr.scal[1] : 1.0;
   const int nq = Q > 0 ? Q : qrt;
   constexpr int UNROLL = Q > 0 ? Q : 1;
   constexpr int TW = D::MT / 2;
@@ -778,7 +788,7 @@
     d4 a[D::MT], rnext[D::MT];
     load_layer(nq, a);
     if (nq > 0) load_layer(nq - 1, rnext);
-    const double vb = pt.valid ? (vbar != nullptr ? xw_ld_g(vbar + pt.p) : 1.0) : 0.0;
+    const double vb = pt.valid ? vbar_at(vbar, vr, vr_cI, vr_S, pt.p) : 0.0;
     d4 dl[D::MT];
 #pragma unroll
     for (int mt = 0; mt < D::MT; ++mt)
@@ -1241,18 +1251,21 @@
 
 #define XW_DISC_BWD(PARAMS, INGRAD)                                                                                      \
   if (d + 2 <= 64)                                                                                                       \
-    hipLaunchKernelGGL((k_disc_bwd<50, 9, 1, PARAMS, INGRAD>), dim3(blocks), dim3(256), 0, s, xT, t, tpp, phi, vbar,     \
+    hipLaunchKernelGGL((k_disc_bwd<50, 9, 1, PARAMS, INGRAD>), dim3(blocks), dim3(256), 0, s, xT, t, tpp, phi, vbar, vr, \
                        N, L, d, gslab, gxv, gtv);                                                                        \
   else                                                                                                                   \
-    hipLaunchKernelGGL((k_disc_bwd<50, 9, 2, PARAMS, INGRAD>), dim3(blocks), dim3(256), 0, s, xT, t, tpp, phi, vbar,     \
+    hipLaunchKernelGGL((k_disc_bwd<50, 9, 2, PARAMS, INGRAD>), dim3(blocks), dim3(256), 0, s, xT, t, tpp, phi, vbar, vr, \
                        N, L, d, gslab, gxv, gtv);
 
-extern "C" int xw_disc_bwd(const double* xT, const double* t, const double* tpp, const double* phi, const double* vbar,
-                           int N, int L, int d, int W, int q, const double* act, double* gslab, void* stream) {
+static int disc_bwd(const double* xT, const double* t, const double* tpp, const double* phi, const double* vbar, const XwVbarRows& vr,
+                    int N, int L, int d, int W, int q, const double* act, double* gslab, void* stream) {
   if (!xT || !phi || !gslab || N <= 0 || L <= 0 || d <= 0) return XW_E_ARG;
   if (!tpp && !t) return XW_E_ARG;
   if (tpp && L != 1) return XW_E_ARG;
-  if (!disc_width_ok(W)) return xwg_disc_bwd(xT, t, tpp, phi, vbar, N, L, d, W, q, act, gslab, bwd_blocks((long)N * L), stream);
+  if (!disc_width_ok(W)) {
+    if (vr.dI != nullptr) return XW_E_DIMS;
+    return xwg_disc_bwd(xT, t, tpp, phi, vbar, N, L, d, W, q, act, gslab, bwd_blocks((long)N * L), stream);
+  }
   if (q < 0 || d + 2 > 128 || ((q != 9 || W != 50) && act == nullptr)) return XW_E_DIMS;
   if ((long)N * L * 4 >= (1L << 31)) return XW_E_ARG;
   hipStream_t s = (hipStream_t)stream;
@@ -1264,8 +1277,8 @@
     static const bool tsum_on = [] { const char* e = getenv("XW_DISC_REC_TSUM"); return !(e && e[0] == '0'); }();
     const bool tsum = tsum_on && tpp == nullptr && (N % 64) == 0;
 #define XW_DISC_REC(W_, Q, NG)                                                                                          \
-    if (tsum) hipLaunchKernelGGL((k_disc_rec<W_, Q, NG, true>), dim3(blocks), dim3(256), 0, s, xT, t, tpp, phi, vbar, N, L, d, gslab, act, q); \
-    else hipLaunchKernelGGL((k_disc_rec<W_, Q, NG, false>), dim3(blocks), dim3(256), 0, s, xT, t, tpp, phi, vbar, N, L, d, gslab, act, q);
+    if (tsum) hipLaunchKernelGGL((k_disc_rec<W_, Q, NG, true>), dim3(blocks), dim3(256), 0, s, xT, t, tpp, phi, vbar, vr, N, L, d, gslab, act, q); \
+    else hipLaunchKernelGGL((k_disc_rec<W_, Q, NG, false>), dim3(blocks), dim3(256), 0, s, xT, t, tpp, phi, vbar, vr, N, L, d, gslab, act, q);
     if (W == 128) {
       if (ng == 1) { XW_DISC_REC(128, 0, 1) } else if (ng == 2) { XW_DISC_REC(128, 0, 2) } else { XW_DISC_REC(128, 0, 3) }
     } else if (W == 96) {
@@ -1280,6 +1293,26 @@
     XW_DISC_BWD(true, false)
   }
   return xw_launch_status();
+}
+
+extern "C" int xw_disc_bwd(const double* xT, const double* t, const double* tpp, const double* phi, const double* vbar,
+                           int N, int L, int d, int W, int q, const double* act, double* gslab, void* stream) {
+  return disc_bwd(xT, t, tpp, phi, vbar, XwVbarRows{}, N, L, d, W, q, act, gslab, stream);
+}
+
+extern "C" int xw_disc_bwd_rows_ok(int W, int q, int have_record) {
+  return disc_width_ok(W) && q >= 0 && (have_record || (W == 50 && q == 9)) ? 1 : 0;
+}
+
+extern "C" int xw_disc_bwd_rows(const double* xT, const double* t, const double* tpp, const double* phi, const double* dI_row,
+                                const double* v, const double* w, int w_per_point, int Nrow, double pollution, const double* scal,
+                                int N, int L, int d, int W, int q, const double* act, double* gslab, void* stream) {
+  if (!dI_row || !v || !w || !scal || Nrow <= 0 || (long)N * L % Nrow != 0) return XW_E_ARG;
+  if (!xw_disc_bwd_rows_ok(W, q, act != nullptr)) return XW_E_DIMS;
+  XwVbarRows vr;
+  vr.dI = dI_row; vr.v = v; vr.w = w; vr.scal = scal;
+  vr.w_per_point = w_per_point; vr.Nrow = Nrow; vr.pollution = pollution;
+  return disc_bwd(xT, t, tpp, phi, nullptr, vr, N, L, d, W, q, act, gslab, stream);
 }
 
 extern "C" int xw_disc_gradx(const double* xT, const double* t, const double* tpp, const double* phi, const double* vbar,
@@ -1291,6 +1324,7 @@
   const int L = 1;
   const int blocks = bwd_blocks((long)N);
   double* gslab = nullptr;
+  const XwVbarRows vr{};
   XW_DISC_BWD(false, true)
   return xw_launch_status();
 }
diff --git a/xnode_wan_pde_solver_amd/csrc/xw_substep.hip b/xnode_wan_pde_solver_amd/csrc/xw_substep.hip
--- a/xnode_wan_pde_solver_amd/csrc/xw_substep.hip
+++ b/xnode_wan_pde_solver_amd/csrc/xw_substep.hip
@@ -175,6 +175,7 @@
   const bool have_i = g->N > 0;
   const int adj = s->adjoint ? 8 : 0;
   double* record = use_record ? g->vact : nullptr;
+  const bool rows = have_i && !shard && xw_disc_bwd_rows_ok(s->W, s->q, record != nullptr);
   void* const main_stream = stream;
   if (have_i) {
     Side* sd = side_of_current_device();
@@ -190,6 +191,9 @@
       jx.gx = g->gx; jx.gs = g->gs;
       XW_TRY(xw_ode_bwd_multi(&jx, 1, g->t, s->theta, s->method, g->L, g->d, s->H, s->K, s->m, 1 | adj | (((g->narrow >> 7) & 1) ? 16 : 0),
                               stream));
+      if (rows)
+        XW_TRY(xw_disc_dI_row(g->u, g->w, g->w_per_point, g->c, g->ckappa, g->f, g->h, g->N, g->L, g->Vol, g->Nglob, g->s3_scale, g->vbar,
+                              stream));
     }
     XW_HIP(hipEventRecord(sd->done, sd->s));
     stream = main_stream;
@@ -203,7 +207,15 @@
     if (g->pair_i) XW_TRY(xw_pair_fold(s->scal, g->Vol, g->Nglob, stream));
   }
   const int nsv = have_i ? xw_disc_bwd_slabs(g->N, g->L) : 0;
-  if (have_i) {
+  if (rows) {
+    if (g->tpp != nullptr) {
+      XW_TRY(xw_disc_bwd_rows(g->xvT_pts, nullptr, g->tpp, s->phi, g->vbar, g->v, g->w, g->w_per_point, g->N, s->pollution, s->scal,
+                              g->N * g->L, 1, g->d, s->W, s->q, record, g->slab_v, stream));
+    } else {
+      XW_TRY(xw_disc_bwd_rows(g->xvT, g->t, nullptr, s->phi, g->vbar, g->v, g->w, g->w_per_point, g->N, s->pollution, s->scal, g->N,
+                              g->L, g->d, s->W, s->q, record, g->slab_v, stream));
+    }
+  } else if (have_i) {
     XW_TRY(xw_disc_cotangent(g->u, g->v, g->w, g->w_per_point, g->c, g->ckappa, g->f, g->h, g->N, g->L, g->Vol, g->Nglob, s->pollution,
                              g->s3_scale, s->scal, g->vbar, stream));
     if (g->tpp != nullptr) {
diff --git a/xnode_wan_pde_solver_amd/csrc/xw_weak.hip b/xnode_wan_pde_solver_amd/csrc/xw_weak.hip
--- a/xnode_wan_pde_solver_amd/csrc/xw_weak.hip
+++ b/xnode_wan_pde_solver_amd/csrc/xw_weak.hip
@@ -243,10 +243,23 @@
     const double ul = u[p], vl = v[p];
     const double wl = w_per_point ? w[p] : w[n];
     const double cl = c != nullptr ? c[p] : ckappa * ul;
-    double dI = cNL * s3_scale * (cl * ul + f[p]) * wl;
-    if (l == L - 1) dI += cN * ul;
-    if (l == 0) dI -= cN * h[n];
-    vbar[p] = pollution * wl - cI * dI + 2.0 * vl / S;
+    const double dI = xw_disc_dI_row(ul, wl, cl, f[p], l == 0 ? h[n] : 0.0, l, L, cN, cNL, s3_scale);
+    vbar[p] = xw_disc_vbar(pollution, wl, cI, dI, vl, S);
+  }
+}
+
+__global__ void __launch_bounds__(256) k_disc_dI(const double* __restrict__ u, const double* __restrict__ w, int w_per_point,
+                                                 const double* __restrict__ c, double ckappa, const double* __restrict__ f,
+                                                 const double* __restrict__ h, int N, int L, double Vol, double Nglob,
+                                                 double s3_scale, double* __restrict__ dI_row) {
+  const double cN = Vol / Nglob, cNL = Vol / Nglob / (double)L;
+  const long P = (long)N * L;
+  for (long p = (long)blockIdx.x * blockDim.x + threadIdx.x; p < P; p += (long)gridDim.x * blockDim.x) {
+    const int l = (int)(p / N), n = (int)(p - (long)l * N);
+    const double ul = u[p];
+    const double wl = w_per_point ? w[p] : w[n];
+    const double cl = c != nullptr ? c[p] : ckappa * ul;
+    dI_row[p] = xw_disc_dI_row(ul, wl, cl, f[p], l == 0 ? h[n] : 0.0, l, L, cN, cNL, s3_scale);
   }
 }
 
@@ -452,6 +465,14 @@
   return xw_launch_status();
 }
 
+extern "C" int xw_disc_dI_row(const double* u, const double* w, int w_per_point, const double* c, double ckappa, const double* f,
+                              const double* h, int N, int L, double Vol, double Nglob, double s3_scale, double* dI_row, void* stream) {
+  if (!u || !w || !f || !h || !dI_row || N <= 0 || L <= 0) return XW_E_ARG;
+  hipLaunchKernelGGL(k_disc_dI, dim3(blocks_for((long)N * L, 256, 2048)), dim3(256), 0, (hipStream_t)stream, u, w, w_per_point, c,
+                     ckappa, f, h, N, L, Vol, Nglob, s3_scale, dI_row);
+  return xw_launch_status();
+}
+
 extern "C" int xw_adam(double* param, const double* gslabA, int nA, const double* gextraA, const double* gslabB, int nB,
                        const double* gextraB, const double* scal, double* m, double* v, long long* step, int bump_step,
                        int P, double lr, double beta1, double beta2, double eps, double* gsum_out, int lag_lo, int lag_hi,
@@ -501,7 +522,7 @@
   return xw_launch_status();
 }
 
-extern "C" int xw_abi_version(void) { return 31; }
+extern "C" int xw_abi_version(void) { return 32; }
 extern "C" int xw_reduce_work_size(void) { return 6 * 1024 + 8; }
 
 extern "C" int xw_supported_dims(char* buf, int buflen) {
diff --git a/xnode_wan_pde_solver_amd/engine.py b/xnode_wan_pde_solver_amd/engine.py
--- a/xnode_wan_pde_solver_amd/engine.py
+++ b/xnode_wan_pde_solver_amd/engine.py
@@ -1107,18 +1107,28 @@
             sweep_x = [self._job(G, 'i', want_x=True)]
             KN.ode_bwd_multi(sweep_x, G.t, th, *M, want_x=True, want_params=False, adjoint=self.adjoint,
                              narrow=self._narrow_ok(sweep_x, alone=lone, params=False), prio_drop=self.prio_drop['X'])
+            if self._disc_rows(G):
+                KN.disc_dI_row(G.u, G.w, G.f, G.h, G.Vol, G.Nglob, G.vbar, c=G.c, ckappa=G.ck, s3_scale=G.s3_scale)
             e_x = self._mark()
         self._join(e_x)
         self._contract(G, self.adam_v)
 
+    def _disc_rows(self, G):
+        return self._world_of(G) is None and KN.disc_rows_ok(self.W, self.q, getattr(G, 'vact_valid', False))
+
     def _disc_mid(self, G):
-        KN.disc_cotangent(G.u, G.v, G.w, G.f, G.h, G.Vol, G.Nglob, self.scal, G.vbar, c=G.c, ckappa=G.ck,
-                          pollution=self.pollution, s3_scale=G.s3_scale)
+        rows = None
+        if self._disc_rows(G):
+            rows = dict(v=G.v, w=G.w, scal=self.scal, pollution=self.pollution)
+        else:
+            KN.disc_cotangent(G.u, G.v, G.w, G.f, G.h, G.Vol, G.Nglob, self.scal, G.vbar, c=G.c, ckappa=G.ck,
+                              pollution=self.pollution, s3_scale=G.s3_scale)
         act = G.vact if getattr(G, 'vact_valid', False) else None
         if G.tpp is None:
-            KN.disc_bwd(G.xvT, G.t, self.phi.data, G.vbar, self.W, self.q, gslab=G.slab_v, act=act)
+            KN.disc_bwd(G.xvT, G.t, self.phi.data, G.vbar, self.W, self.q, gslab=G.slab_v, act=act, rows=rows)
         else:
-            KN.disc_bwd(G.xvT_pts, None, self.phi.data, G.vbar.view(1, -1), self.W, self.q, tpp=G.tpp, gslab=G.slab_v, act=act)
+            KN.disc_bwd(G.xvT_pts, None, self.phi.data, G.vbar.view(1, -1), self.W, self.q, tpp=G.tpp, gslab=G.slab_v, act=act,
+                        rows=rows)
 
     def _disc_mid_packed(self, G):
         if G.N == 0:
diff --git a/xnode_wan_pde_solver_amd/kernels.py b/xnode_wan_pde_solver_amd/kernels.py
--- a/xnode_wan_pde_solver_amd/kernels.py
+++ b/xnode_wan_pde_solver_amd/kernels.py
@@ -306,7 +306,7 @@
     return lib.xw_disc_bwd_slabs(N, L)
 
 
-def disc_bwd(xT, t, phi, vbar, W, q, tpp=None, gslab=None, act=None):
+def disc_bwd(xT, t, phi, vbar, W, q, tpp=None, gslab=None, act=None, rows=None):
     _need_gpu()
     d, N = xT.shape
     L = 1 if tpp is not None else t.shape[0]
@@ -321,8 +321,18 @@
         disc_fwd(xT, t, phi, W, q, tpp=tpp, want_vt=False, act=act)
     if act is not None:
         _chk(act, F64, (disc_act_rows(W, q), disc_act_cols(L * N)), 'act')
-    check(lib.xw_disc_bwd(_p(xT), _p(t), _p(tpp), _p(phi), _p(vbar), N, L, d, W, q, _p(act), _p(gslab), _stream()),
-          'xw_disc_bwd')
+    if rows is None:
+        check(lib.xw_disc_bwd(_p(xT), _p(t), _p(tpp), _p(phi), _p(vbar), N, L, d, W, q, _p(act), _p(gslab), _stream()),
+              'xw_disc_bwd')
+        return gslab
+    v, w = rows['v'], rows['w']
+    _chk(v, F64, None, 'v'); _chk(w, F64, None, 'w'); _chk(rows['scal'], F64, (16,), 'scal')
+    per_point = 1 if w.dim() == 2 else 0
+    if v.numel() != L * N or (per_point and w.numel() != L * N) or (L * N) % w.shape[-1]:
+        raise ValueError('disc_bwd(rows=...): v %s / w %s do not cover the %d points' % (tuple(v.shape), tuple(w.shape), L * N))
+    check(lib.xw_disc_bwd_rows(_p(xT), _p(t), _p(tpp), _p(phi), _p(vbar), _p(v), _p(w), per_point, w.shape[-1],
+                               float(rows['pollution']), _p(rows['scal']), N, L, d, W, q, _p(act), _p(gslab), _stream()),
+          'xw_disc_bwd_rows')
     return gslab
 
 
@@ -448,6 +458,20 @@
                                 float(Nglob), float(pollution), float(s3_scale), _p(scal), _p(vbar), _stream()), 'xw_disc_cotangent')
 
 
+def disc_dI_row(u, w, f, h, Vol, Nglob, dI, c=None, ckappa=0.0, s3_scale=1.0):
+    _need_gpu()
+    L, N = u.shape
+    per_point = 1 if w.dim() == 2 else 0
+    _chk(u, F64, (L, N), 'u'); _chk(w, F64, (L, N) if per_point else (N,), 'w'); _chk(c, F64, (L, N), 'c')
+    _chk(f, F64, (L, N), 'f'); _chk(h, F64, (N,), 'h'); _chk(dI, F64, (L, N), 'dI')
+    check(lib.xw_disc_dI_row(_p(u), _p(w), per_point, _p(c), float(ckappa), _p(f), _p(h), N, L, float(Vol), float(Nglob),
+                             float(s3_scale), _p(dI), _stream()), 'xw_disc_dI_row')
+
+
+def disc_rows_ok(W, q, have_record):
+    return bool(lib.xw_disc_bwd_rows_ok(int(W), int(q), int(bool(have_record))))
+
+
 def losses(scal, L, Lb, Vol, Nglob, Nbglob, alpha, step=None, init_off=0.0, bdry_off=0.0):
     _need_gpu()
     _chk(scal, F64, (16,), 'scal'); _chk(step, torch.int64, (1,), 'step')
```
